# ATTron/astroz

Hardware: AMD Instinct MI355X
Metric: propagations/sec, 13,478 sats x 1,440 times, at 1/2/4/8 MI355X (higher is better)
Workload: dtype f64

## Files before the change

astroz_amd/csrc/astroz_hip.hip:

```cpp
#include "../../include/astroz_hip.h"

#include <hip/hip_runtime.h>
#include <dlfcn.h>
#include <rccl/rccl.h>

#include <algorithm>
#include <atomic>
#include <cmath>
#include <condition_variable>
#include <deque>
#include <map>
#include <cstdio>
#include <cstdlib>
#include <cstring>
#include <mutex>
#include <new>
#include <memory>
#include <string>
#include <thread>
#include <type_traits>
#include <vector>

#include "kernels.h"
#include "passes_kernel.h"
#include "coverage_kernel.h"
#include "sun.h"
#include "eclipse_kernel.h"
#include "los.h"
#include "access_kernel.h"
#include "conjunction.h"
#include "conjunction_kernel.h"
#include "tle_host.h"
#include "host_step.h"

namespace {

thread_local std::string g_last_error;

bool hip_ok(hipError_t e, const char *what)
{
    if (e == hipSuccess) return true;
    g_last_error = std::string(what) + ": " + hipGetErrorString(e);
    (void)hipGetLastError();
    return false;
}
#define HIP_TRY(expr)                                                                                       \
    do {                                                                                                    \
        if (!hip_ok((expr), #expr)) return AZ_ERR_HIP;                                                      \
    } while (0)

AzGrav make_grav(int which)
{
    AzGrav g;
    if (which == AZ_WGS72) {
        g.radius_km = 6378.135;
        g.j2 = 0.001082616;
        g.j4 = -0.00000165597;
        g.xke = 0.0743669161331734132;
        g.j3oj2 = -0.00234506972242078;
    } else {
        g.radius_km = 6378.137;
        g.j2 = 0.00108262998905;
        g.j4 = -0.00000161098761;
        g.xke = 0.07436685316871385;
        g.j3oj2 = -0.00233899967218727;
    }
    g.vkmpersec = g.xke * g.radius_km / 60.0;
    g.half_j2 = 0.5 * g.j2;
    return g;
}

const char *const kFieldNames[] = {
#define X(n) #n,
    AZ_SGP4_FIELDS(X) AZ_DEEP_FIELDS(X)
#undef X
};


template <class T>
struct DevBuf {
    T *p = nullptr;
    size_t cap = 0;
    DevBuf() = default;
    DevBuf(DevBuf &&o) noexcept { swap(o); }
    DevBuf &operator=(DevBuf &&o) noexcept { swap(o); return *this; }
    ~DevBuf() { if (p) (void)hipFree(p); }
    void swap(DevBuf &o) noexcept { std::swap(p, o.p); std::swap(cap, o.cap); }
    int ensure(size_t n)
    {
        if (n <= cap) return AZ_OK;
        if (p) (void)hipFree(p);
        p = nullptr;
        cap = 0;
        size_t want = std::max<size_t>(n, 64);
        if (!hip_ok(hipMalloc((void **)&p, want * sizeof(T)), "hipMalloc")) return AZ_ERR_HIP;
        cap = want;
        return AZ_OK;
    }
};

struct PinnedBuf {
    void *p = nullptr;
    size_t cap = 0;
    PinnedBuf() = default;
    PinnedBuf(PinnedBuf &&o) noexcept { swap(o); }
    PinnedBuf &operator=(PinnedBuf &&o) noexcept { swap(o); return *this; }
    ~PinnedBuf() { if (p) (void)hipHostFree(p); }
    void swap(PinnedBuf &o) noexcept { std::swap(p, o.p); std::swap(cap, o.cap); }
    int32_t ensure(size_t bytes)
    {
        if (bytes <= cap) return AZ_OK;
        size_t want = std::max<size_t>(cap, 65536);
        while (want < bytes) want *= 2;
        if (p) (void)hipHostFree(p);
        p = nullptr;
        cap = 0;
        if (!hip_ok(hipHostMalloc(&p, want, hipHostMallocDefault), "hipHostMalloc")) return AZ_ERR_HIP;
        cap = want;
        return AZ_OK;
    }
};

template <class H, hipError_t (*Create)(H *, unsigned), hipError_t (*Destroy)(H)>
class HipHandle {
  public:
    HipHandle() = default;
    HipHandle(HipHandle &&o) noexcept { swap(o); }
    HipHandle &operator=(HipHandle &&o) noexcept { swap(o); return *this; }
    ~HipHandle() { reset(); }
    void swap(HipHandle &o) noexcept { std::swap(h_, o.h_); std::swap(own_, o.own_); }
    hipError_t create(unsigned flags)
    {
        reset();
        own_ = true;
        return Create(&h_, flags);
    }
    void borrow(H h)
    {
        reset();
        h_ = h;
        own_ = false;
    }
    void reset()
    {
        if (h_ && own_) (void)Destroy(h_);
        h_ = nullptr;
    }
    bool owned() const { return h_ && own_; }
    operator H() const { return h_; }

  private:
    H h_ = nullptr;
    bool own_ = false;
};
using Stream = HipHandle<hipStream_t, hipStreamCreateWithFlags, hipStreamDestroy>;
using Event = HipHandle<hipEvent_t, hipEventCreateWithFlags, hipEventDestroy>;

constexpr int kStageSlots = 3;
constexpr size_t kStageChunk = size_t(16) << 20;
struct HostStager {
    Event ev[kStageSlots];
    PinnedBuf slot[kStageSlots];
    int32_t ensure()
    {
        for (int k = 0; k < kStageSlots; ++k) {
            if (slot[k].ensure(kStageChunk) != AZ_OK) return AZ_ERR_HIP;
            if (!ev[k] && !hip_ok(ev[k].create(hipEventDisableTiming), "hipEventCreate")) return AZ_ERR_HIP;
        }
        return AZ_OK;
    }
};
}

struct azh_constellation {
    int device = 0;
    size_t n = 0, n_pad = 0;
    AzGrav g{};
    Stream s_main, s_deep, s_ecc;
    Event ev_fork, ev_join, ev_fork2, ev_join2, ev_t0, ev_t1;
    Event ev_one;
    Event ev_graph;
    DevBuf<double> d_el;
    DevBuf<unsigned> d_flags;
    std::vector<unsigned> h_flags;
    std::vector<double> h_epoch;
    std::vector<double> h_raw[AZ_NUM_RAW];
    DevBuf<unsigned> d_list;
    std::vector<unsigned> h_list;
    unsigned n_sgp4 = 0, n_sdp4 = 0, n_bad = 0;
    DevBuf<double> d_times, d_offsets, d_sin, d_cos, d_seeds;
    DevBuf<double> d_node_cache;
    struct FastPlan {
        bool valid = false, mixed32 = false;
        unsigned tile_c = 0, tile_e = 0, n_list = 0, n_seg = 0, parity = 0;
        DevBuf<double> win;
        DevBuf<unsigned char> flag;
        DevBuf<unsigned> redo;
    } plan[4];
    int last_plan = -1;
    DevBuf<double> d_inc;
    DevBuf<double> d_fast_rec;
    double uniform_step = 0.0;
    DevBuf<float> d_delta;
    double delta_max = 0.0;
    std::vector<float> h_delta;
    DevBuf<double> d_delta64;
    std::vector<double> h_delta64;
    bool delta_wide = false;
    double grid_t0 = 0.0;
    unsigned last_path = 0;
    DevBuf<double> d_tgt, d_part_d2, d_out_d;
    DevBuf<unsigned> d_part_t, d_out_t;
    DevBuf<double> d_one_t, d_one_o;
    DevBuf<unsigned char> d_one_e;
    DevBuf<unsigned> d_one_items;
    unsigned one_segments = 0;
    PinnedBuf h_stage;
    std::vector<double> h_times, h_offsets;
    std::vector<uint8_t> h_mask;
    double staged_ref_jd = 0.0;
    hipStream_t staged_stream = nullptr;
    bool staged_valid = false;
    PinnedBuf h_small;
    HostStager stager;
    bool seeds_valid = false;
    unsigned seeds_tile = 0;
    bool seeds_rows = false;
    DevBuf<unsigned char> d_mask;
    DevBuf<double> d_host_pos, d_host_vel;
    DevBuf<unsigned char> d_host_err;
    bool have_offsets = false, have_mask = false;
    AzObserver obs{};
    DevBuf<AzObserver> d_obs;
    bool have_observer = false, obs_dirty = false;
    DevBuf<double> d_pass_pos, d_pass_vel;
    DevBuf<unsigned char> d_pass_err;
    DevBuf<azh_pass> d_pass_out;
    DevBuf<uint32_t> d_pass_n;
    std::vector<AzStation> h_stations;
    DevBuf<AzStation> d_stations;
    DevBuf<azh_coverage> d_cov_stats;
    DevBuf<uint32_t> d_cov_counts;
    DevBuf<AzSunPoint> d_sun;
    DevBuf<azh_eclipse> d_ecl_out;
    DevBuf<unsigned char> d_ecl_state;
    DevBuf<double> d_acc_track;
    DevBuf<azh_access> d_acc_out;
    DevBuf<unsigned char> d_acc_state;
    DevBuf<double> d_conj_track;
    std::vector<unsigned> h_conj_slots;
    DevBuf<unsigned> d_conj_slots;
    DevBuf<azh_conjunction> d_conj_out;
    unsigned cached_n_times = 0;
    int cached_mode = 0;
    unsigned off_cat = 0;
    unsigned off_deep_cat = 0;
    unsigned off_rowmap = 0;
    unsigned off_rowmap2 = 0;
    struct LaunchGraph {
        const void *pos, *vel, *err;
        int layout, f32;
        size_t stride, row_lo, row_hi;
        hipStream_t st;
        unsigned sig_before, sig_after;
        unsigned path;
        unsigned seen;
        unsigned fails;
        hipGraph_t graph;
        hipGraphExec_t exec;
        int plan = -1;
    };
    std::vector<LaunchGraph> graphs;
    int graphs_on = 0;
    bool capturing = false;
    int cols_kernel = 0;
    DevBuf<double> d_deep_tmp;
    bool tile_kernel = true;
    unsigned off_circ = 0, n_circ = 0;
    bool timed = false;
    bool timing = true;
    unsigned tile_sgp4 = 0, tile_sdp4 = 0;
    int f32_mode = 0;
    bool fast_path = true;
    std::vector<double> h_el;
    std::vector<std::pair<size_t, std::vector<double>>> h_cols;
    size_t h_cols_next = 0;
    ~azh_constellation();
};

namespace {

constexpr size_t kHostMirrorPad = 64;
constexpr size_t kHostCols = 256;
constexpr size_t kHostColsBeforeTable = 8;
constexpr size_t kHostTableMax = size_t(64) << 20;
std::atomic<size_t> g_host_points{[] {
    const char *e = getenv("ASTROZ_AMD_HOST_POINTS");
    return e ? (size_t)strtoull(e, nullptr, 10) : size_t(128);
}()};
inline size_t host_points() { return azhost::cpu_ok() ? g_host_points.load(std::memory_order_relaxed) : 0; }

constexpr int32_t AZ_RC_EAGER = 0x7a5eca9;
int set_device(const azh_constellation *c) { return hip_ok(hipSetDevice(c->device), "hipSetDevice") ? AZ_OK : AZ_ERR_HIP; }

hipStream_t small_stream(int device)
{
    static std::mutex mu;
    static std::map<int, hipStream_t> streams;
    std::lock_guard<std::mutex> lk(mu);
    auto it = streams.find(device);
    if (it != streams.end()) return it->second;
    hipStream_t s = nullptr;
    if (!hip_ok(hipStreamCreateWithFlags(&s, hipStreamNonBlocking), "hipStreamCreate")) return nullptr;
    streams[device] = s;
    return s;
}

void drop_graphs(azh_constellation *c);

int32_t build(const std::vector<double> (&cols)[AZ_NUM_RAW], size_t n, int grav, int device, azh_constellation **out)
{
    if (!out) return AZ_ERR_NULL_POINTER;
    *out = nullptr;
    if (n == 0) return AZ_ERR_VALUE;
    if (n > 0x7fffffffu) return AZ_ERR_VALUE;
    int ndev = 0;
    HIP_TRY(hipGetDeviceCount(&ndev));
    if (device < 0 || device >= ndev) {
        g_last_error = "no such HIP device";
        return AZ_ERR_HIP;
    }
    std::unique_ptr<azh_constellation> c(new (std::nothrow) azh_constellation());
    if (!c) return AZ_ERR_ALLOC_FAILED;
    c->device = device;
    c->n = n;
    c->n_pad = (n + 63) / 64 * 64;
    c->g = make_grav(grav);
    if (set_device(c.get()) != AZ_OK) return AZ_ERR_HIP;
    if (n > 16) {
        if (!hip_ok(c->s_main.create(hipStreamNonBlocking), "hipStreamCreate") ||
            !hip_ok(c->s_deep.create(hipStreamNonBlocking), "hipStreamCreate") ||
            !hip_ok(c->s_ecc.create(hipStreamNonBlocking), "hipStreamCreate") ||
            !hip_ok(c->ev_graph.create(hipEventDisableTiming | hipEventDisableSystemFence), "hipEventCreate"))
            return AZ_ERR_HIP;
    } else {
        c->s_main.borrow(small_stream(device));
        if (!c->s_main) return AZ_ERR_HIP;
        c->s_deep.borrow(c->s_main);
        c->s_ecc.borrow(c->s_main);
    }
    for (Event *e : {&c->ev_fork2, &c->ev_join2, &c->ev_fork, &c->ev_join, &c->ev_one})
        if (!hip_ok(e->create(hipEventDisableTiming), "hipEventCreate")) return AZ_ERR_HIP;
    if (!hip_ok(c->ev_t0.create(hipEventDefault), "hipEventCreate") || !hip_ok(c->ev_t1.create(hipEventDefault), "hipEventCreate"))
        return AZ_ERR_HIP;
    const size_t np = c->n_pad;
    DevBuf<double> d_raw;
    if (c->d_el.ensure((size_t)AZ_NUM_FIELDS * np) != AZ_OK || c->d_flags.ensure(np) != AZ_OK || d_raw.ensure((size_t)AZ_NUM_RAW * np) != AZ_OK)
        return AZ_ERR_HIP;
    std::vector<double> staging((size_t)AZ_NUM_RAW * np, 0.0);
    for (int k = 0; k < AZ_NUM_RAW; ++k) memcpy(&staging[(size_t)k * np], cols[k].data(), sizeof(double) * n);
    if (!hip_ok(hipMemcpyAsync(d_raw.p, staging.data(), sizeof(double) * staging.size(), hipMemcpyHostToDevice, c->s_main), "H2D raw") ||
        !hip_ok(hipMemsetAsync(c->d_el.p, 0, sizeof(double) * AZ_NUM_FIELDS * np, c->s_main), "memset el") ||
        !hip_ok(hipMemsetAsync(c->d_flags.p, 0, sizeof(unsigned) * np, c->s_main), "memset flags"))
        return AZ_ERR_HIP;
    hipLaunchKernelGGL(k_init, dim3((unsigned)(np / 64)), dim3(64), 0, c->s_main, d_raw.p, n, np, c->g, c->d_el.p, c->d_flags.p);
    if (!hip_ok(hipGetLastError(), "k_init launch")) return AZ_ERR_HIP;
    c->h_flags.resize(n);
    if (np <= kHostMirrorPad) {
        c->h_el.resize((size_t)AZ_NUM_FIELDS * np);
        if (!hip_ok(hipMemcpyAsync(c->h_el.data(), c->d_el.p, sizeof(double) * c->h_el.size(), hipMemcpyDeviceToHost, c->s_main), "D2H el"))
            return AZ_ERR_HIP;
    }
    if (!hip_ok(hipMemcpyAsync(c->h_flags.data(), c->d_flags.p, sizeof(unsigned) * n, hipMemcpyDeviceToHost, c->s_main), "D2H flags") ||
        !hip_ok(hipStreamSynchronize(c->s_main), "sync(init)"))
        return AZ_ERR_HIP;
    c->h_epoch = cols[R_epoch_jd];
    for (int k = 0; k < AZ_NUM_RAW; ++k) c->h_raw[k] = cols[k];
    std::vector<unsigned> list;
    list.reserve(n);
    for (size_t s = 0; s < n; ++s)
        if (AZ_FLAG_ERR(c->h_flags[s]) == 0 && !(c->h_flags[s] & AZ_FLAG_DEEP)) list.push_back((unsigned)s);
    c->n_sgp4 = (unsigned)list.size();
    for (size_t g0 = 0; g0 < list.size(); g0 += AZ_BLOCK) {
        const size_t g1 = std::min(g0 + (size_t)AZ_BLOCK, list.size());
        std::stable_sort(list.begin() + g0, list.begin() + g1, [&](unsigned x, unsigned y) {
            return AZ_FLAG_ECLASS(c->h_flags[x]) < AZ_FLAG_ECLASS(c->h_flags[y]);
        });
    }
    {
        std::vector<unsigned> deep;
        for (size_t s = 0; s < n; ++s)
            if (AZ_FLAG_ERR(c->h_flags[s]) == 0 && (c->h_flags[s] & AZ_FLAG_DEEP)) deep.push_back((unsigned)s);
        const std::vector<double> &incl = cols[R_incl_deg];
        auto key = [&](unsigned s) {
            const unsigned f = c->h_flags[s];
            const unsigned low = incl[s] < 12.5 ? 1u : 0u;
            return (AZ_FLAG_IREZ(f) << 4) | (low << 2) | AZ_FLAG_ECLASS(f);
        };
        std::stable_sort(deep.begin(), deep.end(), [&](unsigned x, unsigned y) { return key(x) < key(y); });
        list.insert(list.end(), deep.begin(), deep.end());
    }
    c->n_sdp4 = (unsigned)list.size() - c->n_sgp4;
    for (size_t s = 0; s < n; ++s)
        if (AZ_FLAG_ERR(c->h_flags[s]) != 0) list.push_back((unsigned)s);
    c->n_bad = (unsigned)list.size() - c->n_sgp4 - c->n_sdp4;
    c->off_circ = (unsigned)list.size();
    for (size_t s = 0; s < n; ++s)
        if (AZ_FLAG_ERR(c->h_flags[s]) == 0 && !(c->h_flags[s] & AZ_FLAG_DEEP) && AZ_FLAG_ECLASS(c->h_flags[s]) == 0)
            list.push_back((unsigned)s);
    c->n_circ = (unsigned)list.size() - c->off_circ;
    for (size_t s = 0; s < n; ++s)
        if (AZ_FLAG_ERR(c->h_flags[s]) == 0 && !(c->h_flags[s] & AZ_FLAG_DEEP) && AZ_FLAG_ECLASS(c->h_flags[s]) != 0)
            list.push_back((unsigned)s);
    c->off_cat = (unsigned)list.size();
    for (size_t s = 0; s < n; ++s)
        if (AZ_FLAG_ERR(c->h_flags[s]) == 0 && !(c->h_flags[s] & AZ_FLAG_DEEP)) list.push_back((unsigned)s);
    c->off_deep_cat = (unsigned)list.size();
    for (size_t s = 0; s < n; ++s)
        if (AZ_FLAG_ERR(c->h_flags[s]) == 0 && (c->h_flags[s] & AZ_FLAG_DEEP)) list.push_back((unsigned)s);
    c->off_rowmap = (unsigned)list.size();
    {
        unsigned near = 0, deepn = 0;
        for (size_t s = 0; s < n; ++s) {
            const unsigned f = c->h_flags[s];
            if (AZ_FLAG_ERR(f) != 0) list.push_back((unsigned)AZ_ROW_ZERO << 30);
            else if (f & AZ_FLAG_DEEP) list.push_back(((unsigned)AZ_ROW_COPY << 30) | deepn++);
            else list.push_back(((unsigned)AZ_ROW_NEAR << 30) | near++);
        }
    }
    c->off_rowmap2 = (unsigned)list.size();
    {
        unsigned circ = 0, eccn = 0, deepn = 0;
        for (size_t s = 0; s < n; ++s) {
            const unsigned f = c->h_flags[s];
            if (AZ_FLAG_ERR(f) != 0) list.push_back((unsigned)AZ_ROW_ZERO << 30);
            else if (f & AZ_FLAG_DEEP) list.push_back(((unsigned)AZ_ROW_COPY << 30) | deepn++);
            else if (AZ_FLAG_ECLASS(f) == 0) list.push_back(((unsigned)AZ_ROW_NEAR << 30) | circ++);
            else list.push_back(((unsigned)AZ_ROW_NEAR << 30) | (c->n_circ + eccn++));
        }
    }
    if (const char *e = getenv("ASTROZ_AMD_COLS")) c->cols_kernel = atoi(e);
    if (const char *e = getenv("ASTROZ_AMD_GRAPHS")) c->graphs_on = atoi(e);
    c->h_list = list;
    if (c->d_list.ensure(list.size()) != AZ_OK ||
        !hip_ok(hipMemcpy(c->d_list.p, list.data(), sizeof(unsigned) * list.size(), hipMemcpyHostToDevice), "H2D list"))
        return AZ_ERR_HIP;
    *out = c.release();
    return AZ_OK;
}

int32_t build_from_records(const std::vector<azh::TleRecord> &recs, int grav, int device, azh_constellation **out)
{
    std::vector<double> cols[AZ_NUM_RAW];
    for (auto &v : cols) v.resize(recs.size());
    azh::parallel_ranges(recs.size(), azh::parse_threads_for(recs.size() * 140), [&](size_t a, size_t b) {
        for (size_t i = a; i < b; ++i) {
            const azh::TleRecord &r = recs[i];
            cols[R_epoch_jd][i] = r.epoch_jd;
            cols[R_mm_revday][i] = r.mm_revday;
            cols[R_ecc][i] = r.ecc;
            cols[R_incl_deg][i] = r.incl_deg;
            cols[R_raan_deg][i] = r.raan_deg;
            cols[R_argp_deg][i] = r.argp_deg;
            cols[R_ma_deg][i] = r.ma_deg;
            cols[R_bstar][i] = r.bstar;
        }
    });
    return build(cols, recs.size(), grav, device, out);
}

unsigned auto_tile(unsigned n_list, unsigned n_times, unsigned forced, unsigned min_tile)
{
    if (forced) return std::min(std::max(forced, 1u), std::max(n_times, 1u));
    const unsigned waves_x = (n_list + 63) / 64;
    unsigned n_tiles = (16384 + waves_x - 1) / std::max(waves_x, 1u);
    n_tiles = std::max(1u, std::min(n_tiles, n_times));
    unsigned tile = (n_times + n_tiles - 1) / n_tiles;
    tile = std::max(tile, std::min(min_tile, n_times));
    return std::max(tile, 1u);
}

inline unsigned pad8(unsigned n) { return (n + 7) / 8 * 8; }
inline unsigned cgrid_y(unsigned n_times, unsigned tile) { return (n_times + tile - 1) / tile; }

template <int V>
using int_c = std::integral_constant<int, V>;
template <class F>
void with_bool(bool b, F &&f)
{
    if (b) f(std::true_type{});
    else f(std::false_type{});
}
template <class F>
void with_vel_frame(bool vel, int mode, F &&f)
{
    const int frame = mode == AZ_OUT_TOPOCENTRIC ? 3 : (mode == AZ_OUT_GEODETIC ? 2 : (mode != AZ_OUT_TEME ? 1 : 0));
    with_bool(vel, [&](auto VEL) {
        if (frame == 3) f(VEL, int_c<3>{});
        else if (frame == 2) f(VEL, int_c<2>{});
        else if (frame == 1) f(VEL, int_c<1>{});
        else f(VEL, int_c<0>{});
    });
}
constexpr int gen_frame(int frame) { return frame == 3 ? 3 : (frame != 0 ? 1 : 0); }
template <class F>
void with_outputs(const PropArgs &a, bool vel, F &&f)
{
    if (a.screen_target) return f(std::false_type{}, int_c<0>{}, int_c<AZ_SINK_SCREEN>{});
    with_vel_frame(vel, a.mode, [&](auto VEL, auto FRAME) {
        if (a.f32) f(VEL, FRAME, int_c<AZ_SINK_F32>{});
        else f(VEL, FRAME, int_c<AZ_SINK_F64>{});
    });
}
template <class F>
void with_delta(int form, F &&f)
{
    if (form == 2) f(int_c<2>{});
    else if (form == 1) f(int_c<1>{});
    else f(int_c<0>{});
}

int32_t stream_after(hipStream_t to, hipStream_t from, hipEvent_t ev)
{
    HIP_TRY(hipEventRecord(ev, from));
    HIP_TRY(hipStreamWaitEvent(to, ev, 0));
    return AZ_OK;
}

unsigned rows_tile(unsigned n_list, unsigned n_times, unsigned forced)
{
    unsigned segs = std::max(1u, std::min((16384u + n_list - 1) / std::max(n_list, 1u), (n_times + 255) / 256));
    if (forced) segs = std::max(1u, (n_times + forced - 1) / forced);
    return ((n_times + segs - 1) / segs + 63) / 64 * 64;
}

bool use_rows(const PropArgs &a, int layout, bool deep)
{
    if (deep && layout == AZ_LAYOUT_TIME_MAJOR && a.n_times >= 32) return true;
    return (layout == AZ_LAYOUT_SAT_MAJOR || a.screen_target) && a.n_times >= 32;
}

unsigned screen_parts(const PropArgs &a, bool deep)
{
    if (use_rows(a, AZ_LAYOUT_SAT_MAJOR, deep)) {
        unsigned tile = rows_tile(a.n_list, a.n_times, a.tile_forced);
        if (deep) tile = std::min(tile, 64u * (unsigned)AZ_DEEP_SEED_MAX);
        return cgrid_y(a.n_times, tile);
    }
    return cgrid_y(a.n_times, a.tile);
}

struct EccSide {
    hipStream_t stream = nullptr;
    hipEvent_t fork = nullptr, join = nullptr;
};

struct FastShape {
    unsigned tile_c = 0, tile_e = 0;
    bool packed32 = false;
    bool mixed32 = false;
    int kind = 0;
};
unsigned fast_window_cap(double step)
{
    const double span = 3000.0 / std::max(std::fabs(step), 1e-9);
    return span >= 4.0e9 ? 0xffffffc0u : std::max(64u, (unsigned)span / 64u * 64u);
}
FastShape fast_shape_rows(const PropArgs &a, unsigned n_sgp4, unsigned n_circ)
{
    FastShape f;
    const unsigned cap = fast_window_cap(a.uniform_step);
    const unsigned n_ecc = n_sgp4 - n_circ;
    f.tile_c = std::min(rows_tile(n_sgp4, a.n_times, a.tile_forced), cap);
    f.tile_e = n_circ >= 4u * n_ecc ? f.tile_c : std::min(rows_tile(std::max(n_ecc, 1u), a.n_times, 256), cap);
    if (a.delta || a.delta64) {
        f.tile_c = std::min(f.tile_c, (unsigned)AZ_DELTA_SEG);
        f.tile_e = std::min(f.tile_e, (unsigned)AZ_DELTA_SEG);
    }
    f.packed32 = a.f32 && a.mode == AZ_OUT_TEME && a.arith32 != 2 && cap >= 128u && !a.delta_wide;
    f.mixed32 = f.packed32 && a.arith32 == 0;
    if (f.packed32) f.tile_c = std::max(128u, f.tile_c / 128u * 128u);
    f.kind = f.packed32 ? 1 : 0;
    return f;
}
FastShape fast_shape_tiles(const PropArgs &a, unsigned n_rows)
{
    FastShape f;
    unsigned tile = std::min(rows_tile(std::max((n_rows + 15u) / 16u, 1u) * 16u, a.n_times, a.tile_forced), fast_window_cap(a.uniform_step));
    if (a.mode != AZ_OUT_TEME) tile = std::min(tile, (unsigned)AZ_TILE_SEG_MAX);
    if (a.delta || a.delta64) tile = std::min(tile, (unsigned)AZ_DELTA_SEG);
    f.tile_c = f.tile_e = tile;
    f.kind = 2;
    return f;
}

template <bool VEL, int FRAME, int SINK, bool ECC>
void launch_rows_fast(const PropArgs &a, unsigned n_slots, hipStream_t st)
{
    with_delta(a.delta_wide ? 2 : (a.delta ? 1 : 0), [&](auto DELTA) {
        hipLaunchKernelGGL((k_rows_fast<VEL, FRAME, SINK, ECC, DELTA>), dim3(pad8(n_slots), cgrid_y(a.n_times, a.tile)), dim3(64), 0, st, a);
    });
}
PropArgs ecc_part(const PropArgs &a, unsigned tile)
{
    PropArgs e = a;
    e.list = a.list + a.n_circ;
    e.n_list = a.n_list - a.n_circ;
    e.tile = tile;
    e.redo_slot0 = a.n_circ;
    return e;
}
template <bool VEL, int FRAME, int SINK>
void launch_redo(const PropArgs &a, dim3 grid, hipStream_t st)
{
    hipLaunchKernelGGL((k_rows<VEL, gen_frame(FRAME), SINK, true>), grid, dim3(64), 0, st, a);
}

int32_t launch_near_fast(const PropArgs &a, bool vel, const FastShape &shape, dim3 rgrid, hipStream_t st, const EccSide &side)
{
    PropArgs e = ecc_part(a, shape.tile_e), c = a;
    c.n_list = a.n_circ;
    c.tile = shape.tile_c;
    unsigned n_e = e.n_list, n_c = c.n_list;
    if (a.row_lo > 0 || a.row_hi < a.n_rows) {
        c.slot_lo = a.win_circ_lo; c.slot_hi = a.win_circ_hi; n_c = c.slot_hi - c.slot_lo;
        e.slot_lo = a.win_ecc_lo; e.slot_hi = a.win_ecc_hi; n_e = e.slot_hi - e.slot_lo;
        if (c.slot_hi == 0) c.n_list = n_c = 0;
        if (e.slot_hi == 0) e.n_list = n_e = 0;
    }
    const bool beside = side.stream != nullptr && n_c;
    const hipStream_t se = beside ? side.stream : st;
    if (beside)
        if (int32_t rc = stream_after(se, st, side.fork); rc != AZ_OK) return rc;
    with_outputs(a, vel, [&](auto VEL, auto FRAME, auto SINK) {
        if (n_e) launch_rows_fast<VEL, FRAME, SINK, true>(e, n_e, se);
        launch_redo<VEL, FRAME, SINK>(a, rgrid, se);
        if (n_c && FRAME == 0 && shape.packed32)
            with_bool(shape.mixed32, [&](auto MIXED) {
                with_bool(a.delta != nullptr, [&](auto DELTA) {
                    hipLaunchKernelGGL((k_rows_fast32<VEL, MIXED, DELTA>), dim3(pad8(n_c), cgrid_y(a.n_times, c.tile)), dim3(64), 0, st, c);
                });
            });
        else if (n_c)
            launch_rows_fast<VEL, FRAME, SINK, false>(c, n_c, st);
    });
    return beside ? stream_after(st, se, side.join) : AZ_OK;
}

void launch_tiles(const PropArgs &a0, bool vel, hipStream_t st, const FastShape &shape)
{
    PropArgs a = a0, r = a0;
    a.tile = r.tile = shape.tile_c;
    r.tm_rows = 1;
    const dim3 grid(pad8((a.n_rows + 15u) / 16u), cgrid_y(a.n_times, a.tile));
    with_vel_frame(vel, a.mode, [&](auto VEL, auto FRAME) {
        with_bool(a.delta64 != nullptr, [&](auto WIDE) {
            hipLaunchKernelGGL((k_tiles_fast<VEL, FRAME, WIDE ? 2 : 0>), grid, dim3(1024), 0, st, a);
        });
        launch_redo<VEL, FRAME, AZ_SINK_F64>(r, dim3(256, 4), st);
    });
}
unsigned cols_tile(unsigned n_rows, unsigned n_times, unsigned forced, double step)
{
    const unsigned cap = fast_window_cap(step);
    if (forced) return std::min(std::max(forced, 1u), std::min(std::max(n_times, 1u), cap));
    const unsigned groups = (n_rows + 63u) / 64u, places = 1024u * (unsigned)AZ_COLS_WAVES;
    const unsigned segs = std::max(1u, places / std::max(groups, 1u));
    unsigned tile = (n_times + segs - 1u) / segs;
    if (tile < 32u) tile = std::min(128u, std::max(n_times, 1u));
    return std::max(1u, std::min(tile, cap));
}
FastShape fast_shape_cols(const PropArgs &a, unsigned n_rows, unsigned n_sgp4, unsigned n_circ)
{
    FastShape f = fast_shape_rows(a, n_sgp4, n_circ);
    f.tile_e = std::min(rows_tile(std::max(n_sgp4 - n_circ, 1u), a.n_times, a.tile_forced ? a.tile_forced : 256u), fast_window_cap(a.uniform_step));
    if (a.delta || a.delta64) f.tile_e = std::min(f.tile_e, (unsigned)AZ_DELTA_SEG);
    f.tile_c = cols_tile(n_rows, a.n_times, a.tile_forced, a.uniform_step);
    f.packed32 = f.mixed32 = false;
    f.kind = 3;
    return f;
}
int32_t launch_cols(const PropArgs &a0, bool vel, hipStream_t st, const FastShape &shape, const EccSide &side, unsigned ecc_row0)
{
    PropArgs a = a0;
    PropArgs e = ecc_part(a, shape.tile_e);
    e.pos = const_cast<double *>(a.tmp_pos);
    e.vel = vel ? const_cast<double *>(a.tmp_vel) : nullptr;
    e.rows_compact = 1;
    e.ecc_row0 = ecc_row0;
    if (e.n_list) {
        const hipStream_t se = side.stream ? side.stream : st;
        if (se != st)
            if (int32_t rc = stream_after(se, st, side.fork); rc != AZ_OK) return rc;
        with_vel_frame(vel, a.mode, [&](auto VEL, auto FRAME) { launch_rows_fast<VEL, FRAME, AZ_SINK_F64, true>(e, e.n_list, se); });
        if (se != st)
            if (int32_t rc = stream_after(st, se, side.join); rc != AZ_OK) return rc;
    }
    a.tile = shape.tile_c;
    a.ecc_row0 = ecc_row0;
    PropArgs r = a;
    r.tm_rows = 1;
    const dim3 grid(pad8((a.n_rows + 63u) / 64u), cgrid_y(a.n_times, a.tile));
    with_vel_frame(vel, a.mode, [&](auto VEL, auto FRAME) {
        with_bool(a.delta64 != nullptr, [&](auto WIDE) {
            hipLaunchKernelGGL((k_cols_fast<VEL, FRAME, WIDE ? 2 : 0>), grid, dim3(64), 0, st, a);
        });
        launch_redo<VEL, FRAME, AZ_SINK_F64>(r, dim3(256, 4), st);
    });
    return AZ_OK;
}

unsigned launch_propagate(const PropArgs &a, int layout, bool vel, bool deep, hipStream_t st)
{
    if (use_rows(a, layout, deep)) {
        PropArgs b = a;
        b.tile = rows_tile(a.n_list, a.n_times, a.tile_forced);
        if (deep) b.tile = std::min(b.tile, 64u * (unsigned)AZ_DEEP_SEED_MAX);
        const unsigned n_slots = a.slot_hi ? a.slot_hi - a.slot_lo : a.n_list;
        const dim3 grid(pad8(n_slots), cgrid_y(a.n_times, b.tile));
        with_outputs(a, vel, [&](auto VEL, auto FRAME, auto SINK) {
            if (deep) hipLaunchKernelGGL((k_rows_deep<VEL, gen_frame(FRAME), SINK>), grid, dim3(64), 0, st, b);
            else hipLaunchKernelGGL((k_rows<VEL, gen_frame(FRAME), SINK>), grid, dim3(64), 0, st, b);
        });
        return deep ? AZH_PATH_DEEP_ROWS : AZH_PATH_ROWS_GENERIC;
    }
    const dim3 grid(pad8((a.n_list + AZ_BLOCK - 1) / AZ_BLOCK), cgrid_y(a.n_times, a.tile));
    with_bool(deep, [&](auto DEEP) {
        if (a.screen_target)
            hipLaunchKernelGGL((k_propagate<0, false, DEEP, 0, true>), grid, dim3(AZ_BLOCK), 0, st, a);
        else
            with_bool(layout == AZ_LAYOUT_TIME_MAJOR, [&](auto TIME_MAJOR) {
                with_vel_frame(vel, a.mode, [&](auto VEL, auto FRAME) {
                    hipLaunchKernelGGL((k_propagate<TIME_MAJOR, VEL, DEEP, gen_frame(FRAME)>), grid, dim3(AZ_BLOCK), 0, st, a);
                });
            });
    });
    return AZH_PATH_LANE_SAT;
}

int32_t stage_inputs(azh_constellation *c, const double *times, size_t n_times, const double *offsets,
                     const uint8_t *mask, int mode, double reference_jd, hipStream_t st)
{
    if (n_times > 0xffffffffu) return AZ_ERR_VALUE;
    {
        const bool same = c->staged_valid && st == c->staged_stream && n_times == c->h_times.size() && mode == c->cached_mode &&
                          (mode == AZ_OUT_TEME || reference_jd == c->staged_ref_jd) &&
                          (offsets != nullptr) == c->have_offsets && (mask != nullptr) == c->have_mask &&
                          (n_times == 0 || memcmp(times, c->h_times.data(), sizeof(double) * n_times) == 0) &&
                          (!offsets || (c->h_offsets.size() == c->n && memcmp(offsets, c->h_offsets.data(), sizeof(double) * c->n) == 0)) &&
                          (!mask || (c->h_mask.size() == c->n && memcmp(mask, c->h_mask.data(), c->n) == 0));
        if (same) return AZ_OK;
        c->staged_valid = false;
    }
    if (c->d_times.ensure(n_times) != AZ_OK) return AZ_ERR_HIP;
    HIP_TRY(hipMemcpyAsync(c->d_times.p, times, sizeof(double) * n_times, hipMemcpyHostToDevice, st));
    c->have_offsets = offsets != nullptr;
    if (offsets) {
        if (c->d_offsets.ensure(c->n) != AZ_OK) return AZ_ERR_HIP;
        HIP_TRY(hipMemcpyAsync(c->d_offsets.p, offsets, sizeof(double) * c->n, hipMemcpyHostToDevice, st));
    }
    c->have_mask = mask != nullptr;
    if (mask) {
        if (c->d_mask.ensure(c->n) != AZ_OK) return AZ_ERR_HIP;
        HIP_TRY(hipMemcpyAsync(c->d_mask.p, mask, c->n, hipMemcpyHostToDevice, st));
    }
    if (mode != AZ_OUT_TEME) {
        if (c->d_sin.ensure(n_times) != AZ_OK || c->d_cos.ensure(n_times) != AZ_OK) return AZ_ERR_HIP;
        hipLaunchKernelGGL(k_gmst, dim3((unsigned)((n_times + 255) / 256)), dim3(256), 0, st, c->d_times.p,
                           (unsigned)n_times, reference_jd, c->d_sin.p, c->d_cos.p);
        HIP_TRY(hipGetLastError());
    }
    c->cached_n_times = (unsigned)n_times;
    c->cached_mode = mode;
    c->seeds_valid = false;
    drop_graphs(c);
    for (auto &pl : c->plan) pl.valid = false;
    c->last_plan = -1;
    c->uniform_step = 0.0;
    c->delta_max = 0.0;
    c->delta_wide = false;
    c->grid_t0 = n_times ? times[0] : 0.0;
    if (n_times >= 2) {
        double t0 = times[0], step = (times[n_times - 1] - t0) / (double)(n_times - 1);
        double tmax = std::max(std::fabs(t0), std::fabs(times[n_times - 1]));
        const double tol = 4.0 * 2.220446049250313e-16 * std::max(tmax, std::fabs(step));
        bool uni = std::isfinite(step) && step != 0.0;
        double dmax = 0.0;
        for (size_t i = 1; uni && i < n_times; ++i) {
            dmax = std::max(dmax, std::fabs(times[i] - std::fma((double)i, step, t0)));
            uni = dmax <= AZ_DELTA_MAX;
        }
        if (uni && dmax > tol) {
            c->h_delta.assign(n_times + AZ_DELTA_SEG, 0.0f);
            for (size_t i = 0; i < n_times; ++i) c->h_delta[i] = (float)(times[i] - std::fma((double)i, step, t0));
            if (c->d_delta.ensure(c->h_delta.size()) != AZ_OK) return AZ_ERR_HIP;
            HIP_TRY(hipMemcpyAsync(c->d_delta.p, c->h_delta.data(), sizeof(float) * c->h_delta.size(), hipMemcpyHostToDevice, st));
            c->h_delta64.assign(n_times + AZ_DELTA_SEG, 0.0);
            for (size_t i = 0; i < n_times; ++i) c->h_delta64[i] = times[i] - std::fma((double)i, step, t0);
            if (c->d_delta64.ensure(c->h_delta64.size()) != AZ_OK) return AZ_ERR_HIP;
            HIP_TRY(hipMemcpyAsync(c->d_delta64.p, c->h_delta64.data(), sizeof(double) * c->h_delta64.size(), hipMemcpyHostToDevice, st));
            c->delta_max = dmax * (1.0 + 1e-6) + 1e-12;
        }
        if (!uni && n_times >= 64) {
            const double nn = (double)n_times, im = 0.5 * (nn - 1.0);
            double tm = 0.0;
            for (size_t i = 0; i < n_times; ++i) tm += times[i];
            tm /= nn;
            double sxy = 0.0, sxx = 0.0;
            for (size_t i = 0; i < n_times; ++i) {
                sxy += ((double)i - im) * (times[i] - tm);
                sxx += ((double)i - im) * ((double)i - im);
            }
            step = sxy / sxx;
            t0 = tm - step * im;
            bool ok = std::isfinite(step) && std::isfinite(t0) && step != 0.0;
            dmax = 0.0;
            for (size_t i = 0; ok && i < n_times; ++i) {
                dmax = std::max(dmax, std::fabs(times[i] - std::fma((double)i, step, t0)));
                ok = dmax <= AZ_DELTA_WIDE_MAX;
            }
            if (ok && dmax <= 0.5 * std::fabs(step)) {
                c->h_delta64.assign(n_times + AZ_DELTA_SEG, 0.0);
                for (size_t i = 0; i < n_times; ++i) c->h_delta64[i] = times[i] - std::fma((double)i, step, t0);
                if (c->d_delta64.ensure(c->h_delta64.size()) != AZ_OK) return AZ_ERR_HIP;
                HIP_TRY(hipMemcpyAsync(c->d_delta64.p, c->h_delta64.data(), sizeof(double) * c->h_delta64.size(), hipMemcpyHostToDevice, st));
                c->delta_max = dmax * (1.0 + 1e-6) + 1e-12;
                c->delta_wide = true;
                c->grid_t0 = t0;
                uni = true;
            }
        }
        if (uni) {
            if (c->d_inc.ensure((size_t)2 * AZ_INC_NUM * c->n_pad) != AZ_OK) return AZ_ERR_HIP;
            hipLaunchKernelGGL(k_prep_inc, dim3((unsigned)((c->n + 255) / 256)), dim3(256), 0, st, c->d_el.p, c->n, c->n_pad,
                               step, c->d_inc.p);
            HIP_TRY(hipGetLastError());
            if (c->d_fast_rec.ensure((size_t)FR_NUM * c->n_pad) != AZ_OK) return AZ_ERR_HIP;
            hipLaunchKernelGGL(k_prep_rec, dim3((unsigned)((c->n + 255) / 256)), dim3(256), 0, st, c->d_el.p, c->d_flags.p, c->n, c->n_pad,
                               c->d_inc.p, c->d_fast_rec.p);
            HIP_TRY(hipGetLastError());
            c->uniform_step = step;
        }
    }
    try {
        c->h_times.assign(times, times + n_times);
        if (offsets) c->h_offsets.assign(offsets, offsets + c->n);
        if (mask) c->h_mask.assign(mask, mask + c->n);
        c->staged_ref_jd = reference_jd;
        c->staged_stream = st;
        c->staged_valid = true;
    } catch (const std::bad_alloc &) {
        c->staged_valid = false;
    }
    return AZ_OK;
}

int32_t prepare_deep(azh_constellation *c, PropArgs &d, hipStream_t st, bool rows, bool beside_bulk = false)
{
    const unsigned n_times = d.n_times;
    d.list = c->d_list.p + (rows ? c->off_deep_cat : c->n_sgp4);
    d.n_list = c->n_sdp4;
    d.tile = auto_tile(c->n_sdp4, n_times, c->tile_sdp4, 8);
    d.tile_forced = c->tile_sdp4 ? c->tile_sdp4 : (rows && beside_bulk && c->n_sgp4 >= 4u * c->n_sdp4 ? rows_tile(c->n_sgp4, n_times, c->tile_sgp4) : 0u);
    const unsigned seed_tile = rows ? 64u : d.tile;
    const unsigned n_tiles = (n_times + seed_tile - 1) / seed_tile;
    if (!c->seeds_valid || c->seeds_tile != seed_tile || c->seeds_rows != rows) {
        if (c->capturing) return AZ_RC_EAGER;
        drop_graphs(c);
        if (c->d_seeds.ensure((size_t)n_tiles * 3 * c->n_sdp4) != AZ_OK) return AZ_ERR_HIP;
        if (c->d_node_cache.p == nullptr) {
            if (c->d_node_cache.ensure(3 * c->n_pad) != AZ_OK) return AZ_ERR_HIP;
            HIP_TRY(hipMemsetAsync(c->d_node_cache.p, 0, sizeof(double) * 3 * c->n_pad, st));
        }
        hipLaunchKernelGGL(k_deep_seed, dim3((c->n_sdp4 + 63) / 64), dim3(64), 0, st, c->d_el.p, c->d_flags.p, c->n_pad,
                           d.list, c->n_sdp4, d.times, n_times, d.offsets, seed_tile, c->d_seeds.p, rows ? 1 : 0, c->d_node_cache.p);
        HIP_TRY(hipGetLastError());
        c->seeds_valid = true;
        c->seeds_tile = seed_tile;
        c->seeds_rows = rows;
    }
    d.seeds = c->d_seeds.p;
    return AZ_OK;
}

int32_t ensure_plan(azh_constellation *c, PropArgs &a, const FastShape &shape, hipStream_t st)
{
    azh_constellation::FastPlan &pl = c->plan[shape.kind];
    const unsigned n_list = a.n_list;
    const unsigned n_seg = (a.n_times + std::min(shape.tile_c, shape.tile_e) - 1) / std::min(shape.tile_c, shape.tile_e);
    if (!pl.valid || pl.tile_c != shape.tile_c || pl.tile_e != shape.tile_e || pl.n_list != n_list || pl.mixed32 != shape.mixed32) {
        if (c->capturing) return AZ_RC_EAGER;
        drop_graphs(c);
        const size_t items = (size_t)n_list * n_seg + ((size_t)a.n_times + 63) / 64 * (c->n_sgp4 - c->n_circ);
        if (pl.redo.cap < 4 + 3 * items || pl.win.cap < (size_t)n_list * n_seg * AZ_PLAN_NUM) HIP_TRY(hipStreamSynchronize(st));
        if (pl.redo.ensure(4 + 3 * items) != AZ_OK || pl.win.ensure((size_t)n_list * n_seg * AZ_PLAN_NUM) != AZ_OK ||
            pl.flag.ensure((size_t)n_list * n_seg) != AZ_OK)
            return AZ_ERR_HIP;
        HIP_TRY(hipMemsetAsync(pl.redo.p, 0, 4 * sizeof(unsigned), st));
        HIP_TRY(hipMemsetAsync(pl.flag.p, 0, (size_t)n_list * n_seg, st));
        PlanArgs q{};
        q.el = a.el; q.flags = a.flags; q.n_pad = a.n_pad; q.list = a.list; q.n_list = n_list; q.n_circ = a.n_circ;
        q.n_times = a.n_times; q.tile_c = shape.tile_c; q.tile_e = shape.tile_e; q.by_flags = shape.kind == 2 ? 1u : 0u;
        q.times = a.times; q.offsets = a.offsets; q.inc = a.inc; q.step = a.uniform_step; q.dt_mult = shape.kind == 1 ? 128.0 : 64.0;
        q.delta_max = (a.delta || a.delta64) ? a.delta_max : 0.0;
        q.grid_t0 = a.grid_t0;
        q.f32_mixed = shape.mixed32 ? 1u : 0u;
        q.win = pl.win.p; q.flag = pl.flag.p;
        q.redo_static = pl.redo.p + 2; q.redo_c0 = pl.redo.p; q.redo_c1 = pl.redo.p + 1; q.redo_items = pl.redo.p + 4;
        q.g = a.g;
        hipLaunchKernelGGL(k_plan_windows, dim3((n_list + 255) / 256, n_seg), dim3(256), 0, st, q);
        hipLaunchKernelGGL(k_plan_arm, dim3(1), dim3(64), 0, st, q.redo_static, q.redo_c0, q.redo_c1);
        HIP_TRY(hipGetLastError());
        pl.valid = true;
        pl.tile_c = shape.tile_c; pl.tile_e = shape.tile_e; pl.n_list = n_list; pl.n_seg = n_seg; pl.parity = 0; pl.mixed32 = shape.mixed32;
    }
    c->last_plan = (int)shape.kind;
    a.plan_win = pl.win.p;
    a.plan_flag = pl.flag.p;
    a.plan_stride = n_list;
    a.redo_static = pl.redo.p + 2;
    a.redo_count = pl.redo.p + pl.parity;
    a.redo_next = pl.redo.p + (pl.parity ^ 1u);
    a.redo_items = pl.redo.p + 4;
    pl.parity ^= 1u;
    return AZ_OK;
}

void drop_graphs(azh_constellation *c)
{
    if (c->graphs.empty()) return;
    if (hipEventSynchronize(c->ev_graph) != hipSuccess) (void)hipGetLastError();
    for (auto &g : c->graphs) {
        if (g.exec) (void)hipGraphExecDestroy(g.exec);
        if (g.graph) (void)hipGraphDestroy(g.graph);
    }
    c->graphs.clear();
}
}

azh_constellation::~azh_constellation()
{
    (void)hipSetDevice(device);
    drop_graphs(this);
}

namespace {
unsigned plan_sig(const azh_constellation *c)
{
    unsigned s = 0;
    for (unsigned k = 0; k < 4; ++k) s |= (c->plan[k].parity & 1u) << k;
    return s;
}

int32_t launch_all(azh_constellation *c, double *d_pos, double *d_vel, int layout, size_t stride, uint8_t *d_err,
                   hipStream_t st, int f32 = 0, size_t row_lo = 0, size_t row_hi = ~(size_t)0)
{
    const unsigned n_times = c->cached_n_times;
    if (n_times == 0) return AZ_OK;
    row_hi = std::min(row_hi, c->n);
    if (row_lo >= row_hi) return AZ_OK;
    if (stride == 0) stride = c->n;
    if (layout == AZ_LAYOUT_TIME_MAJOR && stride < c->n) return AZ_ERR_VALUE;
    c->last_plan = -1;

    PropArgs a{};
    a.el = c->d_el.p;
    a.flags = c->d_flags.p;
    a.n_pad = c->n_pad;
    a.times = c->d_times.p;
    a.n_times = n_times;
    a.offsets = c->have_offsets ? c->d_offsets.p : nullptr;
    a.pos = d_pos;
    a.vel = d_vel;
    a.sin_g = c->d_sin.p;
    a.cos_g = c->d_cos.p;
    a.mask = c->have_mask ? c->d_mask.p : nullptr;
    a.err = d_err;
    a.stride_sats = stride;
    a.mode = c->cached_mode;
    if (a.mode == AZ_OUT_TOPOCENTRIC) {
        if (c->obs_dirty) {
            if (c->capturing) return AZ_RC_EAGER;
            if (c->d_obs.ensure(1) != AZ_OK) return AZ_ERR_HIP;
            HIP_TRY(hipMemcpyAsync(c->d_obs.p, &c->obs, sizeof(AzObserver), hipMemcpyHostToDevice, st));
            c->obs_dirty = false;
        }
        a.obs = c->d_obs.p;
    }
    a.f32 = f32;
    a.arith32 = f32 ? c->f32_mode : 2;
    a.g = c->g;
    a.uniform_step = c->fast_path ? c->uniform_step : 0.0;
    a.inc = (a.uniform_step != 0.0) ? c->d_inc.p : nullptr;
    a.fast_rec = (a.uniform_step != 0.0) ? c->d_fast_rec.p : nullptr;
    a.delta = (a.uniform_step != 0.0 && c->delta_max > 0.0 && !c->delta_wide) ? c->d_delta.p : nullptr;
    a.delta64 = (a.uniform_step != 0.0 && c->delta_max > 0.0) ? c->d_delta64.p : nullptr;
    a.delta_wide = c->delta_wide ? 1 : 0;
    a.grid_t0 = c->grid_t0;
    a.delta_max = c->delta_max;
    a.grid_exact_uniform = (c->uniform_step != 0.0 && c->delta_max == 0.0) ? 1 : 0;
    a.row_lo = (unsigned)row_lo;
    a.row_hi = (unsigned)row_hi;
    const bool windowed = row_lo > 0 || row_hi < c->n;
    auto slots_of = [&](unsigned off, unsigned cnt, unsigned &lo, unsigned &hi) {
        const unsigned *b = c->h_list.data() + off, *e = b + cnt;
        lo = (unsigned)(std::lower_bound(b, e, (unsigned)row_lo) - b);
        hi = (unsigned)(std::lower_bound(b, e, (unsigned)row_hi) - b);
    };
    unsigned deep_lo = 0, deep_hi = 0;
    if (windowed) {
        slots_of(c->off_circ, c->n_circ, a.win_circ_lo, a.win_circ_hi);
        slots_of(c->off_circ + c->n_circ, c->n_sgp4 - c->n_circ, a.win_ecc_lo, a.win_ecc_hi);
        slots_of(c->off_deep_cat, c->n_sdp4, deep_lo, deep_hi);
    }

    unsigned path = 0;
    if (c->timing) HIP_TRY(hipEventRecord(c->ev_t0, st));
    if (d_err) HIP_TRY(hipMemsetAsync(d_err + row_lo * (size_t)n_times, 0, (row_hi - row_lo) * (size_t)n_times, st));
    const bool tiles = c->n_sgp4 > 0 && c->tile_kernel && a.inc != nullptr && layout == AZ_LAYOUT_TIME_MAJOR && !f32 &&
                       n_times >= 64 &&
                       (size_t)stride * 64 * 24 < 0xf0000000ull;
    const bool cols = tiles && c->cols_kernel != 0 && a.mask == nullptr;
    const unsigned n_ecc = c->n_sgp4 - c->n_circ;
    const size_t scratch_rows = (size_t)c->n_sdp4 + (cols ? n_ecc : 0u);
    const size_t scratch_per = scratch_rows * n_times * 3, scratch_words = f32 ? (scratch_per + 1) / 2 : scratch_per;
    auto ensure_scratch = [&](hipStream_t user) -> int32_t {
        if (c->capturing && c->d_deep_tmp.cap < scratch_words * (d_vel ? 2 : 1)) return AZ_RC_EAGER;
        if (c->d_deep_tmp.cap < scratch_words * (d_vel ? 2 : 1)) {
            drop_graphs(c);
            HIP_TRY(hipStreamSynchronize(user));
        }
        if (c->d_deep_tmp.ensure(scratch_words * (d_vel ? 2 : 1)) != AZ_OK) return AZ_ERR_HIP;
        a.tmp_pos = c->d_deep_tmp.p;
        a.tmp_vel = d_vel ? c->d_deep_tmp.p + scratch_words : nullptr;
        return AZ_OK;
    };
    const bool fork = c->n_sdp4 > 0;
    if (cols && !fork && n_ecc)
        if (int32_t rc = ensure_scratch(st); rc != AZ_OK) return rc;
    if (fork) {
        if (int32_t rc = stream_after(c->s_deep, st, c->ev_fork); rc != AZ_OK) return rc;
        PropArgs d = a;
        const bool deep_rows = use_rows(d, layout, true);
        const bool deep_skip = windowed && deep_rows && deep_hi == deep_lo;
        if (windowed && deep_rows) { d.slot_lo = deep_lo; d.slot_hi = deep_hi; }
        if (int32_t rc = prepare_deep(c, d, c->s_deep, deep_rows, !tiles && a.inc != nullptr); rc != AZ_OK) return rc;
        if (deep_rows && layout == AZ_LAYOUT_TIME_MAJOR) {
            if (int32_t rc = ensure_scratch(c->s_deep); rc != AZ_OK) return rc;
            PropArgs t = d;
            t.pos = const_cast<double *>(a.tmp_pos);
            t.vel = const_cast<double *>(a.tmp_vel);
            t.rows_compact = 1;
            if (!deep_skip) path |= launch_propagate(t, AZ_LAYOUT_SAT_MAJOR, d_vel != nullptr, true, c->s_deep);
            HIP_TRY(hipGetLastError());
            dim3 tg((c->n_sdp4 + AZ_TR_ROWS - 1) / AZ_TR_ROWS, (n_times + 63) / 64);
            if (tiles || deep_skip) {  }
            else if (f32)
                hipLaunchKernelGGL((k_deep_transpose<float>), tg, dim3(192), 0, c->s_deep, reinterpret_cast<const float *>(t.pos),
                                   reinterpret_cast<const float *>(t.vel), reinterpret_cast<float *>(d_pos), reinterpret_cast<float *>(d_vel),
                                   d.list, c->n_sdp4, n_times, stride, d.mask, d.row_lo, d.row_hi);
            else
                hipLaunchKernelGGL((k_deep_transpose<double>), tg, dim3(192), 0, c->s_deep, t.pos, t.vel, d_pos, d_vel, d.list, c->n_sdp4,
                                   n_times, stride, d.mask, d.row_lo, d.row_hi);
        } else if (!deep_skip) {
            path |= launch_propagate(d, layout, d_vel != nullptr, true, c->s_deep);
        }
        HIP_TRY(hipGetLastError());
        HIP_TRY(hipEventRecord(c->ev_join, c->s_deep));
    }
    if (c->n_sgp4 > 0) {
        a.list = c->d_list.p;
        a.n_list = c->n_sgp4;
        a.tile = auto_tile(c->n_sgp4, n_times, c->tile_sgp4, 8);
        a.tile_forced = c->tile_sgp4;
        if (tiles && fork) HIP_TRY(hipStreamWaitEvent(st, c->ev_join, 0));
        if (tiles && !cols) a.list = c->d_list.p + c->off_cat;
        FastShape shape;
        const bool fast = a.inc != nullptr && (tiles || use_rows(a, layout, false));
        if (fast) {
            if (!tiles || cols) a.list = c->d_list.p + c->off_circ;
            a.n_list = c->n_sgp4;
            a.n_circ = c->n_circ;
            a.rowmap = c->d_list.p + (cols ? c->off_rowmap2 : c->off_rowmap);
            a.n_rows = (unsigned)c->n;
            shape = cols ? fast_shape_cols(a, (unsigned)c->n, c->n_sgp4, c->n_circ)
                         : (tiles ? fast_shape_tiles(a, (unsigned)c->n) : fast_shape_rows(a, c->n_sgp4, c->n_circ));
            if (int32_t rc = ensure_plan(c, a, shape, st); rc != AZ_OK) return rc;
        }
        const EccSide side{c->s_ecc, c->ev_fork2, c->ev_join2};
        if (a.n_list > 0 && cols) {
            if (int32_t rc = launch_cols(a, d_vel != nullptr, st, shape, side, c->n_sdp4); rc != AZ_OK) return rc;
            path |= AZH_PATH_COLS_FAST;
        } else if (a.n_list > 0 && tiles) {
            launch_tiles(a, d_vel != nullptr, st, shape);
            path |= AZH_PATH_TILES_FAST;
        } else if (a.n_list > 0 && fast) {
            const dim3 rgrid(std::min(8192u, std::max(256u, (a.n_list * cgrid_y(a.n_times, shape.tile_c) + 63u) / 64u)), 4);
            if (int32_t rc = launch_near_fast(a, d_vel != nullptr, shape, rgrid, st, side); rc != AZ_OK) return rc;
            path |= AZH_PATH_ROWS_FAST;
        } else if (a.n_list > 0) {
            path |= launch_propagate(a, layout, d_vel != nullptr, false, st);
        }
        if ((a.delta || a.delta64) && (path & (AZH_PATH_TILES_FAST | AZH_PATH_ROWS_FAST | AZH_PATH_COLS_FAST))) path |= AZH_PATH_QUASI_UNIFORM;
        HIP_TRY(hipGetLastError());
    }
    if (c->n_bad > 0) {
        hipLaunchKernelGGL(k_fill_bad, dim3((n_times + 255) / 256, c->n_bad), dim3(256), 0, st,
                           c->d_list.p + c->n_sgp4 + c->n_sdp4, c->n_bad, c->d_flags.p, n_times, d_pos, d_vel, d_err,
                           c->have_mask ? c->d_mask.p : nullptr, layout, stride, f32, a.row_lo, a.row_hi);
        HIP_TRY(hipGetLastError());
    }
    if (fork && !tiles) HIP_TRY(hipStreamWaitEvent(st, c->ev_join, 0));
    c->last_path = path;
    if (c->timing) {
        HIP_TRY(hipEventRecord(c->ev_t1, st));
        c->timed = true;
    }
    return AZ_OK;
}

int32_t launch_cached(azh_constellation *c, double *d_pos, double *d_vel, int layout, size_t stride, uint8_t *d_err, hipStream_t st,
                      int f32 = 0, size_t row_lo = 0, size_t row_hi = ~(size_t)0)
{
    if (!c->graphs_on || c->timing || c->cached_n_times == 0 || !c->s_main.owned()) return launch_all(c, d_pos, d_vel, layout, stride, d_err, st, f32, row_lo, row_hi);
    const unsigned sig = plan_sig(c);
    azh_constellation::LaunchGraph *hit = nullptr, *pending = nullptr;
    for (auto &g : c->graphs)
        if (g.pos == d_pos && g.vel == d_vel && g.err == d_err && g.layout == layout && g.f32 == f32 && g.stride == stride &&
            g.row_lo == row_lo && g.row_hi == row_hi && g.st == st) {
            if (g.fails >= 2) return launch_all(c, d_pos, d_vel, layout, stride, d_err, st, f32, row_lo, row_hi);
            if (g.exec && g.sig_before == sig) { hit = &g; break; }
            if (!g.exec && g.sig_before == sig) pending = &g;
        }
    if (hit) {
        HIP_TRY(hipGraphLaunch(hit->exec, st));
        for (unsigned k = 0; k < 4; ++k) c->plan[k].parity = (hit->sig_after >> k) & 1u;
        c->last_path = hit->path;
        c->last_plan = hit->plan;
        HIP_TRY(hipEventRecord(c->ev_graph, st));
        return AZ_OK;
    }
    if (!pending) {
        if (c->graphs.size() >= 24) drop_graphs(c);
        const int32_t rc = launch_all(c, d_pos, d_vel, layout, stride, d_err, st, f32, row_lo, row_hi);
        if (rc == AZ_OK) {
            try {
                c->graphs.push_back({d_pos, d_vel, d_err, layout, f32, stride, row_lo, row_hi, st, sig, plan_sig(c), c->last_path, 1u, 0u, nullptr, nullptr});
            } catch (const std::bad_alloc &) {
            }
        }
        return rc;
    }
    if (hipStreamBeginCapture(st, hipStreamCaptureModeThreadLocal) != hipSuccess) {
        (void)hipGetLastError();
        return launch_all(c, d_pos, d_vel, layout, stride, d_err, st, f32, row_lo, row_hi);
    }
    unsigned parity0[4];
    for (unsigned k = 0; k < 4; ++k) parity0[k] = c->plan[k].parity;
    c->capturing = true;
    const int32_t rc = launch_all(c, d_pos, d_vel, layout, stride, d_err, st, f32, row_lo, row_hi);
    c->capturing = false;
    hipGraph_t graph = nullptr;
    const hipError_t e_end = hipStreamEndCapture(st, &graph);
    hipGraphExec_t exec = nullptr;
    if (rc != AZ_OK || e_end != hipSuccess || !graph || hipGraphInstantiate(&exec, graph, nullptr, nullptr, 0) != hipSuccess) {
        (void)hipGetLastError();
        if (graph) (void)hipGraphDestroy(graph);
        for (unsigned k = 0; k < 4; ++k) c->plan[k].parity = parity0[k];
        pending->fails += 1;
        if (rc != AZ_OK && rc != AZ_RC_EAGER) return rc;
        return launch_all(c, d_pos, d_vel, layout, stride, d_err, st, f32, row_lo, row_hi);
    }
    pending->graph = graph;
    pending->exec = exec;
    pending->sig_after = plan_sig(c);
    pending->path = c->last_path;
    pending->plan = c->last_plan;
    HIP_TRY(hipGraphLaunch(exec, st));
    HIP_TRY(hipEventRecord(c->ev_graph, st));
    return AZ_OK;
}

class HostPool {
  public:
    int32_t alloc(size_t bytes, void **out)
    {
        if (!out) return AZ_ERR_NULL_POINTER;
        *out = nullptr;
        const size_t need = std::max<size_t>((bytes + kGrain - 1) / kGrain * kGrain, kGrain);
        {
            std::lock_guard<std::mutex> lock(mu_);
            auto it = free_.lower_bound(need);
            if (it != free_.end() && it->first <= need + need / 4 + kGrain) {
                void *q = it->second;
                free_bytes_ -= it->first;
                live_[static_cast<char *>(q)] = it->first;
                free_.erase(it);
                *out = q;
                return AZ_OK;
            }
        }
        void *q = nullptr;
        if (hipHostMalloc(&q, need, hipHostMallocPortable) != hipSuccess || !q) {
            (void)hipGetLastError();
            trim(0);
            if (!hip_ok(hipHostMalloc(&q, need, hipHostMallocPortable), "hipHostMalloc(result)")) return AZ_ERR_ALLOC_FAILED;
        }
        std::lock_guard<std::mutex> lock(mu_);
        live_[static_cast<char *>(q)] = need;
        *out = q;
        return AZ_OK;
    }
    void release(void *q)
    {
        if (!q) return;
        {
            std::lock_guard<std::mutex> lock(mu_);
            auto it = live_.find(static_cast<char *>(q));
            if (it == live_.end()) return;
            free_.emplace(it->second, q);
            free_bytes_ += it->second;
            live_.erase(it);
        }
        trim(cap());
    }
    bool owns(const void *q, size_t len)
    {
        if (!q) return false;
        std::lock_guard<std::mutex> lock(mu_);
        auto it = live_.upper_bound(const_cast<char *>(static_cast<const char *>(q)));
        if (it == live_.begin()) return false;
        --it;
        return static_cast<const char *>(q) + len <= it->first + it->second;
    }
    void stats(size_t *live_bytes, size_t *free_bytes)
    {
        std::lock_guard<std::mutex> lock(mu_);
        size_t l = 0;
        for (auto &kv : live_) l += kv.second;
        if (live_bytes) *live_bytes = l;
        if (free_bytes) *free_bytes = free_bytes_;
    }
    void trim(size_t keep)
    {
        std::vector<void *> drop;
        {
            std::lock_guard<std::mutex> lock(mu_);
            while (free_bytes_ > keep && !free_.empty()) {
                auto it = std::prev(free_.end());
                drop.push_back(it->second);
                free_bytes_ -= it->first;
                free_.erase(it);
            }
        }
        for (void *q : drop) (void)hipHostFree(q);
    }

  private:
    static constexpr size_t kGrain = size_t(2) << 20;
    static size_t cap()
    {
        static const size_t c = [] {
            const char *e = getenv("ASTROZ_AMD_HOST_POOL_MB");
            return (size_t)(e ? std::max(0L, atol(e)) : 4096L) << 20;
        }();
        return c;
    }
    std::mutex mu_;
    std::map<char *, size_t> live_;
    std::multimap<size_t, void *> free_;
    size_t free_bytes_ = 0;
};
HostPool &host_pool()
{
    static HostPool *p = new HostPool();
    return *p;
}

class CopyPool {
  public:
    explicit CopyPool(unsigned k)
    {
        for (unsigned i = 0; i < k; ++i) {
            try {
                th_.emplace_back([this, i] { work(i); });
            } catch (const std::system_error &) {
                break;
            }
        }
    }
    unsigned size() const { return (unsigned)th_.size(); }
    size_t submit(char *dst, const char *src, size_t len)
    {
        std::lock_guard<std::mutex> lock(mu_);
        jobs_.push_back({dst, src, len, (unsigned)th_.size()});
        cv_.notify_all();
        return jobs_.size() - 1;
    }
    void wait(size_t ticket)
    {
        std::unique_lock<std::mutex> lock(mu_);
        done_cv_.wait(lock, [&] { return jobs_[ticket].left == 0; });
    }
    ~CopyPool()
    {
        {
            std::lock_guard<std::mutex> lock(mu_);
            stop_ = true;
            cv_.notify_all();
        }
        for (auto &t : th_) t.join();
    }

  private:
    struct Job {
        char *dst;
        const char *src;
        size_t len;
        unsigned left;
    };
    void work(unsigned me)
    {
        size_t next = 0;
        for (;;) {
            Job j;
            {
                std::unique_lock<std::mutex> lock(mu_);
                cv_.wait(lock, [&] { return stop_ || next < jobs_.size(); });
                if (next >= jobs_.size()) return;
                j = jobs_[next];
            }
            const size_t k = th_.size(), piece = ((j.len + k - 1) / k + 63) & ~size_t(63);
            const size_t lo = std::min(j.len, piece * me), hi = std::min(j.len, piece * (me + 1));
            if (hi > lo) memcpy(j.dst + lo, j.src + lo, hi - lo);
            {
                std::lock_guard<std::mutex> lock(mu_);
                if (--jobs_[next].left == 0) done_cv_.notify_all();
            }
            ++next;
        }
    }
    std::mutex mu_;
    std::condition_variable cv_, done_cv_;
    std::deque<Job> jobs_;
    std::vector<std::thread> th_;
    bool stop_ = false;
};
std::atomic<int> g_host_copy_threads{-1};

int32_t copy_back_staged(HostStager &hs, void *const *dst, const void *const *src, const size_t *bytes, int n_arrays, hipStream_t st,
                         unsigned threads)
{
    if (int32_t rc = hs.ensure(); rc != AZ_OK) return rc;
    struct Chunk {
        char *dst;
        const char *src;
        size_t len;
    };
    std::vector<Chunk> chunks;
    for (int k = 0; k < n_arrays; ++k)
        for (size_t o = 0; o < bytes[k]; o += kStageChunk)
            chunks.push_back({static_cast<char *>(dst[k]) + o, static_cast<const char *>(src[k]) + o, std::min(kStageChunk, bytes[k] - o)});
    CopyPool pool(threads);
    const bool pooled = pool.size() > 0;
    std::vector<size_t> ticket(chunks.size(), 0);
    auto land = [&](size_t i) -> int32_t {
        HIP_TRY(hipEventSynchronize(hs.ev[i % kStageSlots]));
        if (pooled) ticket[i] = pool.submit(chunks[i].dst, static_cast<const char *>(hs.slot[i % kStageSlots].p), chunks[i].len);
        else memcpy(chunks[i].dst, hs.slot[i % kStageSlots].p, chunks[i].len);
        return AZ_OK;
    };
    for (size_t i = 0; i < chunks.size(); ++i) {
        if (pooled && i >= (size_t)kStageSlots) pool.wait(ticket[i - kStageSlots]);
        HIP_TRY(hipMemcpyAsync(hs.slot[i % kStageSlots].p, chunks[i].src, chunks[i].len, hipMemcpyDeviceToHost, st));
        HIP_TRY(hipEventRecord(hs.ev[i % kStageSlots], st));
        if (i >= 1)
            if (int32_t rc = land(i - 1); rc != AZ_OK) return rc;
    }
    if (!chunks.empty())
        if (int32_t rc = land(chunks.size() - 1); rc != AZ_OK) return rc;
    if (pooled)
        for (size_t i = chunks.size() > (size_t)kStageSlots ? chunks.size() - kStageSlots : 0; i < chunks.size(); ++i) pool.wait(ticket[i]);
    return AZ_OK;
}

unsigned host_copy_threads()
{
    const int want = g_host_copy_threads.load(std::memory_order_relaxed);
    if (want >= 0) return (unsigned)want;
    return std::min(6u, std::max(1u, std::thread::hardware_concurrency() / 2));
}

#ifndef AZ_ONE_FAST
#define AZ_ONE_FAST 1
#endif
constexpr size_t kOneFastMin = size_t(1) << 20;
int32_t launch_one(azh_constellation *c, size_t sat, const double *d_t, size_t n, double *d_p, double *d_v, unsigned char *d_e,
                   int interleaved, hipStream_t st)
{
    const unsigned f = sat < c->h_flags.size() ? c->h_flags[sat] : ~0u;
    const bool fast = AZ_ONE_FAST && !interleaved && n >= kOneFastMin && f != ~0u && AZ_FLAG_ERR(f) == 0 && !(f & AZ_FLAG_DEEP);
    c->one_segments = 0;
    if (fast) {
        const unsigned n_seg = (unsigned)((n + AZ_ONE_SEG - 1) / AZ_ONE_SEG);
        const unsigned cap = (n_seg + AZ_ONE_LISTS - 1) / AZ_ONE_LISTS;
        if (c->d_one_items.ensure((size_t)AZ_ONE_HEAD + (size_t)cap * AZ_ONE_LISTS) != AZ_OK) return AZ_ERR_HIP;
        c->one_segments = n_seg;
        HIP_TRY(hipMemsetAsync(c->d_one_items.p, 0, sizeof(unsigned) * AZ_ONE_HEAD, st));
        if (d_v)
            hipLaunchKernelGGL((k_one_fast<true>), dim3(n_seg), dim3(64), 0, st, c->d_el.p, c->d_flags.p, c->n_pad, (unsigned)sat, d_t,
                               (unsigned)n, d_p, d_v, d_e, c->g, (const double *)nullptr, c->d_one_items.p, cap);
        else
            hipLaunchKernelGGL((k_one_fast<false>), dim3(n_seg), dim3(64), 0, st, c->d_el.p, c->d_flags.p, c->n_pad, (unsigned)sat, d_t,
                               (unsigned)n, d_p, d_v, d_e, c->g, (const double *)nullptr, c->d_one_items.p, cap);
        HIP_TRY(hipGetLastError());
        hipLaunchKernelGGL((k_one_satellite<true>), dim3(4096), dim3(64), 0, st, c->d_el.p, c->d_flags.p, c->n_pad, (unsigned)sat, d_t,
                           (unsigned)n, d_p, d_v, d_e, 0, c->g, (const double *)nullptr, 0, (const unsigned *)c->d_one_items.p, cap);
        HIP_TRY(hipEventRecord(c->ev_one, st));
    } else {
        hipLaunchKernelGGL((k_one_satellite<false>), dim3((unsigned)((n + 63) / 64)), dim3(64), 0, st, c->d_el.p, c->d_flags.p, c->n_pad,
                           (unsigned)sat, d_t, (unsigned)n, d_p, d_v, d_e, interleaved, c->g, (const double *)nullptr, 0,
                           (const unsigned *)nullptr);
    }
    HIP_TRY(hipGetLastError());
    return AZ_OK;
}

#ifndef AZ_ONE_ZERO_COPY
#define AZ_ONE_ZERO_COPY 1
#endif
#ifndef AZ_ONE_ZERO_COPY_MAX
#define AZ_ONE_ZERO_COPY_MAX 16384
#endif
constexpr size_t kOneStage = 16384;
constexpr size_t kOnePointBytes = 7 * sizeof(double) + 8;
constexpr size_t kSmallOut = size_t(512) << 10;
constexpr size_t kOneZeroCopy = AZ_ONE_ZERO_COPY_MAX;

const double *host_column(azh_constellation *c, size_t sat, size_t &n_pad, size_t &col)
{
    if (!c->h_el.empty()) {
        n_pad = c->n_pad;
        col = sat;
        return c->h_el.data();
    }
    for (auto &e : c->h_cols)
        if (e.first == sat) {
            n_pad = 1;
            col = 0;
            return e.second.data();
        }
    if (set_device(c) != AZ_OK) return nullptr;
    if (c->h_cols.size() >= kHostColsBeforeTable && (size_t)AZ_NUM_FIELDS * c->n_pad * sizeof(double) <= kHostTableMax) {
        try {
            c->h_el.resize((size_t)AZ_NUM_FIELDS * c->n_pad);
        } catch (const std::bad_alloc &) {
            c->h_el.clear();
        }
        if (!c->h_el.empty()) {
            if (hip_ok(hipMemcpy(c->h_el.data(), c->d_el.p, sizeof(double) * c->h_el.size(), hipMemcpyDeviceToHost), "D2H table")) {
                c->h_cols.clear();
                n_pad = c->n_pad;
                col = sat;
                return c->h_el.data();
            }
            c->h_el.clear();
        }
    }
    n_pad = 1;
    col = 0;
    std::vector<double> f(AZ_NUM_FIELDS);
// ... 2372 lines not shown
```

astroz_amd/csrc/fast_step.h:

```cpp
#pragma once
#include <type_traits>

#include "propagate_device.h"

#define AZ_FASTK_COLD(X)                                                                                     \
    X(cc1) X(d2) X(d3) X(d4) X(nl2) X(nl3) X(nl4) X(nl5) X(eta) X(omgcof) X(xmcof) X(xd) X(bc4) X(bc5) X(ecb) X(sab)
#define AZ_FASTK_HOT(X)                                                                                      \
    X(aycof) X(xlcof) X(xnodcf) X(sinio) X(cosio) X(k_mrt) X(k_c2u) X(k_su) X(k_node) X(k_inc) X(x1mth2) X(k_rv) \
    X(sdA) X(cdA) X(sdW) X(cdW) X(tc) X(sdU) X(cdU) X(tmid) X(nodedot) X(sOc) X(cOc)
enum FastCold {
#define X(n) FC_##n,
    AZ_FASTK_COLD(X)
#undef X
    FC_NUM
};
#define AZ_FASTK_DELTA(X) X(mdot) X(argpdot) X(udot)
enum FastColdX {
    FCX_first_ = FC_NUM - 1,
#define X(n) FCX_##n,
    AZ_FASTK_DELTA(X)
#undef X
    FCX_NUM
};
#define AZ_DELTA_MAX 4.0e-6
#define AZ_DELTA_WIDE_MAX 0.5
#define AZ_DELTA_SEG 768
struct FastK {
    static constexpr bool SCALAR = false;
#define X(n) double n##_;
    AZ_FASTK_COLD(X) AZ_FASTK_HOT(X) AZ_FASTK_DELTA(X)
#undef X
#define X(n) AZ_MEMBER double n() const { return n##_; }
    AZ_FASTK_COLD(X) AZ_FASTK_HOT(X) AZ_FASTK_DELTA(X)
#undef X
};
struct FastKBcast {
    static constexpr bool SCALAR = true;
    const double *cold;
#define X(n) double n##_;
    AZ_FASTK_HOT(X)
#undef X
#define X(n) AZ_MEMBER double n() const { return n##_; }
    AZ_FASTK_HOT(X)
#undef X
#define X(n) AZ_MEMBER double n() const { return cold[FC_##n]; }
    AZ_FASTK_COLD(X)
#undef X
#define X(n) AZ_MEMBER double n() const { return cold[FCX_##n]; }
    AZ_FASTK_DELTA(X)
#undef X
};

struct FastKCol {
    static constexpr bool SCALAR = false;
    const double *cold;
#define X(n) double n##_;
    AZ_FASTK_HOT(X)
#undef X
#define X(n) AZ_MEMBER double n() const { return n##_; }
    AZ_FASTK_HOT(X)
#undef X
#define X(n) AZ_MEMBER double n() const { return cold[FC_##n * AZ_COLD_STRIDE]; }
    AZ_FASTK_COLD(X)
#undef X
#define X(n) AZ_MEMBER double n() const { return 0.0; }
    AZ_FASTK_DELTA(X)
#undef X
};

struct FastCarry {
    double sA, cA, sW, cW, sU, cU;
};

enum { AZ_INC_sdA, AZ_INC_cdA, AZ_INC_sdW, AZ_INC_cdW, AZ_INC_NUM };

AZ_DEVICE void az_load_fast_with(const double *__restrict__ el, size_t n_pad, size_t i, unsigned flags, double sdA, double cdA,
                                 double sdW, double cdW, FastK &k)
{
#define L(f) el[(size_t)F_##f * n_pad + i]
    const bool ho = !(flags & AZ_FLAG_ISIMP);
    const double no = L(no_unkozai);
    k.cc1_ = L(cc1); k.d2_ = L(d2); k.d3_ = L(d3); k.d4_ = L(d4);
    k.nl2_ = no * L(t2cof); k.nl3_ = no * L(t3cof); k.nl4_ = no * L(t4cof); k.nl5_ = no * L(t5cof);
    k.eta_ = L(eta);
    k.omgcof_ = ho ? L(omgcof) : 0.0;
    k.xmcof_ = ho ? L(xmcof) : 0.0;
    k.xd_ = k.xmcof_ * L(delmo);
    k.bc4_ = L(bc4);
    k.bc5_ = ho ? L(bc5) : 0.0;
    k.ecb_ = fma(k.bc5_, L(sinmao), L(ecco));
    k.sab_ = L(sqrt_a_base);
    k.aycof_ = L(aycof); k.xlcof_ = L(xlcof); k.xnodcf_ = L(xnodcf);
    k.sinio_ = L(sinio); k.cosio_ = L(cosio);
    az_j2_factors(L(con41), L(x1mth2), L(x7thm1), k.sinio_, k.cosio_, k.k_mrt_, k.k_c2u_, k.k_su_, k.k_node_,
                  k.k_inc_, k.k_rv_);
    k.x1mth2_ = L(x1mth2);
    k.sdA_ = sdA; k.cdA_ = cdA;
    k.sdW_ = sdW; k.cdW_ = cdW;
    k.nodedot_ = L(nodedot);
    k.mdot_ = L(mdot); k.argpdot_ = L(argpdot);
    k.udot_ = k.mdot_ + k.argpdot_;
#undef L
}
AZ_DEVICE void az_load_fast(const double *__restrict__ el, size_t n_pad, size_t i, unsigned flags,
                            const double *__restrict__ inc, int which, FastK &k)
{
    const double *q = inc + (size_t)(AZ_INC_NUM * which) * n_pad + i;
    az_load_fast_with(el, n_pad, i, flags, q[(size_t)AZ_INC_sdA * n_pad], q[(size_t)AZ_INC_cdA * n_pad], q[(size_t)AZ_INC_sdW * n_pad],
                      q[(size_t)AZ_INC_cdW * n_pad], k);
}
AZ_DEVICE void az_fast_udot(FastK &k) { k.udot_ = fma(2.0 * k.nl2_, k.tc_, k.mdot_ + k.argpdot_); }

template <class K>
AZ_DEVICE void az_fast_window(const double *__restrict__ el, size_t n_pad, size_t i, double t_a, double t_b, double dt, K &k)
{
#define L(f) el[(size_t)F_##f * n_pad + i]
    const double kappa = L(no_unkozai) * L(t2cof);
    const double tmax = fmax(fabs(t_a), fabs(t_b));
    k.tmid_ = 0.5 * (t_a + t_b);
    az_sincos(fma(k.nodedot_, k.tmid_, L(nodeo)), k.sOc_, k.cOc_);
    if (!az_any(fabs(kappa) * tmax * tmax > 0.05)) {
        k.tc_ = 0.0;
        k.sdU_ = fma(k.sdA_, k.cdW_, k.cdA_ * k.sdW_);
        k.cdU_ = fma(k.cdA_, k.cdW_, -(k.sdA_ * k.sdW_));
    } else {
        k.tc_ = 0.5 * (t_a + t_b);
        az_sincos((L(mdot) + L(argpdot) + 2.0 * kappa * k.tc_) * dt, k.sdU_, k.cdU_);
    }
    if constexpr (std::is_same<K, FastK>::value) az_fast_udot(k);
#undef L
}

#define AZ_FASTK_HOT_REC(X)                                                                                  \
    X(aycof) X(xlcof) X(xnodcf) X(sinio) X(cosio) X(k_mrt) X(k_c2u) X(k_su) X(k_node) X(k_inc) X(x1mth2) X(k_rv) \
    X(sdA) X(cdA) X(sdW) X(cdW) X(nodedot)
enum FastRec {
    FR_COLD0 = 0,
    FR_HOT0 = FCX_NUM,
#define X(n) FR_##n,
    FR_first_hot_ = FR_HOT0 - 1,
    AZ_FASTK_HOT_REC(X)
#undef X
    FR_mo, FR_mdot, FR_argpo, FR_argpdot,
    FR_USED,
    FR_NUM = (FR_USED + 7) & ~7
};
AZ_DEVICE void az_fast_rec_store(const double *__restrict__ el, size_t n_pad, size_t i, const FastK &k, double *__restrict__ rec)
{
#define X(n) rec[FC_##n] = k.n##_;
    AZ_FASTK_COLD(X)
#undef X
    rec[FCX_mdot] = k.mdot_; rec[FCX_argpdot] = k.argpdot_; rec[FCX_udot] = k.mdot_ + k.argpdot_;
#define X(n) rec[FR_##n] = k.n##_;
    AZ_FASTK_HOT_REC(X)
#undef X
#define L(f) el[(size_t)F_##f * n_pad + i]
    rec[FR_mo] = L(mo); rec[FR_mdot] = L(mdot); rec[FR_argpo] = L(argpo); rec[FR_argpdot] = L(argpdot);
#undef L
    for (int j = FR_USED; j < FR_NUM; ++j) rec[j] = 0.0;
}
template <class K, class P = const double *__restrict__>
AZ_DEVICE void az_fast_rec_hot(P rec, K &k)
{
#define X(n) k.n##_ = rec[FR_##n];
    AZ_FASTK_HOT_REC(X)
#undef X
}
template <class M>
AZ_DEVICE void az_seed_fast_rec(const double *__restrict__ rec, double kappa, double t, double tc, FastCarry &st, const M &m)
{
    az_sincos_m(fma(rec[FR_mdot], t, rec[FR_mo]), st.sA, st.cA, m);
    az_sincos_m(fma(rec[FR_argpdot], t, rec[FR_argpo]), st.sW, st.cW, m);
    if (!az_any(tc != 0.0)) {
        st.sU = fma(st.sA, st.cW, st.cA * st.sW);
        st.cU = fma(st.cA, st.cW, -(st.sA * st.sW));
    } else {
        az_sincos_m(fma(rec[FR_mdot] + rec[FR_argpdot] + 2.0 * kappa * tc, t, rec[FR_mo] + rec[FR_argpo] - kappa * tc * tc), st.sU, st.cU, m);
    }
}

AZ_DEVICE void az_seed_fast(const double *__restrict__ el, size_t n_pad, size_t i, double t, double tc, FastCarry &st)
{
#define L(f) el[(size_t)F_##f * n_pad + i]
    az_sincos(fma(L(mdot), t, L(mo)), st.sA, st.cA);
    az_sincos(fma(L(argpdot), t, L(argpo)), st.sW, st.cW);
    if (!az_any(tc != 0.0)) {
        st.sU = fma(st.sA, st.cW, st.cA * st.sW);
        st.cU = fma(st.cA, st.cW, -(st.sA * st.sW));
    } else {
        const double kappa = L(no_unkozai) * L(t2cof);
        az_sincos(fma(L(mdot) + L(argpdot) + 2.0 * kappa * tc, t, L(mo) + L(argpo) - kappa * tc * tc), st.sU, st.cU);
    }
#undef L
}

AZ_DEVICE void az_rot_apply2(double &s, double &c, double p, double q)
{
    const double ns = fma(c, p, fma(s, q, s));
    c = fma(-s, p, fma(c, q, c));
    s = ns;
}
enum RotCoef { RC_n6, RC_p24, RC_p120, RC_n720, RC_n5040, RC_p40320, RC_p362880, RC_n3628800, RC_p8,
               RC_n11f, RC_p12f, RC_p13f, RC_n14f, RC_n15f, RC_p16f, RC_NUM };
#define AZ_RC_VALUES                                                                                                      \
    {-1.0 / 6.0, 1.0 / 24.0, 1.0 / 120.0, -1.0 / 720.0, -1.0 / 5040.0, 1.0 / 40320.0, 1.0 / 362880.0, -1.0 / 3628800.0, 0.125,     \
     -1.0 / 39916800.0, 1.0 / 479001600.0, 1.0 / 6227020800.0, -1.0 / 87178291200.0, -1.0 / 1307674368000.0,                   \
     1.0 / 20922789888000.0}
struct RotCoefLit {
    AZ_MEMBER double operator()(int k) const
    {
        constexpr double v[RC_NUM] = AZ_RC_VALUES;
        return v[k];
    }
};
struct RotCoefLds {
    const double *p;
    AZ_MEMBER double operator()(int k) const { return p[k]; }
};
template <class W>
AZ_DEVICE void az_rotcoef_store(W write)
{
    const RotCoefLit lit;
#pragma unroll
    for (int k = 0; k < RC_NUM; ++k) write(k, lit(k));
}

template <class RC>
AZ_DEVICE void az_rotate_tiny2(double &s, double &c, double d, const RC &k)
{
    const double d2 = d * d;
    const double q = -0.5 * d2;
    const double p = fma(d2 * k(RC_n6), d, d);
    az_rot_apply2(s, c, p, q);
}
template <class RC>
AZ_DEVICE void az_fpq_small(double d, const RC &k, double &p, double &q)
{
    const double d2 = d * d;
    q = d2 * fma(d2, fma(d2, k(RC_n720), k(RC_p24)), -0.5);
    p = d * fma(d2, fma(d2, k(RC_p120), k(RC_n6)), 1.0);
}

#define AZ_ROT_16TH 0.0625
template <class RC>
AZ_DEVICE void az_pq_16th(double d, const RC &k, double &p, double &q)
{
    const double d2 = d * d;
    q = d2 * fma(d2, fma(d2, fma(d2, k(RC_p40320), k(RC_n720)), k(RC_p24)), -0.5);
    p = d * fma(d2, fma(d2, fma(d2, k(RC_n5040), k(RC_p120)), k(RC_n6)), 1.0);
}

template <class RC>
AZ_DEVICE void az_pq_large(double d, const RC &k, double &p, double &q)
{
    const double d2 = d * d;
    q = fma(d2, k(RC_p16f), k(RC_n14f));
    q = fma(d2, q, k(RC_p12f));
    q = fma(d2, q, k(RC_n3628800));
    q = fma(d2, q, k(RC_p40320));
    q = fma(d2, q, k(RC_n720));
    q = fma(d2, q, k(RC_p24));
    q = d2 * fma(d2, q, -0.5);
    p = fma(d2, k(RC_n15f), k(RC_p13f));
    p = fma(d2, p, k(RC_n11f));
    p = fma(d2, p, k(RC_p362880));
    p = fma(d2, p, k(RC_n5040));
    p = fma(d2, p, k(RC_p120));
    p = fma(d2, p, k(RC_n6));
    p = d * fma(d2, p, 1.0);
}

template <class RC>
AZ_DEVICE void az_pq_med(double d, const RC &k, double &p, double &q)
{
    const double d2 = d * d;
    q = fma(d2, k(RC_n3628800), k(RC_p40320));
    q = fma(d2, q, k(RC_n720));
    q = fma(d2, q, k(RC_p24));
    q = d2 * fma(d2, q, -0.5);
    p = fma(d2, k(RC_p362880), k(RC_n5040));
    p = fma(d2, p, k(RC_p120));
    p = fma(d2, p, k(RC_n6));
    p = d * fma(d2, p, 1.0);
}


template <bool SCALAR>
AZ_DEVICE void az_pair_advance(double &s, double &c, double sd, double cd)
{
#ifndef AZ_HOST_EMUL
    if (SCALAR) {
        double m, m2;
        asm("v_mul_f64 %2, %1, %4\n\t"
            "v_mul_f64 %3, %0, %4\n\t"
            "v_fma_f64 %0, %0, %5, %2\n\t"
            "v_fma_f64 %1, %1, %5, -%3"
            : "+v"(s), "+v"(c), "=&v"(m), "=&v"(m2)
            : "s"(sd), "s"(cd));
        return;
    }
#endif
    const double ns = fma(s, cd, c * sd);
    c = fma(c, cd, -(s * sd));
    s = ns;
}

template <class RC>
AZ_DEVICE void az_pq_ecc_scaled(double d, const RC &k, double &p, double &q)
{
    const double d2 = d * d;
    q = d2 * fma(d2, k(RC_p24), -0.5);
    p = d * fma(d2, fma(d2, k(RC_p120), k(RC_n6)), 1.0);
}
template <class RC>
AZ_DEVICE void az_fpq_milli(double d, const RC &k, double &p, double &q)
{
    const double d2 = d * d;
    q = d2 * fma(d2, k(RC_p24), -0.5);
    p = fma(d2 * k(RC_n6), d, d);
}

#define AZ_FAST_EL2 1.6e-5
#define AZ_FAST_TEMP2 6.0e-4

enum { AZ_TIER_GENERAL = 0, AZ_TIER_EPS = 1, AZ_TIER_NUM = 2 };
#define AZ_TIER_EPS_MAX 0.0009765625
#define AZ_FAST_EM_MIN 1.0e-6

enum { AZ_ETIER_E1 = 1, AZ_ETIER_E2 = 2, AZ_ETIER_NUM = 3 };
#define AZ_ETIER_E1_MAX 0.01
#define AZ_ETIER_E2_MAX 0.1

template <bool ECC>
AZ_DEVICE int az_fast_window_tier(const FastK &k, const AzGrav &g, double t_a, double t_b, double dmax = 0.0)
{
    const double T = fmax(fabs(t_a), fabs(t_b)) + dmax;
    const double ae = fabs(k.eta_);
    const double th = fma(fabs(k.xmcof_), ae * fma(2.0 * ae, ae, 6.0), fabs(k.omgcof_) * T);
    const double da = T * fma(T, fma(T, fma(T, fabs(k.d4_), fabs(k.d3_)), fabs(k.d2_)), fabs(k.cc1_));
    const double dem = fma(fabs(k.bc4_), T, fabs(k.bc5_));
    const double em = fabs(k.ecb_) + dem;
    bool ok = (th <= AZ_ROT_16TH) & (da <= 0.25) & (em <= 0.9);
    ok &= k.ecb_ - dem >= AZ_FAST_EM_MIN;
    const double sam = k.sab_ * (1.0 - da);
    const double inv_am = 1.0 / (sam * sam);
    const double temp = inv_am / fma(-em, em, 1.0);
    const double el = fma(temp, fabs(k.aycof_), em);
    const double el2 = el * el;
    if (!ECC) ok &= el2 <= AZ_FAST_EL2;
    ok &= el2 <= 0.81;
    const double dc = fmax(fabs(t_a - k.tc_), fabs(t_b - k.tc_)) + dmax;
    const double eps = fma(temp * fabs(k.xlcof_), em, fma(fabs(k.nl2_) * dc, dc, T * T * T * fma(T, fma(T, fabs(k.nl5_), fabs(k.nl4_)), fabs(k.nl3_)))) +
                       fabs(k.udot_) * dmax;
    ok &= eps <= AZ_ROT_MED;
    const double inv_pl = inv_am / (1.0 - el2);
    const double temp2 = g.half_j2 * inv_pl * inv_pl;
    ok &= temp2 <= AZ_FAST_TEMP2;
    const double a_nd = fma(fabs(k.k_node_), temp2, fma(fabs(k.nodedot_), 0.5 * fabs(t_b - t_a) + dmax, fabs(k.xnodcf_) * T * T));
    ok &= a_nd <= AZ_ROT_MED;
    if (!ok) return -1;
    if (ECC) return el <= AZ_ETIER_E1_MAX ? (int)AZ_ETIER_E1 : (el <= AZ_ETIER_E2_MAX ? (int)AZ_ETIER_E2 : (int)AZ_TIER_GENERAL);
    return eps <= AZ_TIER_EPS_MAX ? AZ_TIER_EPS : AZ_TIER_GENERAL;
}
template <bool ECC>
AZ_DEVICE bool az_fast_window_ok(const FastK &k, const AzGrav &g, double t_a, double t_b, double dmax = 0.0)
{
    return az_fast_window_tier<ECC>(k, g, t_a, t_b, dmax) >= 0;
}

#ifndef AZ_FAST_PROBE
#define AZ_FAST_PROBE(name, value)
#endif
#ifndef AZ_FAST_PROBE_KEPLER
#define AZ_FAST_PROBE_KEPLER(name, value)
#endif

template <bool VEL, bool ECC = false, int DELTA = 0, int TIER = AZ_TIER_GENERAL, class K = FastK, class RC = RotCoefLit>
AZ_DEVICE bool az_sgp4_fast_step(const K &k, const AzGrav &g, const RC &rk, double t, FastCarry &st, double r[3],
                                  double v[3], double dl = 0.0)
{
    az_pair_advance<K::SCALAR>(st.sA, st.cA, k.sdA(), k.cdA());
    az_pair_advance<K::SCALAR>(st.sW, st.cW, k.sdW(), k.cdW());
    az_pair_advance<K::SCALAR>(st.sU, st.cU, k.sdU(), k.cdU());
    double sA = st.sA, cA = st.cA, sW = st.sW, cW = st.cW;
    if constexpr ((DELTA == 1 && ECC) || DELTA == 2) {
        const double a = k.mdot() * dl, b = k.argpdot() * dl;
        if constexpr (DELTA == 2 && ECC) {
            double pa, qa;
            az_pq_16th(a, rk, pa, qa);
            az_rot_apply2(sA, cA, pa, qa);
        } else if constexpr (DELTA == 2) {
            az_rotate_tiny2(sA, cA, a, rk);
        } else {
            sA = fma(st.cA, a, st.sA); cA = fma(-st.sA, a, st.cA);
        }
        if constexpr (DELTA == 2 && ECC) az_rotate_tiny2(sW, cW, b, rk);
        else { sW = fma(st.cW, b, st.sW); cW = fma(-st.sW, b, st.cW); }
    }
    const double t2 = t * t;
    constexpr bool E1 = ECC && TIER == AZ_ETIER_E1, E2 = ECC && TIER == AZ_ETIER_E2;

    const double dm = fma(k.eta(), cA, 1.0);
    const double th = fma(k.xmcof(), dm * dm * dm, fma(k.omgcof(), t, -k.xd()));
    const double tempa = fma(-t, fma(t, fma(t, fma(t, k.d4(), k.d3()), k.d2()), k.cc1()), 1.0);
    const double dtc = t - k.tc();
    double nl = fma(k.nl2() * dtc, dtc, t2 * (t * fma(t, fma(t, k.nl5(), k.nl4()), k.nl3())));
    if constexpr (DELTA != 0) nl = fma(k.udot(), dl, nl);
    bool bad = false;
    double p, q;
    if (E1) az_fpq_small(th, rk, p, q);
    else if (ECC) az_pq_16th(th, rk, p, q);
    else az_pq_ecc_scaled(th, rk, p, q);
    const double smm = fma(cA, p, fma(sA, q, sA));
    const double sw = fma(-cW, p, fma(sW, q, sW));
    const double cw = fma(sW, p, fma(cW, q, cW));
    const double em = fma(-k.bc5(), smm, fma(-k.bc4(), t, k.ecb()));
    AZ_FAST_PROBE(th, th)
    AZ_FAST_PROBE(em, em)

    const double sqrt_am = k.sab() * fabs(tempa);
    const double am = sqrt_am * sqrt_am;
    const double omem2 = fma(-em, em, 1.0);
    const double R = az_rcp(sqrt_am * omem2);
    const double ra = R * omem2;
    const double temp = ra * R;

    const double axnl = em * cw;
    const double aynl = fma(em, sw, temp * k.aycof());
    double s = st.sU, c = st.cU;
    {
        const double eps = fma(temp * k.xlcof(), axnl, nl);
        AZ_FAST_PROBE(eps, eps)
        if constexpr (!ECC && TIER >= AZ_TIER_EPS) az_rotate_tiny2(s, c, eps, rk);
        else {
            az_pq_16th(eps, rk, p, q);
            az_rot_apply2(s, c, p, q);
        }
    }

    const double el2 = fma(axnl, axnl, aynl * aynl);
    double ecose, esine, ome, inv_ome, betal, inv_omel2, inv_1pb;
    AZ_FAST_PROBE_KEPLER(el2, el2)
    if (!ECC || E1) {
        const double rden = az_rcp1(fma(-s, aynl, fma(-c, axnl, 1.0)));
        const double d0 = fma(axnl, s, -(aynl * c)) * rden;
        AZ_FAST_PROBE_KEPLER(d0, d0)
        if (E1) az_pq_ecc_scaled(d0, rk, p, q);
        else az_fpq_milli(d0, rk, p, q);
        az_rot_apply2(s, c, p, q);
        const double d1 = fma(axnl, s, fma(-aynl, c, -d0)) * rden;
        AZ_FAST_PROBE_KEPLER(d1, d1)
        {
            const double s1 = fma(c, d1, s);
            c = fma(-s, d1, c);
            s = s1;
        }
        if (E1) {
            const double d2 = fma(axnl, s, fma(-aynl, c, -(d0 + d1))) * rden;
            AZ_FAST_PROBE_KEPLER(d2, d2)
            const double s1 = fma(c, d2, s);
            c = fma(-s, d2, c);
            s = s1;
        }
        ecose = fma(axnl, c, aynl * s);
        esine = fma(axnl, s, -(aynl * c));
        ome = 1.0 - ecose;
        const double x = fma(-ome, rden, 1.0);
        inv_ome = fma(rden, E1 ? fma(x, fma(x, x, x), x) : fma(x, x, x), rden);
        betal = fma(el2, fma(el2, -0.125, -0.5), 1.0);
        inv_omel2 = el2 + 1.0;
        if (E1) inv_omel2 = fma(el2, inv_omel2, 1.0);
        inv_1pb = fma(el2, rk(RC_p8), 0.5);
    } else if (E2) {
        double rden = az_rcp1(fma(-s, aynl, fma(-c, axnl, 1.0)));
        const double d0 = fma(axnl, s, -(aynl * c)) * rden;
        AZ_FAST_PROBE_KEPLER(d0, d0)
        az_pq_med(d0, rk, p, q);
        az_rot_apply2(s, c, p, q);
        rden = az_rcp1(fma(-s, aynl, fma(-c, axnl, 1.0)));
        const double d1 = fma(axnl, s, fma(-aynl, c, -d0)) * rden;
        AZ_FAST_PROBE_KEPLER(d1, d1)
        az_fpq_milli(d1, rk, p, q);
        az_rot_apply2(s, c, p, q);
        rden = az_rcp1(fma(-s, aynl, fma(-c, axnl, 1.0)));
        const double d2 = fma(axnl, s, fma(-aynl, c, -(d0 + d1))) * rden;
        AZ_FAST_PROBE_KEPLER(d2, d2)
        {
            const double s1 = fma(c, d2, s);
            c = fma(-s, d2, c);
            s = s1;
        }
        ecose = fma(axnl, c, aynl * s);
        esine = fma(axnl, s, -(aynl * c));
        ome = 1.0 - ecose;
        inv_ome = fma(rden, fma(-ome, rden, 1.0), rden);
        const double omel2 = 1.0 - el2;
        const double rb = az_rsqrt(omel2);
        betal = omel2 * rb;
        inv_omel2 = rb * rb;
        inv_1pb = az_rcp(1.0 + betal);
    } else {
        double eps = 0.0, rden = 1.0, d = 0.0;
#pragma unroll
        for (int it = 0; it < 5; ++it) {
            rden = az_rcp1(fma(-s, aynl, fma(-c, axnl, 1.0)));
            d = fma(axnl, s, fma(-aynl, c, -eps)) * rden;
            eps += d;
            if (it == 0) {
                bad |= !(fabs(d) <= 0.5);
                az_pq_large(d, rk, p, q);
                az_rot_apply2(s, c, p, q);
            } else if (it == 1) {
                bad |= !(fabs(d) <= AZ_ROT_MED);
                az_pq_med(d, rk, p, q);
                az_rot_apply2(s, c, p, q);
            } else {
                bad |= !(fabs(d) <= AZ_ROT_SMALL);
                az_fpq_small(d, rk, p, q);
                az_rot_apply2(s, c, p, q);
            }
        }
        const double d2 = d * d;
        bad |= !(el2 * d2 * d2 < 4.0e-26);
        ecose = fma(axnl, c, aynl * s);
        esine = fma(axnl, s, -(aynl * c));
        ome = 1.0 - ecose;
        inv_ome = fma(rden, fma(-ome, rden, 1.0), rden);
        const double omel2 = 1.0 - el2;
        const double rb = az_rsqrt(omel2);
        betal = omel2 * rb;
        inv_omel2 = rb * rb;
        inv_1pb = az_rcp(1.0 + betal);
    }

    const double est = esine * inv_1pb;
    const double sinu = inv_ome * (s - fma(axnl, est, aynl));
    const double cosu = inv_ome * (c + fma(aynl, est, -axnl));
    const double sin2u = (sinu + sinu) * cosu;
    const double cos2u = fma(-2.0 * sinu, sinu, 1.0);

    const double inv_am = ra * ra;
    const double rl = am * ome;
    const double inv_pl = inv_am * inv_omel2;
    const double temp1 = g.half_j2 * inv_pl;
    const double temp2 = temp1 * inv_pl;

    const double mrt = fma(rl, fma(k.k_mrt() * temp2, betal, 1.0), k.k_c2u() * temp1 * cos2u);
    const double t2s = temp2 * sin2u;
    const double a_nd = fma(k.k_node(), t2s, fma(k.nodedot(), t - k.tmid(), k.xnodcf() * t2));
    AZ_FAST_PROBE(a_nd, a_nd)
    double ssu = sinu, csu = cosu, sn = k.sOc(), cn = k.cOc(), si = k.sinio(), ci = k.cosio();
    az_rotate_tiny2(ssu, csu, k.k_su() * t2s, rk);
    az_pq_16th(a_nd, rk, p, q);
    az_rot_apply2(sn, cn, p, q);
    az_rotate_tiny2(si, ci, k.k_inc() * temp2 * cos2u, rk);

    const double xmx = -sn * ci, xmy = cn * ci;
    const double rs = mrt * g.radius_km;
    const double ra_s = rs * ssu, ra_c = rs * csu;
    r[0] = fma(xmx, ra_s, cn * ra_c);
    r[1] = fma(xmy, ra_s, sn * ra_c);
    r[2] = si * ra_s;
    if (VEL) {
        const double rv = ra * g.vkmpersec;
        const double vk = rv * inv_ome;
        const double nxt = rv * inv_am * temp1;
        const double mvt = fma(-nxt * k.x1mth2(), sin2u, vk * esine);
        const double rvdot = fma(nxt, fma(k.x1mth2(), cos2u, k.k_rv()), vk * betal);
        const double va_s = fma(mvt, ssu, rvdot * csu), va_c = fma(mvt, csu, -(rvdot * ssu));
        v[0] = fma(xmx, va_s, cn * va_c);
        v[1] = fma(xmy, va_s, sn * va_c);
        v[2] = si * va_s;
    }
    return bad;
}
```

astroz_amd/csrc/kernels.h:

```cpp
#pragma once
#include <hip/hip_runtime.h>

#include <type_traits>

#include "init_device.h"
#include "propagate_device.h"
#include "fast_step.h"
#include "fast_step_f32.h"

#ifndef AZ_BLOCK
#define AZ_BLOCK 256
#endif
#ifndef AZ_PROP_FAST
#define AZ_PROP_FAST 1
#endif
#ifndef AZ_MIN_WAVES
#define AZ_MIN_WAVES 1
#endif
#ifndef AZ_ROWS_WAVES
#define AZ_ROWS_WAVES 3
#endif
#ifndef AZ_DEEP_WAVES
#define AZ_DEEP_WAVES 2
#endif
#define AZ_RESEED 256
#ifndef AZ_SM_CHUNK
#define AZ_SM_CHUNK 4
#endif

struct PropArgs {
    const double *el;
    const unsigned *flags;
    size_t n_pad;
    const unsigned *list;
    unsigned n_list;
    const double *times;
    unsigned n_times;
    const double *offsets;
    double *pos, *vel;
    const double *sin_g, *cos_g;
    const unsigned char *mask;
    unsigned char *err;
    size_t stride_sats;
    unsigned tile;
    unsigned tile_e, screen_nseg;
    unsigned tile_forced;
    const double *seeds;
    int mode;
    int f32;
    int tm_rows;
    int rows_compact;
    unsigned ecc_row0;
    const double *screen_target;
    union {
        double *part_d2;
        const AzObserver *obs;
    };
    unsigned *part_t;
    double uniform_step;
    int grid_exact_uniform;
    const float *delta;
    double delta_max;
    const double *delta64;
    int delta_wide;
    double grid_t0;
    const double *inc;
    const double *fast_rec;
    unsigned row_lo, row_hi;
    unsigned slot_lo, slot_hi;
    unsigned win_circ_lo, win_circ_hi, win_ecc_lo, win_ecc_hi;
    int arith32;
    unsigned n_circ;
    unsigned redo_slot0;
    unsigned *redo_count;
    unsigned *redo_next;
    unsigned *redo_items;
    const unsigned *rowmap;
    const double *tmp_pos, *tmp_vel;
    unsigned n_rows;
    const double *plan_win;
    const unsigned char *plan_flag;
    unsigned plan_stride;
    const unsigned *redo_static;
    AzGrav g;
};
enum { AZ_ROW_NEAR = 0, AZ_ROW_COPY = 1, AZ_ROW_ZERO = 2 };
enum { AZ_PLAN_sOc, AZ_PLAN_cOc, AZ_PLAN_sdU, AZ_PLAN_cdU, AZ_PLAN_s1U, AZ_PLAN_c1U, AZ_PLAN_NUM };
#define AZ_PLAN_OK 1u
#define AZ_PLAN_TC 2u
#define AZ_PLAN_TIER_SHIFT 2
#define AZ_PLAN_TIER_MASK 1u
#define AZ_PLAN_ETIER_MASK 3u
#ifndef AZ_ROWS_ETIERS
#define AZ_ROWS_ETIERS 1
#endif
#define AZ_PLAN_ECC 16u
#define AZ_PLAN_SET 32u

template <class T>
__device__ __forceinline__ void az_put3(T *o, const double r[3])
{
    o[0] = (T)r[0];
    o[1] = (T)r[1];
    o[2] = (T)r[2];
}
typedef double az_d2s __attribute__((ext_vector_type(2), aligned(8)));
typedef float az_f3s __attribute__((ext_vector_type(3), aligned(4)));
#ifndef AZ_ROWS_NT
#define AZ_ROWS_NT 1
#endif
__device__ __forceinline__ void az_put3_stream(double *o, const double r[3])
{
#if AZ_ROWS_NT
    const az_d2s a = {r[0], r[1]};
    __builtin_nontemporal_store(a, reinterpret_cast<az_d2s *>(o));
    __builtin_nontemporal_store(r[2], o + 2);
#else
    az_put3(o, r);
#endif
}
__device__ __forceinline__ void az_put3_stream(float *o, const double r[3])
{
#if AZ_ROWS_NT
    const az_f3s a = {(float)r[0], (float)r[1], (float)r[2]};
    __builtin_nontemporal_store(a, reinterpret_cast<az_f3s *>(o));
#else
    az_put3(o, r);
#endif
}

__device__ __forceinline__ void az_epilogue(double r[3], double v[3], int mode, bool vel, const double *sin_g,
                                            const double *cos_g, unsigned i)
{
    if (mode != 0) {
        const double sg = sin_g[i], cg = cos_g[i];
        az_to_ecef(r, sg, cg);
        if (vel) az_to_ecef(v, sg, cg);
        if (mode == 2) az_ecef_to_geodetic(r);
    }
}
template <bool VEL>
__device__ __forceinline__ void az_epilogue_topo(double r[3], double v[3], const PropArgs &p, unsigned i)
{
    const double sg = p.sin_g[i], cg = p.cos_g[i];
    az_to_ecef(r, sg, cg);
    if (VEL) az_to_ecef(v, sg, cg);
    az_topocentric<VEL>(r, v, *p.obs);
}

#define AZ_TM_ROW 256
#define AZ_SM_ROW (AZ_SM_CHUNK * 3 + 1)

typedef double az_d2 __attribute__((ext_vector_type(2)));

#if defined(AZ_STORE_POLICY) && AZ_STORE_POLICY == 1
#define AZ_ST1(ptr, val) __builtin_nontemporal_store((val), (ptr))
#define AZ_ST2(ptr, val) __builtin_nontemporal_store((val), (ptr))
#else
#define AZ_ST1(ptr, val) (*(ptr) = (val))
#define AZ_ST2(ptr, val) (*(ptr) = (val))
#endif

__device__ __forceinline__ double az_readlane_f64(double x, unsigned lane_uniform)
{
    const int lo = __builtin_amdgcn_readlane(__double2loint(x), (int)lane_uniform);
    const int hi = __builtin_amdgcn_readlane(__double2hiint(x), (int)lane_uniform);
    return __hiloint2double(hi, lo);
}

__device__ __forceinline__ void az_wave_lds_fence()
{
    __builtin_amdgcn_fence(__ATOMIC_RELEASE, "wavefront");
    __builtin_amdgcn_wave_barrier();
    __builtin_amdgcn_fence(__ATOMIC_ACQUIRE, "wavefront");
}

__device__ __forceinline__ void az_tm_flush(const double *L, double *row, size_t pitch, unsigned lane, unsigned par, bool last)
{
    const az_d2 *lp = reinterpret_cast<const az_d2 *>(L);
    az_d2 *g = reinterpret_cast<az_d2 *>(row);
    if (par == 0u) {
        AZ_ST2(g + lane, lp[32u + lane]);
        if (last && lane < 32u) AZ_ST2(g + 64u + lane, lp[96u + lane]);
    } else {
        az_d2 *gprev = reinterpret_cast<az_d2 *>(row - pitch);
        AZ_ST2(lane < 32u ? gprev + (64u + lane) : g + (lane - 32u), lp[lane < 32u ? 96u + lane : lane - 32u]);
        AZ_ST2(g + (32u + lane), lp[32u + lane]);
    }
}

template <int LAYOUT, bool VEL, bool DEEP, int FRAME, bool SCREEN = false>
__global__ void __launch_bounds__(AZ_BLOCK, (AZ_MIN_WAVES > 1 ? AZ_MIN_WAVES : (FRAME ? 1 : (DEEP ? (LAYOUT == 1 ? 1 : AZ_DEEP_WAVES) : 3)))) k_propagate(PropArgs p)
{
    constexpr int WAVES = AZ_BLOCK / 64;
    constexpr int SLICE = (LAYOUT == 1) ? (DEEP ? 0 : AZ_TM_ROW) : (AZ_SM_CHUNK > 0 ? 64 * AZ_SM_ROW : 0);
    constexpr int COLD = (DEEP ? (int)D_NUM : (int)C_NUM) * 64;
    __shared__ __attribute__((aligned(16))) double lds[WAVES * ((VEL ? 2 : 1) * SLICE + COLD)];

    const unsigned lane = threadIdx.x & 63u;
    const unsigned wave = threadIdx.x >> 6;
    double *lds_w = lds + wave * ((VEL ? 2 : 1) * SLICE + COLD);
    double *lds_p = lds_w;
    double *lds_v = lds_w + SLICE;
    double *cold = lds_w + (VEL ? 2 : 1) * SLICE + lane;
    ColdLds cold4{cold};

    const unsigned li0 = blockIdx.x * AZ_BLOCK + wave * 64;
    if (li0 >= p.n_list) return;
    const unsigned li = li0 + lane;
    const bool in_range = li < p.n_list;
    const unsigned s = p.list[in_range ? li : p.n_list - 1];
    const unsigned fl = p.flags[s];
    const bool wr = in_range && (p.mask == nullptr || p.mask[s] != 0) && s >= p.row_lo && s < p.row_hi;
    if (!SCREEN && !az_any(wr)) return;
    const double off = p.offsets ? p.offsets[s] : 0.0;
    const unsigned t0 = blockIdx.y * p.tile;
    const unsigned t1 = min(t0 + p.tile, p.n_times);

    const unsigned s_first = p.list[li0];
    const bool dense = (LAYOUT == 1) && !DEEP && (p.mask == nullptr) && !p.f32 && !az_any(!(wr && s == s_first + lane));

    double tcache = 0.0;
    const RotK rk = az_rotk();
    double best_d2 = __builtin_inf();
    unsigned best_t = 0xffffffffu;

    auto emit = [&](unsigned i, double (&r)[3], double (&v)[3], int rc) {
        if (FRAME == 3) az_epilogue_topo<VEL>(r, v, p, i);
        else if (FRAME) az_epilogue(r, v, p.mode, VEL, p.sin_g, p.cos_g, i);
        if (SCREEN) {
            const double *q = p.screen_target + (size_t)i * 3;
            const double dx = q[0] - r[0], dy = q[1] - r[1], dz = q[2] - r[2];
            const double d2 = dx * dx + dy * dy + dz * dz;
            if (rc == 0 && d2 < best_d2) {
                best_d2 = d2;
                best_t = i;
            }
            return;
        }
        if (DEEP) {
            if (rc != 0) {
                r[0] = r[1] = r[2] = 0.0;
                v[0] = v[1] = v[2] = 0.0;
                if (p.err && wr) p.err[(size_t)s * p.n_times + i] = (unsigned char)rc;
            }
        }
#if defined(AZ_ABLATE) && AZ_ABLATE == 1
        if (r[0] != 1.2345e300) return;
#endif
        if (LAYOUT == 1) {
            if (dense) {
                const unsigned par = (i - t0) & 1u;
                double *sp = lds_p + (par ? 0 : 64);
                sp[lane * 3 + 0] = r[0];
                sp[lane * 3 + 1] = r[1];
                sp[lane * 3 + 2] = r[2];
                if (VEL) {
                    double *sv = lds_v + (par ? 0 : 64);
                    sv[lane * 3 + 0] = v[0];
                    sv[lane * 3 + 1] = v[1];
                    sv[lane * 3 + 2] = v[2];
                }
                az_wave_lds_fence();
                const size_t ob = ((size_t)i * p.stride_sats + s_first) * 3;
                az_tm_flush(lds_p, p.pos + ob, (size_t)p.stride_sats * 3, lane, par, i + 1 == t1);
                if (VEL) az_tm_flush(lds_v, p.vel + ob, (size_t)p.stride_sats * 3, lane, par, i + 1 == t1);
                az_wave_lds_fence();
            } else if (wr) {
#if defined(AZ_ABLATE) && AZ_ABLATE == 3
                const size_t ob = (((size_t)i * p.stride_sats + s) * 3) & 0x1ffffu;
#else
                const size_t ob = ((size_t)i * p.stride_sats + s) * 3;
#endif
                if (p.f32) {
                    az_put3(reinterpret_cast<float *>(p.pos) + ob, r);
                    if (VEL) az_put3(reinterpret_cast<float *>(p.vel) + ob, v);
                    return;
                }
                AZ_ST1(p.pos + ob, r[0]);
                AZ_ST1(p.pos + ob + 1, r[1]);
                AZ_ST1(p.pos + ob + 2, r[2]);
                if (VEL) {
                    AZ_ST1(p.vel + ob, v[0]);
                    AZ_ST1(p.vel + ob + 1, v[1]);
                    AZ_ST1(p.vel + ob + 2, v[2]);
                }
            }
        } else if (AZ_SM_CHUNK == 0) {
            if (wr) {
                const size_t ob = ((size_t)s * p.n_times + i) * 3;
                if (p.f32) {
                    az_put3(reinterpret_cast<float *>(p.pos) + ob, r);
                    if (VEL) az_put3(reinterpret_cast<float *>(p.vel) + ob, v);
                    return;
                }
                AZ_ST1(p.pos + ob, r[0]);
                AZ_ST1(p.pos + ob + 1, r[1]);
                AZ_ST1(p.pos + ob + 2, r[2]);
                if (VEL) {
                    AZ_ST1(p.vel + ob, v[0]);
                    AZ_ST1(p.vel + ob + 1, v[1]);
                    AZ_ST1(p.vel + ob + 2, v[2]);
                }
            }
        } else {
            const unsigned k = (i - t0) % (AZ_SM_CHUNK > 0 ? AZ_SM_CHUNK : 1);
            double *row = lds_p + lane * AZ_SM_ROW + k * 3;
            row[0] = r[0];
            row[1] = r[1];
            row[2] = r[2];
            if (VEL) {
                double *vrow = lds_v + lane * AZ_SM_ROW + k * 3;
                vrow[0] = v[0];
                vrow[1] = v[1];
                vrow[2] = v[2];
            }
            const bool flush = (k == AZ_SM_CHUNK - 1) || (i + 1 == t1);
            if (flush) {
                az_wave_lds_fence();
                const unsigned nsteps = k + 1;
                const unsigned tb = i - k;
                const unsigned words = nsteps * 3;
                const unsigned total = 64 * words;
                for (unsigned w = lane; w < total; w += 64) {
                    const unsigned rl = w / words, cw = w - rl * words;
                    const unsigned lj = li0 + rl;
                    if (lj < p.n_list) {
                        const unsigned sj = p.list[lj];
                        if (p.mask == nullptr || p.mask[sj] != 0) {
                            const size_t ob = ((size_t)sj * p.n_times + tb) * 3 + cw;
                            if (p.f32) {
                                reinterpret_cast<float *>(p.pos)[ob] = (float)lds_p[rl * AZ_SM_ROW + cw];
                                if (VEL) reinterpret_cast<float *>(p.vel)[ob] = (float)lds_v[rl * AZ_SM_ROW + cw];
                            } else {
                                p.pos[ob] = lds_p[rl * AZ_SM_ROW + cw];
                                if (VEL) p.vel[ob] = lds_v[rl * AZ_SM_ROW + cw];
                            }
                        }
                    }
                }
                az_wave_lds_fence();
            }
        }
    };
    auto time_at = [&](unsigned i) {
        const unsigned k64 = __builtin_amdgcn_readfirstlane((i - t0) & 63u);
        if (k64 == 0) tcache = p.times[min(i + lane, p.n_times - 1)];
        return az_readlane_f64(tcache, k64) + off;
    };

    unsigned i = t0;
#if AZ_PROP_FAST
    if (!DEEP && p.inc != nullptr && p.uniform_step != 0.0 && p.delta == nullptr && p.delta64 == nullptr && !az_any(AZ_FLAG_ECLASS(fl) != 0)) {
        FastKCol k;
        bool window_ok;
        {
            FastK k0;
            az_load_fast(p.el, p.n_pad, s, fl, p.inc, 1, k0);
            az_fast_window(p.el, p.n_pad, s, p.times[t0] + off, p.times[t1 - 1] + off, p.uniform_step, k0);
            window_ok = !az_any(in_range && !az_fast_window_ok<false>(k0, p.g, p.times[t0] + off, p.times[t1 - 1] + off));
            static_assert((int)FC_NUM <= (int)C_NUM, "the fast step's cold constants share the generic step's LDS columns");
#define X(n) cold[FC_##n * AZ_COLD_STRIDE] = k0.n##_;
            AZ_FASTK_COLD(X)
#undef X
#define X(n) k.n##_ = k0.n##_;
            AZ_FASTK_HOT(X)
#undef X
            k.cold = cold;
            az_wave_lds_fence();
        }
        FastCarry fc;
        az_seed_fast(p.el, p.n_pad, s, p.times[t0] + off - p.uniform_step, k.tc_, fc);
#pragma unroll 1
        for (; window_ok && i < t1; ++i) {
            const double t = time_at(i);
            double r[3], v[3];
#if defined(AZ_ABLATE) && AZ_ABLATE == 2
            r[0] = t; r[1] = t + 1.0; r[2] = t + 2.0; v[0] = t + 3.0; v[1] = t + 4.0; v[2] = t + 5.0;
#else
            az_sgp4_fast_step<VEL, false>(k, p.g, RotCoefLit(), t, fc, r, v);
#endif
            emit(i, r, v, 0);
        }
    }
#endif
    if (i < t1) {
        const unsigned g0 = i;
        if ((g0 - t0) & 63u) tcache = p.times[min(g0 - ((g0 - t0) & 63u) + lane, p.n_times - 1)];
        Sgp4Lane e4;
        Sgp4Carry c4;
        Sdp4Lane e8;
        Sdp4Carry c8;
        if (DEEP) {
            az_load_sdp4(p.el, p.n_pad, s, fl, e8, ColdLds{cold});
            if (p.seeds) {
                const double *sd = p.seeds + (size_t)blockIdx.y * 3 * p.n_list + (in_range ? li : p.n_list - 1);
                c8.atime = sd[0];
                c8.xli = sd[p.n_list];
                c8.xni = sd[2 * (size_t)p.n_list];
            } else {
                c8.atime = 0.0;
                c8.xli = e8(H_xlamo);
                c8.xni = e8(H_no_unkozai);
            }
        } else {
            az_load_sgp4(p.el, p.n_pad, s, fl, e4, cold4);
            c4.t_prev = 0.0;
            c4.sW = c4.sO = c4.sA = 0.0;
            c4.cW = c4.cO = c4.cA = 1.0;
        }
#pragma unroll 1
        for (; i < t1; ++i) {
            const double t = time_at(i);
            double r[3], v[3];
            int rc = 0;
#if defined(AZ_ABLATE) && AZ_ABLATE == 2
            r[0] = t; r[1] = t + 1.0; r[2] = t + 2.0; v[0] = t + 3.0; v[1] = t + 4.0; v[2] = t + 5.0;
#else
            if (DEEP) {
                rc = az_sdp4_step<VEL>(e8, ColdLds{cold}, p.g, rk, t, c8, r, v);
            } else {
                const bool first = ((i - g0) % AZ_RESEED) == 0;
                az_sgp4_step<VEL>(e4, cold4, p.el, p.n_pad, s, p.g, rk, t, first, c4, r, v);
            }
#endif
            emit(i, r, v, rc);
        }
    }
    if (SCREEN && in_range) {
        p.part_d2[(size_t)blockIdx.y * p.n_list + li] = best_d2;
        p.part_t[(size_t)blockIdx.y * p.n_list + li] = best_t;
    }
}

__global__ void __launch_bounds__(64) k_deep_seed(const double *el, const unsigned *flags, size_t n_pad,
                                                  const unsigned *list, unsigned n_list, const double *times,
                                                  unsigned n_times, const double *offsets, unsigned tile,
                                                  double *seeds, int nearest, double *node_cache)
{
    __shared__ double cold_lds[D_NUM * 64];
    const unsigned li = blockIdx.x * 64 + threadIdx.x;
    const bool in_range = li < n_list;
    const unsigned s = list[in_range ? li : n_list - 1];
    const unsigned fl = flags[s];
    Sdp4Lane e;
    double *cold = cold_lds + threadIdx.x;
    az_load_sdp4(el, n_pad, s, fl, e, ColdLds{cold});
    Sdp4Carry cy;
    cy.atime = 0.0;
    cy.xli = e(H_xlamo);
    cy.xni = e(H_no_unkozai);
    if (node_cache && node_cache[s] != 0.0) {
        cy.atime = node_cache[s];
        cy.xli = node_cache[n_pad + s];
        cy.xni = node_cache[2 * n_pad + s];
    }
    Sdp4Carry near = cy;
    bool have_near = false;
    const double off = offsets ? offsets[s] : 0.0;
    const unsigned n_tiles = (n_times + tile - 1) / tile;
    for (unsigned k = 0; k < n_tiles; ++k) {
        double t = times[k * tile] + off;
        if (nearest) {
            const double t_end = times[min((k + 1) * tile, n_times) - 1] + off;
            if (t * t_end <= 0.0) t = 0.0;
            else if (fabs(t_end) < fabs(t)) t = t_end;
        }
        if (az_any(e.irez != 0)) az_resonance_advance(e, ColdLds{cold}, t, cy);
        if (!have_near || fabs(cy.atime) < fabs(near.atime)) {
            near = cy;
            have_near = true;
        }
        if (in_range) {
            double *sd = seeds + (size_t)k * 3 * n_list + li;
            sd[0] = cy.atime;
            sd[n_list] = cy.xli;
            sd[2 * (size_t)n_list] = cy.xni;
        }
    }
    if (node_cache && in_range && e.irez != 0 && have_near) {
        node_cache[s] = near.atime;
        node_cache[n_pad + s] = near.xli;
        node_cache[2 * n_pad + s] = near.xni;
    }
}

#ifndef AZ_ONE_SEG
#define AZ_ONE_SEG 1024
#endif
#define AZ_ONE_LISTS 64u
#define AZ_ONE_HEAD (32u * AZ_ONE_LISTS)
template <bool ITEMS = false>
__global__ void __launch_bounds__(64) k_one_satellite(const double *__restrict__ el, const unsigned *__restrict__ flags,
                                                            size_t n_pad, unsigned sat, const double *__restrict__ tsince,
                                                            unsigned n, double *pos, double *vel,
                                                            unsigned char *err, int interleaved, AzGrav g,
                                                            const double *__restrict__ offsets, int nan_on_error,
                                                            const unsigned *__restrict__ items = nullptr, unsigned list_cap = 0)
{
    const unsigned sub = ITEMS ? (blockIdx.x % AZ_ONE_LISTS) : 0u;
    const unsigned n_work = ITEMS ? items[32u * sub] * (AZ_ONE_SEG / 64u) : 1u;
#pragma unroll 1
    for (unsigned w = ITEMS ? blockIdx.x / AZ_ONE_LISTS : 0u; w < n_work; w += ITEMS ? gridDim.x / AZ_ONE_LISTS : 1u) {
    const unsigned i = ITEMS ? items[AZ_ONE_HEAD + sub * list_cap + w / (AZ_ONE_SEG / 64u)] * AZ_ONE_SEG + (w % (AZ_ONE_SEG / 64u)) * 64u + threadIdx.x
                             : blockIdx.x * 64 + threadIdx.x;
    if (ITEMS && i - threadIdx.x >= n) continue;
    const double t = tsince[i < n ? i : n - 1] + (offsets ? offsets[sat] : 0.0);
    const unsigned fl = flags[sat];
    double r[3], v[3];
    int rc = AZ_FLAG_ERR(fl);
    if (rc == 0) {
        if (fl & AZ_FLAG_DEEP) {
            Sdp4Lane e;
            Sdp4Carry c;
            __shared__ double cold_deep[D_NUM * 64];
            double *cold = cold_deep + threadIdx.x;
            az_load_sdp4(el, n_pad, sat, fl, e, ColdLds{cold});
            c.atime = 0.0;
            c.xli = e(H_xlamo);
            c.xni = e(H_no_unkozai);
            rc = az_sdp4_step<true>(e, ColdLds{cold}, g, az_rotk(), t, c, r, v);
        } else {
            Sgp4Lane e;
            Sgp4Carry c;
            ColdRegs cold;
            az_load_sgp4(el, n_pad, sat, fl, e, cold);
            c.t_prev = 0.0;
            az_sgp4_step<true>(e, cold, el, n_pad, sat, g, az_rotk(), t, true, c, r, v);
        }
    }
    if (rc != 0) {
        r[0] = r[1] = r[2] = nan_on_error ? __builtin_nan("") : 0.0;
        v[0] = v[1] = v[2] = 0.0;
    }
    if (i < n) {
        if (interleaved) {
            double *o = pos + (size_t)i * 6;
            o[0] = r[0]; o[1] = r[1]; o[2] = r[2]; o[3] = v[0]; o[4] = v[1]; o[5] = v[2];
        } else {
            pos[(size_t)i * 3] = r[0]; pos[(size_t)i * 3 + 1] = r[1]; pos[(size_t)i * 3 + 2] = r[2];
            if (vel) { vel[(size_t)i * 3] = v[0]; vel[(size_t)i * 3 + 1] = v[1]; vel[(size_t)i * 3 + 2] = v[2]; }
        }
        if (err) err[i] = (unsigned char)rc;
    }
    }
}

struct PlanArgs {
    const double *el;
    const unsigned *flags;
    size_t n_pad;
    const unsigned *list;
    unsigned n_list, n_circ, n_times, tile_c, tile_e, by_flags;
    unsigned f32_mixed;
    const double *times, *offsets, *inc;
    double step, dt_mult, delta_max, grid_t0;
    double *win;
    unsigned char *flag;
    unsigned *redo_static, *redo_c0, *redo_c1, *redo_items;
    AzGrav g;
};
__global__ void __launch_bounds__(256) k_plan_windows(PlanArgs a)
{
    const unsigned slot = blockIdx.x * 256 + threadIdx.x;
    const unsigned seg = blockIdx.y;
    if (slot >= a.n_list) return;
    const unsigned s = a.list[slot];
    const unsigned fl = a.flags[s];
    const bool ecc = a.by_flags ? AZ_FLAG_ECLASS(fl) != 0 : slot >= a.n_circ;
    const unsigned tile = ecc ? a.tile_e : a.tile_c;
    const unsigned t_lo = seg * tile;
    if (t_lo >= a.n_times) return;
    const unsigned t_hi = min(t_lo + tile, a.n_times);
    const double t_first = a.grid_t0 + (a.offsets ? a.offsets[s] : 0.0);
    const double w_a = fma((double)t_lo, a.step, t_first), w_b = fma((double)(t_hi - 1), a.step, t_first);
    FastK k0, k1;
    az_load_fast(a.el, a.n_pad, s, fl, a.inc, 0, k0);
    const double dt_mult = ecc ? 64.0 : a.dt_mult;
    if (dt_mult == 128.0) az_double_increments(k0);
    az_fast_window(a.el, a.n_pad, s, w_a, w_b, dt_mult * a.step, k0);
    az_load_fast(a.el, a.n_pad, s, fl, a.inc, 1, k1);
    az_fast_window(a.el, a.n_pad, s, w_a, w_b, a.step, k1);
    int tier = ecc ? az_fast_window_tier<true>(k0, a.g, w_a, w_b, a.delta_max) : az_fast_window_tier<false>(k0, a.g, w_a, w_b, a.delta_max);
    if (ecc && (AZ_ROWS_ETIERS == 0 || (AZ_ROWS_ETIERS == 2 && tier == AZ_ETIER_E2))) tier = min(tier, (int)AZ_TIER_GENERAL);
    bool ok = tier >= 0;
    if (!ecc && AZ_FLAG_ECLASS(fl) != 0) ok = false;
    if (!ecc && a.f32_mixed && !az_fast32p_window_ok(k0, w_a, w_b)) ok = false;
    const size_t at = (size_t)seg * a.n_list + slot;
    double *w = a.win + at * AZ_PLAN_NUM;
    w[AZ_PLAN_sOc] = k0.sOc_; w[AZ_PLAN_cOc] = k0.cOc_; w[AZ_PLAN_sdU] = k0.sdU_; w[AZ_PLAN_cdU] = k0.cdU_;
    w[AZ_PLAN_s1U] = k1.sdU_; w[AZ_PLAN_c1U] = k1.cdU_;
    a.flag[at] = (unsigned char)((ok ? AZ_PLAN_OK | ((unsigned)tier << AZ_PLAN_TIER_SHIFT) : 0u) | (k0.tc_ != 0.0 ? AZ_PLAN_TC : 0u) |
                                 (ecc ? AZ_PLAN_ECC : 0u) | AZ_PLAN_SET);
    if (!ok) {
        const unsigned k = atomicAdd(a.redo_static, 1u);
        a.redo_items[3 * (size_t)k + 0] = slot;
        a.redo_items[3 * (size_t)k + 1] = t_lo;
        a.redo_items[3 * (size_t)k + 2] = t_hi;
    }
}
__global__ void k_plan_arm(unsigned *redo_static, unsigned *c0, unsigned *c1)
{
    if (threadIdx.x == 0 && blockIdx.x == 0) *c0 = *c1 = *redo_static;
}
template <class K>
__device__ __forceinline__ bool az_plan_window(const PropArgs &p, unsigned seg, unsigned slot, double w_a, double w_b, K &k0, unsigned *tier = nullptr)
{
    const size_t at = (size_t)seg * p.plan_stride + slot;
    const double *w = p.plan_win + at * AZ_PLAN_NUM;
    const unsigned f = p.plan_flag[at];
    k0.tmid_ = 0.5 * (w_a + w_b);
    k0.tc_ = (f & AZ_PLAN_TC) ? k0.tmid_ : 0.0;
    k0.sOc_ = w[AZ_PLAN_sOc]; k0.cOc_ = w[AZ_PLAN_cOc]; k0.sdU_ = w[AZ_PLAN_sdU]; k0.cdU_ = w[AZ_PLAN_cdU];
    if (tier) *tier = (f >> AZ_PLAN_TIER_SHIFT) & ((f & AZ_PLAN_ECC) ? AZ_PLAN_ETIER_MASK : AZ_PLAN_TIER_MASK);
    return (f & AZ_PLAN_OK) != 0;
}

AZ_DEVICE double az_uniform(double x)
{
#ifdef AZ_HOST_EMUL
    return x;
#else
    return __hiloint2double(__builtin_amdgcn_readfirstlane(__double2hiint(x)),
                            __builtin_amdgcn_readfirstlane(__double2loint(x)));
#endif
}
AZ_DEVICE float az_uniform32(float x)
{
#ifdef AZ_HOST_EMUL
    return x;
#else
    return __int_as_float(__builtin_amdgcn_readfirstlane(__float_as_int(x)));
#endif
}
__device__ __forceinline__ const double *az_opaque_lds(const double *p)
{
    typedef __attribute__((address_space(3))) const double lds_cdouble;
    lds_cdouble *q = (lds_cdouble *)p;
    asm volatile("" : "+v"(q));
    return (const double *)q;
}
struct ColdBroadcast;
struct ColdBroadcast {
    double *p;
    const double *m = nullptr;
    __device__ __forceinline__ double operator()(int k) const { return p[k]; }
    __device__ __forceinline__ void set(int k, double v) const { p[k] = v; }
    __device__ __forceinline__ double mc(int k) const { return m[k]; }
    __device__ __forceinline__ ColdBroadcast fresh() const;
};
struct ColdBroadcastLit {
    double *p;
    __device__ __forceinline__ double operator()(int k) const { return p[k]; }
    __device__ __forceinline__ void set(int k, double v) const { p[k] = v; }
    __device__ __forceinline__ double mc(int k) const { return az_mc_literal(k); }
    __device__ __forceinline__ const ColdBroadcastLit &fresh() const { return *this; }
};
__device__ const double az_mc_table[MC_NUM] = AZ_MC_VALUES;
__device__ const double az_rc_table[RC_NUM] = AZ_RC_VALUES;
#define AZ_SC_NUM (MC_C5 + 1)
#define AZ_FAST_TABLE ((FCX_NUM + RC_NUM + AZ_SC_NUM + 1) & ~1)
struct McLds {
    const double *p;
    __device__ __forceinline__ double mc(int k) const { return p[k]; }
};
__device__ __forceinline__ void az_fill_fast_table(double *table, const double *__restrict__ rec, unsigned lane)
{
    static_assert(FCX_NUM + RC_NUM + AZ_SC_NUM <= 64, "one lane per table entry");
    const double *src = lane < FCX_NUM ? rec + lane
                        : lane < FCX_NUM + RC_NUM ? az_rc_table + (lane - FCX_NUM) : az_mc_table + (lane - (FCX_NUM + RC_NUM));
    if (lane < FCX_NUM + RC_NUM + AZ_SC_NUM) table[lane] = *src;
}
__device__ __forceinline__ ColdBroadcast ColdBroadcast::fresh() const { return ColdBroadcast{p, az_opaque_lds(m)}; }
#ifndef AZ_ROWSF_WAVES
#define AZ_ROWSF_WAVES 6
#endif
#ifndef AZ_ROWS_TIERS
#define AZ_ROWS_TIERS 1
#endif
#ifndef AZ_ROWSF32_WAVES
#define AZ_ROWSF32_WAVES 4
#endif
#ifndef AZ_ROWSF32P_WAVES
#define AZ_ROWSF32P_WAVES 3
#endif
#ifndef AZ_ROWSF_ECC_WAVES
#define AZ_ROWSF_ECC_WAVES 4
#endif
#ifndef AZ_ROWS_TLDS
#define AZ_ROWS_TLDS 1024
#endif

enum { AZ_SINK_F64 = 0, AZ_SINK_F32 = 1, AZ_SINK_SCREEN = 2 };

__device__ __forceinline__ void az_wave_argmin(double &d2, unsigned &t)
{
#pragma unroll
    for (int off = 32; off > 0; off >>= 1) {
        const double od = __shfl_xor(d2, off, 64);
        const unsigned ot = __shfl_xor(t, off, 64);
        if (od < d2 || (od == d2 && ot < t)) {
            d2 = od;
            t = ot;
        }
    }
}


#ifndef AZ_ROWS_LDS_STORE
#define AZ_ROWS_LDS_STORE 1
#endif
typedef float az_f4 __attribute__((ext_vector_type(4)));
template <class T>
__device__ __forceinline__ void az_stage3(T *stage, unsigned lane, const double r[3])
{
    stage[lane * 3 + 0] = (T)r[0];
    stage[lane * 3 + 1] = (T)r[1];
    stage[lane * 3 + 2] = (T)r[2];
}
typedef unsigned az_u4 __attribute__((ext_vector_type(4)));
struct AzRowSink {
    __amdgpu_buffer_rsrc_t pos, vel;
};
template <class T>
__device__ __forceinline__ AzRowSink az_row_sink(T *prow, T *vrow, unsigned n_times)
{
    const unsigned row_bytes = n_times * 3u * (unsigned)sizeof(T);
    return AzRowSink{__builtin_amdgcn_make_buffer_rsrc(prow, 0, row_bytes, 0x00020000),
                     __builtin_amdgcn_make_buffer_rsrc(vrow ? vrow : prow, 0, row_bytes, 0x00020000)};
}
#ifndef AZ_AUX_NT
#define AZ_AUX_NT 2
#endif
template <bool VEL, class T>
__device__ __forceinline__ void az_flush_stage(const T *stage, const AzRowSink &sink, unsigned base, unsigned lane)
{
    constexpr unsigned PIECES = 64 * 3 * sizeof(T) / 16;
    constexpr int aux = AZ_ROWS_NT ? AZ_AUX_NT : 0;
    const az_u4 *src = reinterpret_cast<const az_u4 *>(stage) + lane;
    const unsigned voff = lane * 16u, soff = base * 3u * (unsigned)sizeof(T);
    if constexpr (PIECES >= 64) {
        const az_u4 a = src[0];
        __builtin_amdgcn_raw_buffer_store_b128(a, sink.pos, voff, soff, aux);
        if (VEL) {
            const az_u4 c = src[PIECES];
            __builtin_amdgcn_raw_buffer_store_b128(c, sink.vel, voff, soff, aux);
        }
        if (lane < PIECES - 64) {
            const az_u4 b = src[64];
            __builtin_amdgcn_raw_buffer_store_b128(b, sink.pos, voff + 1024u, soff, aux);
            if (VEL) {
                const az_u4 d = src[PIECES + 64];
                __builtin_amdgcn_raw_buffer_store_b128(d, sink.vel, voff + 1024u, soff, aux);
            }
        }
    } else if (lane < PIECES) {
        const az_u4 a = src[0];
        __builtin_amdgcn_raw_buffer_store_b128(a, sink.pos, voff, soff, aux);
        if (VEL) {
            const az_u4 c = src[PIECES];
            __builtin_amdgcn_raw_buffer_store_b128(c, sink.vel, voff, soff, aux);
        }
    }
}
__device__ __forceinline__ unsigned az_xcd_row()
{
    const unsigned per_xcd = gridDim.x >> 3;
    const unsigned range = per_xcd <= 8u ? ((blockIdx.x + blockIdx.y) & 7u) : (blockIdx.x & 7u);
    return range * per_xcd + (blockIdx.x >> 3);
}
__device__ __forceinline__ unsigned az_list_slot(const PropArgs &p) { return p.slot_lo + az_xcd_row(); }
__device__ __forceinline__ unsigned az_list_end(const PropArgs &p) { return p.slot_hi ? p.slot_hi : p.n_list; }
template <bool VEL, class out_t>
__device__ __forceinline__ void az_rows_store(bool staged, bool full, bool live, unsigned lane, out_t *stage, out_t *prow,
                                              out_t *vrow, unsigned base, const double r[3], const double v[3], const AzRowSink &sink)
{
    if (staged && full) {
        az_stage3(stage, lane, r);
        if (VEL) az_stage3(stage + 192, lane, v);
        az_wave_lds_fence();
        az_flush_stage<VEL>(stage, sink, base, lane);
        az_wave_lds_fence();
    } else if (live) {
        az_put3_stream(prow + (size_t)(base + lane) * 3, r);
        if (VEL) az_put3_stream(vrow + (size_t)(base + lane) * 3, v);
    }
}

template <bool VEL>
__global__ void __launch_bounds__(64, 3) k_one_fast(const double *el, const unsigned *flags, size_t n_pad, unsigned sat,
                                                    const double *tsince, unsigned n, double *pos, double *vel, unsigned char *err,
                                                    AzGrav g, const double *offsets, unsigned *items, unsigned list_cap)
{
    const unsigned lane = threadIdx.x, seg = blockIdx.x, lo = seg * AZ_ONE_SEG;
    const unsigned cnt = min((unsigned)AZ_ONE_SEG, n - lo);
    const unsigned fl = flags[sat];
    __shared__ float dl_lds[AZ_ONE_SEG];
    __shared__ __attribute__((aligned(16))) double rows_stage[2 * 64 * 3];
    const double off = az_uniform(offsets ? offsets[sat] : 0.0);
    const bool ecc = AZ_FLAG_ECLASS(fl) != 0;
    bool ok = AZ_FLAG_ERR(fl) == 0 && !(fl & AZ_FLAG_DEEP) && cnt >= 128u;
    double t0 = 0.0, step = 0.0;
    FastK k;
    if (ok) {
        t0 = az_uniform(tsince[lo]) + off;
        step = ((az_uniform(tsince[lo + cnt - 1]) + off) - t0) / (double)(cnt - 1u);
        bool far = false;
#pragma unroll 4
        for (unsigned j = lane; j < (unsigned)AZ_ONE_SEG; j += 64u) {
            const unsigned jj = min(j, cnt - 1u);
            const double d = (tsince[lo + jj] + off) - fma((double)jj, step, t0);
            dl_lds[j] = (float)d;
            far |= !(fabs(d) <= AZ_DELTA_MAX);
        }
        ok = !az_any(far) && step != 0.0 && fabs(step) * (double)cnt <= 3000.0;
    }
    if (ok) {
#define L(f) el[(size_t)F_##f * n_pad + sat]
        double sdA, cdA, sdW, cdW;
        az_sincos(L(mdot) * (64.0 * step), sdA, cdA);
        az_sincos(L(argpdot) * (64.0 * step), sdW, cdW);
#undef L
        az_load_fast_with(el, n_pad, sat, fl, sdA, cdA, sdW, cdW, k);
        const double w_a = t0, w_b = fma((double)(cnt - 1u), step, t0);
        az_fast_window(el, n_pad, sat, w_a, w_b, 64.0 * step, k);
        ok = ecc ? az_fast_window_ok<true>(k, g, w_a, w_b, AZ_DELTA_MAX) : az_fast_window_ok<false>(k, g, w_a, w_b, AZ_DELTA_MAX);
    }
    if (ok) {
        FastCarry fc;
        az_seed_fast(el, n_pad, sat, fma((double)lane - 64.0, step, t0), k.tc_, fc);
        double *prow = pos + (size_t)lo * 3, *vrow = VEL ? vel + (size_t)lo * 3 : nullptr;
        const bool staged = ((reinterpret_cast<size_t>(prow) | (VEL ? reinterpret_cast<size_t>(vrow) : 0)) & 15u) == 0;
        const AzRowSink sink = az_row_sink(prow, vrow, cnt);
        az_wave_lds_fence();
#pragma unroll 1
        for (unsigned base = 0; base < cnt; base += 64u) {
            const unsigned i = base + lane;
            const bool live = i < cnt;
            const double dl = (double)dl_lds[i];
            const double t = fma((double)i, step, t0) + dl;
            double r[3], v[3];
            const bool bad = ecc ? az_sgp4_fast_step<VEL, true, 1>(k, g, RotCoefLit(), t, fc, r, v, dl)
                                 : az_sgp4_fast_step<VEL, false, 1>(k, g, RotCoefLit(), t, fc, r, v, dl);
            if (az_any(bad && live)) {
                ok = false;
                break;
            }
            az_rows_store<VEL>(staged, base + 64u <= cnt, live, lane, rows_stage, prow, vrow, base, r, v, sink);
            if (err && live) err[lo + i] = 0;
        }
    }
    if (!ok && lane == 0) {
        const unsigned sub = seg % AZ_ONE_LISTS;
        items[AZ_ONE_HEAD + sub * list_cap + atomicAdd(items + 32u * sub, 1u)] = seg;
    }
}

#define AZ_FRAME_SEG 256
template <bool VEL, int FRAME, int SINK, bool ECC, int DELTA = 0>
__global__ void __launch_bounds__(64, FRAME >= 2 ? 4 : (ECC ? AZ_ROWSF_ECC_WAVES : (FRAME == 1 || DELTA == 2 ? 5 : AZ_ROWSF_WAVES))) k_rows_fast(PropArgs p)
{
    typedef typename std::conditional<SINK == AZ_SINK_F32, float, double>::type out_t;
    const unsigned lane = threadIdx.x;
    const unsigned row = az_list_slot(p);
    [[maybe_unused]] const AzObserver obs = FRAME == 3 ? *p.obs : AzObserver{};
    if (row >= az_list_end(p)) return;
    const unsigned s = p.list[row];
    if (SINK != AZ_SINK_SCREEN && ((p.mask != nullptr && p.mask[s] == 0) || s < p.row_lo || s >= p.row_hi)) return;
    const unsigned t_lo = blockIdx.y * p.tile;
    if (t_lo >= p.n_times) return;
    const unsigned t_hi = min(t_lo + p.tile, p.n_times);
    unsigned base = t_lo;
    bool window_ok;
    unsigned tier = AZ_TIER_GENERAL;
    double best_d2 = __builtin_inf();
    unsigned best_t = 0xffffffffu;
    {
        __shared__ __attribute__((aligned(16))) double cold_lds[AZ_FAST_TABLE];
        __shared__ __attribute__((aligned(16))) out_t rows_stage[AZ_ROWS_LDS_STORE ? 2 * 64 * 3 : 4];
        const double off = az_uniform(p.offsets ? p.offsets[s] : 0.0);
        const double *__restrict__ rec = p.fast_rec + (size_t)s * FR_NUM;
        az_fill_fast_table(cold_lds, rec, lane);
        const size_t out_row = p.rows_compact ? (size_t)p.ecc_row0 + row : (size_t)s;
        out_t *prow = SINK == AZ_SINK_SCREEN ? nullptr : reinterpret_cast<out_t *>(p.pos) + out_row * p.n_times * 3;
        out_t *vrow = VEL ? reinterpret_cast<out_t *>(p.vel) + out_row * p.n_times * 3 : nullptr;
        const bool staged = AZ_ROWS_LDS_STORE && SINK != AZ_SINK_SCREEN &&
                            (((reinterpret_cast<size_t>(prow) | (VEL ? reinterpret_cast<size_t>(vrow) : 0)) & 15u) == 0);
        FastKBcast k;
        {
            const double w_a = fma((double)t_lo, p.uniform_step, p.grid_t0 + off), w_b = fma((double)(t_hi - 1), p.uniform_step, p.grid_t0 + off);
            window_ok = az_plan_window(p, blockIdx.y, row + p.redo_slot0, w_a, w_b, k, &tier);
            if (!window_ok) return;
            az_fast_rec_hot(rec, k);
            az_wave_lds_fence();
            if (DELTA && k.tc_ != 0.0 && lane == 0) cold_lds[FCX_udot] = fma(2.0 * rec[FC_nl2], k.tc_, rec[FCX_udot]);
        }
        typedef typename std::conditional<DELTA == 2, double, float>::type dl_t;
        __shared__ dl_t dl_lds[DELTA ? AZ_DELTA_SEG : 1];
        if (DELTA) {
            const dl_t *src = DELTA == 2 ? reinterpret_cast<const dl_t *>(p.delta64) : reinterpret_cast<const dl_t *>(p.delta);
#pragma unroll
            for (unsigned j = lane; j < AZ_DELTA_SEG; j += 64) dl_lds[j] = src[t_lo + j];
        }
        az_wave_lds_fence();
        const double step = p.uniform_step;
        const double t_first = p.grid_t0 + off;
        FastCarry fc;
        az_seed_fast_rec(rec, rec[FC_nl2], fma((double)(t_lo + lane) - 64.0, step, t_first), k.tc_, fc,
                         McLds{cold_lds + FCX_NUM + RC_NUM});
        __shared__ double gst_lds[FRAME ? 2 * AZ_FRAME_SEG : 2];
        if (FRAME) {
#pragma unroll
            for (unsigned j = lane; j < AZ_FRAME_SEG; j += 64) {
                const unsigned jj = min(t_lo + j, p.n_times - 1);
                gst_lds[2 * j] = p.sin_g[jj];
                gst_lds[2 * j + 1] = p.cos_g[jj];
            }
            az_wave_lds_fence();
        }
        AzRowSink sink{};
        if constexpr (SINK != AZ_SINK_SCREEN) sink = az_row_sink(prow, vrow, p.n_times);
        auto run = [&](auto tier_c, const unsigned t_end) __attribute__((always_inline)) {
        constexpr int TIER = decltype(tier_c)::value;
#pragma unroll 1
        for (; window_ok && base < t_end; base += 64) {
            const unsigned i = base + lane;
            const bool live = i < t_hi;
            double t = fma((double)i, step, t_first), dl = 0.0;
            if (DELTA) {
                dl = (double)dl_lds[i - t_lo];
                t += dl;
            }
            const double *cold_now = az_opaque_lds(cold_lds);
            k.cold = cold_now;
            const RotCoefLds rk{cold_now + FCX_NUM};
            double r[3], v[3];
#if defined(AZ_ABLATE) && AZ_ABLATE == 2
            r[0] = t; r[1] = t + 1.0; r[2] = t + 2.0; v[0] = t + 3.0; v[1] = t + 4.0; v[2] = t + 5.0;
#else
            const bool bad = az_sgp4_fast_step<VEL, ECC, DELTA, TIER>(k, p.g, rk, t, fc, r, v, dl);
            if (az_any(bad && live)) break;
#endif
            if (SINK == AZ_SINK_SCREEN) {
                const double *q = p.screen_target + (size_t)(live ? i : t_hi - 1) * 3;
                const double dx = q[0] - r[0], dy = q[1] - r[1], dz = q[2] - r[2];
                const double d2 = fma(dx, dx, fma(dy, dy, dz * dz));
                if (live && d2 < best_d2) {
                    best_d2 = d2;
                    best_t = i;
                }
                continue;
            }
            if (FRAME) {
                if (((base - t_lo) & (AZ_FRAME_SEG - 1u)) == 0u && base != t_lo) {
                    az_wave_lds_fence();
#pragma unroll
                    for (unsigned j = lane; j < AZ_FRAME_SEG; j += 64) {
                        const unsigned jn = min(base + j, p.n_times - 1);
                        gst_lds[2 * j] = p.sin_g[jn];
                        gst_lds[2 * j + 1] = p.cos_g[jn];
                    }
                    az_wave_lds_fence();
                }
                const unsigned jj = (i - t_lo) & (AZ_FRAME_SEG - 1u);
                const double sg = gst_lds[2 * jj], cg = gst_lds[2 * jj + 1];
                az_to_ecef(r, sg, cg);
                if (VEL) az_to_ecef(v, sg, cg);
                if (FRAME == 2) az_ecef_to_geodetic(r);
                if (FRAME == 3) az_topocentric<VEL>(r, v, obs);
            }
#if defined(AZ_ABLATE) && AZ_ABLATE == 1
            if (!(live && (r[0] + r[1] + r[2] + (VEL ? v[0] + v[1] + v[2] : 0.0)) == 1.2345e300)) continue;
#endif
            az_rows_store<VEL>(staged, base + 64 <= t_hi, live, lane, rows_stage, prow, vrow, base, r, v, sink);
        }
        };
        if constexpr (AZ_ROWS_TIERS && !ECC && FRAME == 0) run(std::integral_constant<int, AZ_TIER_EPS>(), tier == AZ_TIER_EPS ? t_hi : t_lo);
        if constexpr (AZ_ROWS_ETIERS && ECC && FRAME == 0 && DELTA != 2) {
            run(std::integral_constant<int, AZ_ETIER_E1>(), tier == AZ_ETIER_E1 ? t_hi : t_lo);
            if constexpr (AZ_ROWS_ETIERS == 1) run(std::integral_constant<int, AZ_ETIER_E2>(), tier == AZ_ETIER_E2 ? t_hi : t_lo);
        }
        run(std::integral_constant<int, AZ_TIER_GENERAL>(), t_hi);
    }
    if (SINK == AZ_SINK_SCREEN) {
        az_wave_argmin(best_d2, best_t);
        if (lane == 0) {
            p.part_d2[(size_t)blockIdx.y * p.plan_stride + row + p.redo_slot0] = best_d2;
            p.part_t[(size_t)blockIdx.y * p.plan_stride + row + p.redo_slot0] = best_t;
        }
    }
    if (ECC && base < t_hi && lane == 0) {
        const unsigned k = atomicAdd(p.redo_count, 1u);
        p.redo_items[3 * (size_t)k + 0] = row + p.redo_slot0;
        p.redo_items[3 * (size_t)k + 1] = base;
        p.redo_items[3 * (size_t)k + 2] = t_hi;
    }
}

#define AZ_TILE_SATS 16
#define AZ_TILE_SEG_MAX 1024
#define AZ_TILE_PITCH 49
template <bool VEL, int FRAME = 0, int DELTA = 0>
__global__ void __launch_bounds__(1024, 1) k_tiles_fast(PropArgs p)
{
    constexpr unsigned NA = VEL ? 2u : 1u;
    constexpr bool ECEF = FRAME != 0;
    [[maybe_unused]] const AzObserver obs = FRAME == 3 ? *p.obs : AzObserver{};
    __shared__ __attribute__((aligned(16))) double cold_all[AZ_TILE_SATS * AZ_FAST_TABLE];
    __shared__ __attribute__((aligned(16))) double tile[2 * NA * 64 * AZ_TILE_PITCH];
    __shared__ double gst[ECEF ? 2 * AZ_TILE_SEG_MAX : 2];
    const unsigned lane = threadIdx.x & 63u, w = __builtin_amdgcn_readfirstlane(threadIdx.x >> 6);
    double *cold_lds = cold_all + w * AZ_FAST_TABLE;
    const unsigned tile_id = az_xcd_row();
    const unsigned s_first = tile_id * AZ_TILE_SATS;
    if (s_first >= p.n_rows) return;
    const unsigned n_valid = min((unsigned)AZ_TILE_SATS, p.n_rows - s_first);
    const bool have = w < n_valid;
    const unsigned s = s_first + (have ? w : 0u);
    const unsigned fl = p.flags[s];
    const unsigned rm = p.rowmap[s], kind = rm >> 30, slot = rm & 0x3fffffffu;
    const unsigned t_lo = blockIdx.y * p.tile, t_hi = min(t_lo + p.tile, p.n_times);
    const bool in_window = have && s >= p.row_lo && s < p.row_hi && (p.mask == nullptr || p.mask[s] != 0);
    __shared__ unsigned writable_lds;
    if (threadIdx.x == 0) writable_lds = 0u;
    __syncthreads();
    if (lane == 0 && in_window) atomicOr(&writable_lds, 1u << w);
    __syncthreads();
    const unsigned writable = writable_lds;
    if (writable == 0u) return;
    const bool contig = writable == 0xffffu;
    bool dead = !(in_window && kind == AZ_ROW_NEAR);
    const bool copy = in_window && kind == AZ_ROW_COPY, zero = in_window && kind == AZ_ROW_ZERO;
    if (ECEF) {
        for (unsigned j = threadIdx.x; j < t_hi - t_lo; j += 1024u) {
            gst[2 * j] = p.sin_g[t_lo + j];
            gst[2 * j + 1] = p.cos_g[t_lo + j];
        }
    }
    const bool ecc = AZ_FLAG_ECLASS(fl) != 0;
    const double off = az_uniform(p.offsets ? p.offsets[s] : 0.0);
    const double step = p.uniform_step, t_first = p.grid_t0 + off;
    typedef double dl_t;
    __shared__ dl_t dl_lds[DELTA ? AZ_DELTA_SEG : 1];
    if (DELTA) {
        const dl_t *src = p.delta64;
        if (threadIdx.x < AZ_DELTA_SEG) dl_lds[threadIdx.x] = src[t_lo + threadIdx.x];
        if (!ECEF) __syncthreads();
    }
    if (ECEF) __syncthreads();
    FastKBcast k;
    FastCarry fc;
    if (!dead) {
        const double *__restrict__ rec = p.fast_rec + (size_t)s * FR_NUM;
        az_fill_fast_table(cold_lds, rec, lane);
        const double w_a = fma((double)t_lo, step, t_first), w_b = fma((double)(t_hi - 1), step, t_first);
        if (!az_plan_window(p, blockIdx.y, slot, w_a, w_b, k)) dead = true;
        az_fast_rec_hot(rec, k);
        az_wave_lds_fence();
        if (DELTA && k.tc_ != 0.0 && lane == 0) cold_lds[FCX_udot] = fma(2.0 * rec[FC_nl2], k.tc_, rec[FCX_udot]);
        az_wave_lds_fence();
        az_seed_fast_rec(rec, rec[FC_nl2], fma((double)(t_lo + lane) - 64.0, step, t_first), k.tc_, fc, McLds{cold_lds + FCX_NUM + RC_NUM});
    }
    unsigned f_lds[3], f_out[3], f_row = 0;
#pragma unroll
    for (unsigned m = 0; m < 3; ++m) {
        const unsigned q = 1024u * m + threadIdx.x, arr = q / 1536u, pq = q - arr * 1536u, row = pq / 24u, col = pq - row * 24u;
        f_lds[m] = arr < NA ? (arr * (64u * AZ_TILE_PITCH) + row * AZ_TILE_PITCH + col * 2u) * 8u : 0xffffffffu;
#if defined(AZ_TILE_ABLATE) && AZ_TILE_ABLATE == 5
        f_out[m] = (unsigned)(((size_t)row * p.stride_sats + (s_first & 511u)) * 24u + col * 16u);
#else
        f_out[m] = (unsigned)(((size_t)row * p.stride_sats + s_first) * 24u + col * 16u);
#endif
        f_row |= (row | (arr << 7)) << (8u * m);
        f_row |= (((writable >> ((col * 2u) / 3u)) & 1u) | (((writable >> ((col * 2u + 1u) / 3u)) & 1u) << 1)) << (24u + 2u * m);
    }
    const bool stream_out = ((p.stride_sats * 24u) & 127u) == 0 && ((reinterpret_cast<size_t>(p.pos) | (VEL ? reinterpret_cast<size_t>(p.vel) : 0)) & 127u) == 0;
    unsigned kiter = 0;
#pragma unroll 1
    for (unsigned base = t_lo; base < t_hi; base += 64, ++kiter) {
        const unsigned i = base + lane;
        const bool live = i < t_hi;
        double r[3], v[3];
        if (!dead) {
            double t = fma((double)i, step, t_first), dl = 0.0;
            if (DELTA) {
                dl = (double)dl_lds[i - t_lo];
                t += dl;
            }
            const double *cold_now = az_opaque_lds(cold_lds);
            k.cold = cold_now;
            const RotCoefLds rk{cold_now + FCX_NUM};
            const bool bad = ecc ? az_sgp4_fast_step<VEL, true, DELTA>(k, p.g, rk, t, fc, r, v, dl) : az_sgp4_fast_step<VEL, false, DELTA>(k, p.g, rk, t, fc, r, v, dl);
            if (ECEF) {
                const unsigned jj = min(i, t_hi - 1) - t_lo;
                const double sg = gst[2 * jj], cg = gst[2 * jj + 1];
                az_to_ecef(r, sg, cg);
                if (VEL) az_to_ecef(v, sg, cg);
                if (FRAME == 2) az_ecef_to_geodetic(r);
                if (FRAME == 3) az_topocentric<VEL>(r, v, obs);
            }
            if (az_any(bad && live)) {
                dead = true;
                if (lane == 0) {
                    const unsigned it = atomicAdd(p.redo_count, 1u);
                    p.redo_items[3 * (size_t)it + 0] = slot;
                    p.redo_items[3 * (size_t)it + 1] = base;
                    p.redo_items[3 * (size_t)it + 2] = t_hi;
                }
            }
        }
        if (copy) {
            const size_t at = ((size_t)slot * p.n_times + min(i, t_hi - 1)) * 3;
            r[0] = p.tmp_pos[at]; r[1] = p.tmp_pos[at + 1]; r[2] = p.tmp_pos[at + 2];
            if (VEL) { v[0] = p.tmp_vel[at]; v[1] = p.tmp_vel[at + 1]; v[2] = p.tmp_vel[at + 2]; }
        } else if (zero) {
            r[0] = r[1] = r[2] = 0.0;
            v[0] = v[1] = v[2] = 0.0;
        }
        double *buf = tile + (kiter & 1u) * (NA * 64 * AZ_TILE_PITCH);
        if (!dead || copy || zero) {
            double *q = buf + lane * AZ_TILE_PITCH + w * 3;
            q[0] = r[0]; q[1] = r[1]; q[2] = r[2];
            if (VEL) {
                q += 64 * AZ_TILE_PITCH;
                q[0] = v[0]; q[1] = v[1]; q[2] = v[2];
            }
        }
        __syncthreads();
#if defined(AZ_TILE_ABLATE) && AZ_TILE_ABLATE == 5
        const size_t gbase = 0;
#else
        const size_t gbase = (size_t)base * p.stride_sats * 3;
#endif
        const bool full = base + 64 <= t_hi;
        if (contig) {
            const char *bufc = reinterpret_cast<const char *>(buf);
            char *pos_b = reinterpret_cast<char *>(p.pos + gbase), *vel_b = VEL ? reinterpret_cast<char *>(p.vel + gbase) : nullptr;
#pragma unroll
            for (unsigned m = 0; m < 3; ++m) {
                if (f_lds[m] == 0xffffffffu || (!full && base + ((f_row >> (8u * m)) & 63u) >= t_hi)) continue;
                const az_d2s val = *reinterpret_cast<const az_d2s *>(bufc + f_lds[m]);
                az_d2s *g = reinterpret_cast<az_d2s *>((((f_row >> (8u * m)) & 128u) ? vel_b : pos_b) + f_out[m]);
                if (stream_out) __builtin_nontemporal_store(val, g);
                else *g = val;
            }
        } else {
            const char *bufc = reinterpret_cast<const char *>(buf);
            char *pos_b = reinterpret_cast<char *>(p.pos + gbase), *vel_b = VEL ? reinterpret_cast<char *>(p.vel + gbase) : nullptr;
#pragma unroll
            for (unsigned m = 0; m < 3; ++m) {
                const unsigned en = (f_row >> (24u + 2u * m)) & 3u;
                if (f_lds[m] == 0xffffffffu || en == 0u || (!full && base + ((f_row >> (8u * m)) & 63u) >= t_hi)) continue;
                const az_d2s val = *reinterpret_cast<const az_d2s *>(bufc + f_lds[m]);
                double *g = reinterpret_cast<double *>((((f_row >> (8u * m)) & 128u) ? vel_b : pos_b) + f_out[m]);
                if (en == 3u) *reinterpret_cast<az_d2s *>(g) = val;
                else if (en == 1u) g[0] = val.x;
                else g[1] = val.y;
            }
        }
    }
}

#include "cols_kernel.h"

__device__ __forceinline__ unsigned az_lds_address(const void *p)
{
    return (unsigned)(size_t)(__attribute__((address_space(3))) const void *)p;
}
__device__ __forceinline__ void az_stage_pair3(unsigned a, const az_f2 q[3])
{
    asm volatile("ds_write2_b32 %0, %1, %2 offset1:3\n\t"
                 "ds_write2_b32 %0, %3, %4 offset0:1 offset1:4\n\t"
                 "ds_write2_b32 %0, %5, %6 offset0:2 offset1:5"
                 :
                 : "v"(a), "v"(q[0].x), "v"(q[0].y), "v"(q[1].x), "v"(q[1].y), "v"(q[2].x), "v"(q[2].y));
}
__device__ __forceinline__ void az_flush_pair3(unsigned a, float *out, unsigned lane)
{
    az_f4 lo, hi;
    asm volatile("ds_read_b128 %0, %2\n\t"
                 "ds_read_b128 %1, %2 offset:1024\n\t"
                 "s_waitcnt lgkmcnt(0)"
                 : "=&v"(lo), "=&v"(hi)
                 : "v"(a));
    az_f4 *dst = reinterpret_cast<az_f4 *>(out);
    __builtin_nontemporal_store(lo, dst + lane);
    if (lane < 32) __builtin_nontemporal_store(hi, dst + lane + 64);
}

template <bool VEL, bool MIXED = false, bool DELTA = false>
__global__ void __launch_bounds__(64, MIXED ? AZ_ROWSF32P_WAVES : AZ_ROWSF32_WAVES) k_rows_fast32(PropArgs p)
{
    const unsigned lane = threadIdx.x;
    const unsigned row = az_list_slot(p);
    if (row >= az_list_end(p)) return;
    const unsigned s = p.list[row];
    const unsigned fl = p.flags[s];
    if ((p.mask != nullptr && p.mask[s] == 0) || s < p.row_lo || s >= p.row_hi) return;
    const unsigned t_lo = blockIdx.y * p.tile;
    const unsigned t_hi = min(t_lo + p.tile, p.n_times);
    unsigned base = t_lo;
    if (AZ_FLAG_ECLASS(fl) == 0) {
        __shared__ __attribute__((aligned(16))) float rows_stage[2 * 128 * 3];
        const double off = az_uniform(p.offsets ? p.offsets[s] : 0.0);
        float *prow = reinterpret_cast<float *>(p.pos) + (size_t)s * p.n_times * 3;
        float *vrow = VEL ? reinterpret_cast<float *>(p.vel) + (size_t)s * p.n_times * 3 : nullptr;
        const bool staged = AZ_ROWS_LDS_STORE &&
                            (((reinterpret_cast<size_t>(prow) | (VEL ? reinterpret_cast<size_t>(vrow) : 0)) & 15u) == 0);
        const double step = p.uniform_step;
        const double t_first = p.grid_t0 + off;
        __shared__ float once_lds[F32_NUM];
        FastK32Bcast k;
        FastCarry32 fc;
        bool window_ok;
        const unsigned stage_w = az_lds_address(rows_stage) + lane * 24, stage_r = az_lds_address(rows_stage) + lane * 16;
        {
            const double w_a = fma((double)t_lo, step, t_first), w_b = fma((double)(t_hi - 1), step, t_first);
            FastK k0, k1;
            az_load_fast(p.el, p.n_pad, s, fl, p.inc, 0, k0);
            az_double_increments(k0);
            window_ok = az_plan_window(p, blockIdx.y, row + p.redo_slot0, w_a, w_b, k0);
            if (!window_ok) return;
            az_fast_udot(k0);
            az_load_fast(p.el, p.n_pad, s, fl, p.inc, 1, k1);
            {
                const double *w = p.plan_win + ((size_t)blockIdx.y * p.plan_stride + row + p.redo_slot0) * AZ_PLAN_NUM;
                k1.sdU_ = w[AZ_PLAN_s1U]; k1.cdU_ = w[AZ_PLAN_c1U];
                k1.tc_ = k0.tc_; k1.tmid_ = k0.tmid_; k1.sOc_ = k0.sOc_; k1.cOc_ = k0.cOc_;
            }
            FastK32 kk;
            az_load_fast32(k0, k1, step, p.g, kk);
#define X(n) if (lane == 0) once_lds[F32_##n] = kk.n##_;
            AZ_F32_ONCE(X)
#undef X
#define X(n) k.n##_ = az_uniform32(kk.n##_);
            AZ_F32_MANY(X)
#undef X
#define U(n) k.n = az_uniform(kk.n);
            U(sab64) U(sdU) U(cdU) U(tc) U(tmid) U(s1U) U(c1U)
            if (MIXED) { U(abase_km64) U(rv0_64) U(sOc64) U(cOc64) U(sinio64) U(cosio64) }
#undef U
            az_wave_lds_fence();
            FastCarry f0;
            az_seed_fast(p.el, p.n_pad, s, fma((double)(t_lo + 2 * lane) - 128.0, step, t_first), k.tc, f0);
            az_seed_fast32(f0, k1, fc);
        }
        __shared__ __attribute__((aligned(8))) float dl_lds[DELTA ? AZ_DELTA_SEG : 2];
        if (DELTA) {
#pragma unroll
            for (unsigned j = lane; j < AZ_DELTA_SEG; j += 64) dl_lds[j] = p.delta[t_lo + j];
            az_wave_lds_fence();
        }
#pragma unroll 1
        for (; window_ok && base < t_hi; base += 128) {
            const unsigned i = base + 2 * lane;
            const bool live_a = i < t_hi, live_b = i + 1 < t_hi;
            const double t = fma((double)i, step, t_first);
            unsigned zero = 0;
            asm volatile("" : "+v"(zero));
            k.once = once_lds + zero;
            az_f2 r[3], v[3];
#if defined(AZ_ABLATE) && AZ_ABLATE == 2
            r[0] = az_splat2((float)t); r[1] = r[0] + 1.0f; r[2] = r[0] + 2.0f; v[0] = r[0] + 3.0f; v[1] = r[0] + 4.0f; v[2] = r[0] + 5.0f;
#else
            az_f2 dl = az_splat2(0.0f);
            if (DELTA) dl = *reinterpret_cast<const az_f2 *>(dl_lds + (i - t_lo));
            if (MIXED) az_sgp4_fast_step_f32p<VEL, DELTA>(k, p.g, t, fc, r, v, dl);
            else az_sgp4_fast_step_f32<VEL, DELTA>(k, p.g, t, fc, r, v, dl);
#endif
#if defined(AZ_ABLATE) && AZ_ABLATE == 1
            if (!(live_a && (r[0].x + r[1].x + r[2].x + r[0].y + r[1].y + r[2].y +
                             (VEL ? v[0].x + v[1].x + v[2].x + v[0].y + v[1].y + v[2].y : 0.0f)) == 1.2345e30f)) continue;
#endif
            if (staged && base + 128 <= t_hi) {
                az_stage_pair3(stage_w, r);
                az_flush_pair3(stage_r, prow + (size_t)base * 3, lane);
                if (VEL) {
                    az_stage_pair3(stage_w + 1536, v);
                    az_flush_pair3(stage_r + 1536, vrow + (size_t)base * 3, lane);
                }
            } else {
                if (live_a) {
                    const az_f3s a = {r[0].x, r[1].x, r[2].x};
                    __builtin_nontemporal_store(a, reinterpret_cast<az_f3s *>(prow + (size_t)i * 3));
                    if (VEL) {
// ... 622 lines not shown
```

Measured before the change: 98.34 billion.

## Precompute per-64-step Taylor blocks for secular polynomials in rows fast path

Adds a precomputed per-satellite, per-64-timestep table of re-centred polynomial coefficients (drag tempa, mean-motion nl, linear theta/em terms, node sin/cos and derivative). The planner fills the table when an error bound holds, and k_rows_fast stages blocks into LDS and evaluates lower-degree polynomials in a local offset. This replaces high-degree polynomial evaluation and node rotation per step. The cost is extra global memory for the table, extra planning work and LDS, a new plan slot, and a fallback path for windows that fail the bound.

Result: slower. 97.08 billion (-1.3%).

```diff
diff --git a/astroz_amd/csrc/astroz_hip.hip b/astroz_amd/csrc/astroz_hip.hip
--- a/astroz_amd/csrc/astroz_hip.hip
+++ b/astroz_amd/csrc/astroz_hip.hip
@@ -196,7 +196,8 @@
         DevBuf<double> win;
         DevBuf<unsigned char> flag;
         DevBuf<unsigned> redo;
-    } plan[4];
+        DevBuf<double> iter;
+    } plan[5];
     int last_plan = -1;
     DevBuf<double> d_inc;
     DevBuf<double> d_fast_rec;
@@ -559,8 +560,10 @@
     unsigned tile_c = 0, tile_e = 0;
     bool packed32 = false;
     bool mixed32 = false;
+    bool iter = false;
     int kind = 0;
 };
+constexpr size_t AZ_ITER_TABLE_MAX = (size_t)64 << 20;
 unsigned fast_window_cap(double step)
 {
     const double span = 3000.0 / std::max(std::fabs(step), 1e-9);
@@ -581,6 +584,10 @@
     f.mixed32 = f.packed32 && a.arith32 == 0;
     if (f.packed32) f.tile_c = std::max(128u, f.tile_c / 128u * 128u);
     f.kind = f.packed32 ? 1 : 0;
+    f.iter = AZ_ROWS_ITER && !a.delta && !a.delta64 && a.mode == AZ_OUT_TEME && !a.screen_target && !f.packed32 &&
+             std::max(f.tile_c, f.tile_e) <= 64u * (unsigned)AZ_ITER_STAGE &&
+             (size_t)n_sgp4 * ((a.n_times + 63u) / 64u) * FI_NUM * sizeof(double) <= AZ_ITER_TABLE_MAX;
+    if (f.iter) f.kind = 4;
     return f;
 }
 FastShape fast_shape_tiles(const PropArgs &a, unsigned n_rows)
@@ -595,8 +602,14 @@
 }
 
 template <bool VEL, int FRAME, int SINK, bool ECC>
-void launch_rows_fast(const PropArgs &a, unsigned n_slots, hipStream_t st)
-{
+void launch_rows_fast(const PropArgs &a, unsigned n_slots, hipStream_t st, bool iter = false)
+{
+    if constexpr (AZ_ROWS_ITER && FRAME == 0 && SINK != AZ_SINK_SCREEN) {
+        if (iter) {
+            hipLaunchKernelGGL((k_rows_fast<VEL, FRAME, SINK, ECC, 0, true>), dim3(pad8(n_slots), cgrid_y(a.n_times, a.tile)), dim3(64), 0, st, a);
+            return;
+        }
+    }
     with_delta(a.delta_wide ? 2 : (a.delta ? 1 : 0), [&](auto DELTA) {
         hipLaunchKernelGGL((k_rows_fast<VEL, FRAME, SINK, ECC, DELTA>), dim3(pad8(n_slots), cgrid_y(a.n_times, a.tile)), dim3(64), 0, st, a);
     });
@@ -618,7 +631,8 @@
 
 int32_t launch_near_fast(const PropArgs &a, bool vel, const FastShape &shape, dim3 rgrid, hipStream_t st, const EccSide &side)
 {
-    PropArgs e = ecc_part(a, shape.tile_e), c = a;
+    PropArgs e = ecc_part(a, shape.tile_e), c = a, r = a;
+    r.iter_tab = nullptr;
     c.n_list = a.n_circ;
     c.tile = shape.tile_c;
     unsigned n_e = e.n_list, n_c = c.n_list;
@@ -633,8 +647,8 @@
     if (beside)
         if (int32_t rc = stream_after(se, st, side.fork); rc != AZ_OK) return rc;
     with_outputs(a, vel, [&](auto VEL, auto FRAME, auto SINK) {
-        if (n_e) launch_rows_fast<VEL, FRAME, SINK, true>(e, n_e, se);
-        launch_redo<VEL, FRAME, SINK>(a, rgrid, se);
+        if (n_e) launch_rows_fast<VEL, FRAME, SINK, true>(e, n_e, se, shape.iter);
+        launch_redo<VEL, FRAME, SINK>(r, rgrid, se);
         if (n_c && FRAME == 0 && shape.packed32)
             with_bool(shape.mixed32, [&](auto MIXED) {
                 with_bool(a.delta != nullptr, [&](auto DELTA) {
@@ -642,7 +656,7 @@
                 });
             });
         else if (n_c)
-            launch_rows_fast<VEL, FRAME, SINK, false>(c, n_c, st);
+            launch_rows_fast<VEL, FRAME, SINK, false>(c, n_c, st, shape.iter);
     });
     return beside ? stream_after(st, se, side.join) : AZ_OK;
 }
@@ -676,7 +690,7 @@
     f.tile_e = std::min(rows_tile(std::max(n_sgp4 - n_circ, 1u), a.n_times, a.tile_forced ? a.tile_forced : 256u), fast_window_cap(a.uniform_step));
     if (a.delta || a.delta64) f.tile_e = std::min(f.tile_e, (unsigned)AZ_DELTA_SEG);
     f.tile_c = cols_tile(n_rows, a.n_times, a.tile_forced, a.uniform_step);
-    f.packed32 = f.mixed32 = false;
+    f.packed32 = f.mixed32 = f.iter = false;
     f.kind = 3;
     return f;
 }
@@ -892,9 +906,11 @@
         if (c->capturing) return AZ_RC_EAGER;
         drop_graphs(c);
         const size_t items = (size_t)n_list * n_seg + ((size_t)a.n_times + 63) / 64 * (c->n_sgp4 - c->n_circ);
-        if (pl.redo.cap < 4 + 3 * items || pl.win.cap < (size_t)n_list * n_seg * AZ_PLAN_NUM) HIP_TRY(hipStreamSynchronize(st));
+        const size_t iter_len = shape.iter ? (size_t)n_list * ((a.n_times + 63u) / 64u) * FI_NUM : 0;
+        if (pl.redo.cap < 4 + 3 * items || pl.win.cap < (size_t)n_list * n_seg * AZ_PLAN_NUM || pl.iter.cap < iter_len)
+            HIP_TRY(hipStreamSynchronize(st));
         if (pl.redo.ensure(4 + 3 * items) != AZ_OK || pl.win.ensure((size_t)n_list * n_seg * AZ_PLAN_NUM) != AZ_OK ||
-            pl.flag.ensure((size_t)n_list * n_seg) != AZ_OK)
+            pl.flag.ensure((size_t)n_list * n_seg) != AZ_OK || (iter_len && pl.iter.ensure(iter_len) != AZ_OK))
             return AZ_ERR_HIP;
         HIP_TRY(hipMemsetAsync(pl.redo.p, 0, 4 * sizeof(unsigned), st));
         HIP_TRY(hipMemsetAsync(pl.flag.p, 0, (size_t)n_list * n_seg, st));
@@ -906,6 +922,7 @@
         q.grid_t0 = a.grid_t0;
         q.f32_mixed = shape.mixed32 ? 1u : 0u;
         q.win = pl.win.p; q.flag = pl.flag.p;
+        q.iter = shape.iter ? pl.iter.p : nullptr;
         q.redo_static = pl.redo.p + 2; q.redo_c0 = pl.redo.p; q.redo_c1 = pl.redo.p + 1; q.redo_items = pl.redo.p + 4;
         q.g = a.g;
         hipLaunchKernelGGL(k_plan_windows, dim3((n_list + 255) / 256, n_seg), dim3(256), 0, st, q);
@@ -918,6 +935,7 @@
     a.plan_win = pl.win.p;
     a.plan_flag = pl.flag.p;
     a.plan_stride = n_list;
+    if (shape.iter) a.iter_tab = pl.iter.p;
     a.redo_static = pl.redo.p + 2;
     a.redo_count = pl.redo.p + pl.parity;
     a.redo_next = pl.redo.p + (pl.parity ^ 1u);
@@ -948,7 +966,7 @@
 unsigned plan_sig(const azh_constellation *c)
 {
     unsigned s = 0;
-    for (unsigned k = 0; k < 4; ++k) s |= (c->plan[k].parity & 1u) << k;
+    for (unsigned k = 0; k < 5; ++k) s |= (c->plan[k].parity & 1u) << k;
     return s;
 }
 
@@ -1134,7 +1152,7 @@
         }
     if (hit) {
         HIP_TRY(hipGraphLaunch(hit->exec, st));
-        for (unsigned k = 0; k < 4; ++k) c->plan[k].parity = (hit->sig_after >> k) & 1u;
+        for (unsigned k = 0; k < 5; ++k) c->plan[k].parity = (hit->sig_after >> k) & 1u;
         c->last_path = hit->path;
         c->last_plan = hit->plan;
         HIP_TRY(hipEventRecord(c->ev_graph, st));
@@ -1155,8 +1173,8 @@
         (void)hipGetLastError();
         return launch_all(c, d_pos, d_vel, layout, stride, d_err, st, f32, row_lo, row_hi);
     }
-    unsigned parity0[4];
-    for (unsigned k = 0; k < 4; ++k) parity0[k] = c->plan[k].parity;
+    unsigned parity0[5];
+    for (unsigned k = 0; k < 5; ++k) parity0[k] = c->plan[k].parity;
     c->capturing = true;
     const int32_t rc = launch_all(c, d_pos, d_vel, layout, stride, d_err, st, f32, row_lo, row_hi);
     c->capturing = false;
@@ -1166,7 +1184,7 @@
     if (rc != AZ_OK || e_end != hipSuccess || !graph || hipGraphInstantiate(&exec, graph, nullptr, nullptr, 0) != hipSuccess) {
         (void)hipGetLastError();
         if (graph) (void)hipGraphDestroy(graph);
-        for (unsigned k = 0; k < 4; ++k) c->plan[k].parity = parity0[k];
+        for (unsigned k = 0; k < 5; ++k) c->plan[k].parity = parity0[k];
         pending->fails += 1;
         if (rc != AZ_OK && rc != AZ_RC_EAGER) return rc;
         return launch_all(c, d_pos, d_vel, layout, stride, d_err, st, f32, row_lo, row_hi);
diff --git a/astroz_amd/csrc/fast_step.h b/astroz_amd/csrc/fast_step.h
--- a/astroz_amd/csrc/fast_step.h
+++ b/astroz_amd/csrc/fast_step.h
@@ -66,6 +66,67 @@
 #define X(n) AZ_MEMBER double n() const { return 0.0; }
     AZ_FASTK_DELTA(X)
 #undef X
+};
+
+enum FastIter { FI_T0, FI_T1, FI_T2, FI_N0, FI_N1, FI_N2, FI_N3, FI_TH0, FI_EM0, FI_sn, FI_cn, FI_ND1, FI_NUM };
+#define AZ_ITER_HALF 32.5
+#define AZ_ITER_RULE 1.0e-13
+#define AZ_ITER_ROT 0.0078125
+#ifndef AZ_ROWS_ITER
+#define AZ_ROWS_ITER 1
+#endif
+template <class K>
+AZ_DEVICE void az_fast_iter_block(const K &k, double nodeo, double t, double *__restrict__ b)
+{
+    const double d2 = k.d2(), d3 = k.d3(), d4 = k.d4();
+    b[FI_T0] = fma(-t, fma(t, fma(t, fma(t, d4, d3), d2), k.cc1()), 1.0);
+    b[FI_T1] = -fma(t, fma(t, fma(4.0 * t, d4, 3.0 * d3), 2.0 * d2), k.cc1());
+    b[FI_T2] = -fma(t, fma(6.0 * t, d4, 3.0 * d3), d2);
+    const double n2 = k.nl2(), n3 = k.nl3(), n4 = k.nl4(), n5 = k.nl5();
+    const double dtc = t - k.tc(), t2 = t * t;
+    b[FI_N0] = fma(n2 * dtc, dtc, t2 * (t * fma(t, fma(t, n5, n4), n3)));
+    b[FI_N1] = fma(2.0 * n2, dtc, t2 * fma(t, fma(5.0 * t, n5, 4.0 * n4), 3.0 * n3));
+    b[FI_N2] = fma(t, fma(t, fma(10.0 * t, n5, 6.0 * n4), 3.0 * n3), n2);
+    b[FI_N3] = fma(t, fma(10.0 * t, n5, 4.0 * n4), n3);
+    b[FI_TH0] = fma(k.omgcof(), t, -k.xd());
+    b[FI_EM0] = fma(-k.bc4(), t, k.ecb());
+    az_sincos(fma(k.xnodcf(), t2, fma(k.nodedot(), t, nodeo)), b[FI_sn], b[FI_cn]);
+    b[FI_ND1] = fma(2.0 * k.xnodcf(), t, k.nodedot());
+}
+template <class K, class = void>
+struct az_k_iter : std::false_type {};
+template <class K>
+struct az_k_iter<K, std::void_t<decltype(K::ITER)>> : std::integral_constant<bool, K::ITER> {};
+#define AZ_FASTK_ITER(X) X(T0) X(T1) X(T2) X(N0) X(N1) X(N2) X(N3) X(TH0) X(EM0) X(sn) X(cn) X(ND1)
+struct FastKIt : FastK {
+    static constexpr bool ITER = true;
+    double blk[FI_NUM];
+#define X(n) AZ_MEMBER double n() const { return blk[FI_##n]; }
+    AZ_FASTK_ITER(X)
+#undef X
+};
+struct FastKBcastItT {
+    static constexpr bool SCALAR = true;
+    static constexpr bool ITER = false;
+    const double *cold, *blk;
+#define X(n) double n##_;
+    AZ_FASTK_HOT(X)
+#undef X
+#define X(n) AZ_MEMBER double n() const { return n##_; }
+    AZ_FASTK_HOT(X)
+#undef X
+#define X(n) AZ_MEMBER double n() const { return blk[FI_##n]; }
+    AZ_FASTK_ITER(X)
+#undef X
+#define X(n) AZ_MEMBER double n() const { return cold[FC_##n]; }
+    AZ_FASTK_COLD(X)
+#undef X
+#define X(n) AZ_MEMBER double n() const { return cold[FCX_##n]; }
+    AZ_FASTK_DELTA(X)
+#undef X
+};
+struct FastKBcastIt : FastKBcastItT {
+    static constexpr bool ITER = true;
 };
 
 struct FastCarry {
@@ -362,6 +423,14 @@
     if (ECC) return el <= AZ_ETIER_E1_MAX ? (int)AZ_ETIER_E1 : (el <= AZ_ETIER_E2_MAX ? (int)AZ_ETIER_E2 : (int)AZ_TIER_GENERAL);
     return eps <= AZ_TIER_EPS_MAX ? AZ_TIER_EPS : AZ_TIER_GENERAL;
 }
+AZ_DEVICE bool az_fast_iter_ok(const FastK &k, double t_a, double t_b, double D)
+{
+    const double D3 = D * D * D, Tj = fmax(fabs(t_a), fabs(t_b)) + D;
+    bool ok = fma(D3, fma(4.0 * fabs(k.d4_), Tj, fabs(k.d3_)), D3 * D * fabs(k.d4_)) <= AZ_ITER_RULE * 0.75;
+    ok &= D3 * D * fma(D, fabs(k.nl5_), fma(5.0 * fabs(k.nl5_), Tj, fabs(k.nl4_))) <= AZ_ITER_RULE;
+    ok &= fma(fabs(k.k_node_), AZ_FAST_TEMP2, D * fma(fabs(k.xnodcf_), fma(2.0, Tj, D), fabs(k.nodedot_))) <= AZ_ITER_ROT;
+    return ok;
+}
 template <bool ECC>
 AZ_DEVICE bool az_fast_window_ok(const FastK &k, const AzGrav &g, double t_a, double t_b, double dmax = 0.0)
 {
@@ -397,14 +466,25 @@
         if constexpr (DELTA == 2 && ECC) az_rotate_tiny2(sW, cW, b, rk);
         else { sW = fma(st.cW, b, st.sW); cW = fma(-st.sW, b, st.cW); }
     }
-    const double t2 = t * t;
     constexpr bool E1 = ECC && TIER == AZ_ETIER_E1, E2 = ECC && TIER == AZ_ETIER_E2;
 
     const double dm = fma(k.eta(), cA, 1.0);
-    const double th = fma(k.xmcof(), dm * dm * dm, fma(k.omgcof(), t, -k.xd()));
-    const double tempa = fma(-t, fma(t, fma(t, fma(t, k.d4(), k.d3()), k.d2()), k.cc1()), 1.0);
-    const double dtc = t - k.tc();
-    double nl = fma(k.nl2() * dtc, dtc, t2 * (t * fma(t, fma(t, k.nl5(), k.nl4()), k.nl3())));
+    double th_lin, em_lin, tempa, nl, t2 = 0.0;
+    if constexpr (az_k_iter<K>::value) {
+        static_assert(DELTA == 0, "the ITER form is for exactly uniform grids");
+        th_lin = fma(k.omgcof(), t, k.TH0());
+        em_lin = fma(-k.bc4(), t, k.EM0());
+        tempa = fma(t, fma(t, k.T2(), k.T1()), k.T0());
+        nl = fma(t, fma(t, fma(t, k.N3(), k.N2()), k.N1()), k.N0());
+    } else {
+        t2 = t * t;
+        th_lin = fma(k.omgcof(), t, -k.xd());
+        em_lin = fma(-k.bc4(), t, k.ecb());
+        tempa = fma(-t, fma(t, fma(t, fma(t, k.d4(), k.d3()), k.d2()), k.cc1()), 1.0);
+        const double dtc = t - k.tc();
+        nl = fma(k.nl2() * dtc, dtc, t2 * (t * fma(t, fma(t, k.nl5(), k.nl4()), k.nl3())));
+    }
+    const double th = fma(k.xmcof(), dm * dm * dm, th_lin);
     if constexpr (DELTA != 0) nl = fma(k.udot(), dl, nl);
     bool bad = false;
     double p, q;
@@ -414,7 +494,7 @@
     const double smm = fma(cA, p, fma(sA, q, sA));
     const double sw = fma(-cW, p, fma(sW, q, sW));
     const double cw = fma(sW, p, fma(cW, q, cW));
-    const double em = fma(-k.bc5(), smm, fma(-k.bc4(), t, k.ecb()));
+    const double em = fma(-k.bc5(), smm, em_lin);
     AZ_FAST_PROBE(th, th)
     AZ_FAST_PROBE(em, em)
 
@@ -547,11 +627,19 @@
 
     const double mrt = fma(rl, fma(k.k_mrt() * temp2, betal, 1.0), k.k_c2u() * temp1 * cos2u);
     const double t2s = temp2 * sin2u;
-    const double a_nd = fma(k.k_node(), t2s, fma(k.nodedot(), t - k.tmid(), k.xnodcf() * t2));
+    double a_nd, sn, cn;
+    if constexpr (az_k_iter<K>::value) {
+        a_nd = fma(k.k_node(), t2s, fma(k.ND1(), t, k.xnodcf() * (t * t)));
+        sn = k.sn(); cn = k.cn();
+    } else {
+        a_nd = fma(k.k_node(), t2s, fma(k.nodedot(), t - k.tmid(), k.xnodcf() * t2));
+        sn = k.sOc(); cn = k.cOc();
+    }
     AZ_FAST_PROBE(a_nd, a_nd)
-    double ssu = sinu, csu = cosu, sn = k.sOc(), cn = k.cOc(), si = k.sinio(), ci = k.cosio();
+    double ssu = sinu, csu = cosu, si = k.sinio(), ci = k.cosio();
     az_rotate_tiny2(ssu, csu, k.k_su() * t2s, rk);
-    az_pq_16th(a_nd, rk, p, q);
+    if constexpr (az_k_iter<K>::value) az_pq_ecc_scaled(a_nd, rk, p, q);
+    else az_pq_16th(a_nd, rk, p, q);
     az_rot_apply2(sn, cn, p, q);
     az_rotate_tiny2(si, ci, k.k_inc() * temp2 * cos2u, rk);
 
diff --git a/astroz_amd/csrc/kernels.h b/astroz_amd/csrc/kernels.h
--- a/astroz_amd/csrc/kernels.h
+++ b/astroz_amd/csrc/kernels.h
@@ -45,7 +45,10 @@
     unsigned tile;
     unsigned tile_e, screen_nseg;
     unsigned tile_forced;
-    const double *seeds;
+    union {
+        const double *seeds;
+        const double *iter_tab;
+    };
     int mode;
     int f32;
     int tm_rows;
@@ -96,6 +99,7 @@
 #endif
 #define AZ_PLAN_ECC 16u
 #define AZ_PLAN_SET 32u
+#define AZ_PLAN_ITER 64u
 
 template <class T>
 __device__ __forceinline__ void az_put3(T *o, const double r[3])
@@ -558,6 +562,7 @@
     double *win;
     unsigned char *flag;
     unsigned *redo_static, *redo_c0, *redo_c1, *redo_items;
+    double *iter;
     AzGrav g;
 };
 __global__ void __launch_bounds__(256) k_plan_windows(PlanArgs a)
@@ -590,8 +595,14 @@
     double *w = a.win + at * AZ_PLAN_NUM;
     w[AZ_PLAN_sOc] = k0.sOc_; w[AZ_PLAN_cOc] = k0.cOc_; w[AZ_PLAN_sdU] = k0.sdU_; w[AZ_PLAN_cdU] = k0.cdU_;
     w[AZ_PLAN_s1U] = k1.sdU_; w[AZ_PLAN_c1U] = k1.cdU_;
+    const bool iter_ok = a.iter && ok && az_fast_iter_ok(k0, w_a, w_b, AZ_ITER_HALF * fabs(a.step));
     a.flag[at] = (unsigned char)((ok ? AZ_PLAN_OK | ((unsigned)tier << AZ_PLAN_TIER_SHIFT) : 0u) | (k0.tc_ != 0.0 ? AZ_PLAN_TC : 0u) |
-                                 (ecc ? AZ_PLAN_ECC : 0u) | AZ_PLAN_SET);
+                                 (ecc ? AZ_PLAN_ECC : 0u) | AZ_PLAN_SET | (iter_ok ? AZ_PLAN_ITER : 0u));
+    if (iter_ok) {
+        const double nodeo = a.el[(size_t)F_nodeo * a.n_pad + s];
+        double *b = a.iter + ((size_t)slot * ((a.n_times + 63u) / 64u) + t_lo / 64u) * FI_NUM;
+        for (unsigned t = t_lo; t < t_hi; t += 64u, b += FI_NUM) az_fast_iter_block(k0, nodeo, fma((double)t + 31.5, a.step, t_first), b);
+    }
     if (!ok) {
         const unsigned k = atomicAdd(a.redo_static, 1u);
         a.redo_items[3 * (size_t)k + 0] = slot;
@@ -604,7 +615,8 @@
     if (threadIdx.x == 0 && blockIdx.x == 0) *c0 = *c1 = *redo_static;
 }
 template <class K>
-__device__ __forceinline__ bool az_plan_window(const PropArgs &p, unsigned seg, unsigned slot, double w_a, double w_b, K &k0, unsigned *tier = nullptr)
+__device__ __forceinline__ bool az_plan_window(const PropArgs &p, unsigned seg, unsigned slot, double w_a, double w_b, K &k0, unsigned *tier = nullptr,
+                                               bool *iter_ok = nullptr)
 {
     const size_t at = (size_t)seg * p.plan_stride + slot;
     const double *w = p.plan_win + at * AZ_PLAN_NUM;
@@ -613,6 +625,7 @@
     k0.tc_ = (f & AZ_PLAN_TC) ? k0.tmid_ : 0.0;
     k0.sOc_ = w[AZ_PLAN_sOc]; k0.cOc_ = w[AZ_PLAN_cOc]; k0.sdU_ = w[AZ_PLAN_sdU]; k0.cdU_ = w[AZ_PLAN_cdU];
     if (tier) *tier = (f >> AZ_PLAN_TIER_SHIFT) & ((f & AZ_PLAN_ECC) ? AZ_PLAN_ETIER_MASK : AZ_PLAN_TIER_MASK);
+    if (iter_ok) *iter_ok = (f & AZ_PLAN_ITER) != 0;
     return (f & AZ_PLAN_OK) != 0;
 }
 
@@ -857,9 +870,13 @@
 }
 
 #define AZ_FRAME_SEG 256
-template <bool VEL, int FRAME, int SINK, bool ECC, int DELTA = 0>
+__device__ __forceinline__ void az_set_blocks(FastKBcastItT &k, const double *b) { k.blk = b; }
+__device__ __forceinline__ void az_set_blocks(FastKBcast &, const double *) {}
+#define AZ_ITER_STAGE 16
+template <bool VEL, int FRAME, int SINK, bool ECC, int DELTA = 0, bool ITER = false>
 __global__ void __launch_bounds__(64, FRAME >= 2 ? 4 : (ECC ? AZ_ROWSF_ECC_WAVES : (FRAME == 1 || DELTA == 2 ? 5 : AZ_ROWSF_WAVES))) k_rows_fast(PropArgs p)
 {
+    static_assert(!ITER || (FRAME == 0 && DELTA == 0 && SINK != AZ_SINK_SCREEN), "the ITER form: TEME rows on an exactly uniform grid");
     typedef typename std::conditional<SINK == AZ_SINK_F32, float, double>::type out_t;
     const unsigned lane = threadIdx.x;
     const unsigned row = az_list_slot(p);
@@ -873,23 +890,31 @@
     unsigned base = t_lo;
     bool window_ok;
     unsigned tier = AZ_TIER_GENERAL;
+    bool iter_ok = false;
     double best_d2 = __builtin_inf();
     unsigned best_t = 0xffffffffu;
     {
-        __shared__ __attribute__((aligned(16))) double cold_lds[AZ_FAST_TABLE];
+        __shared__ __attribute__((aligned(16))) double cold_lds[AZ_FAST_TABLE + (ITER ? AZ_ITER_STAGE * FI_NUM : 0)];
         __shared__ __attribute__((aligned(16))) out_t rows_stage[AZ_ROWS_LDS_STORE ? 2 * 64 * 3 : 4];
         const double off = az_uniform(p.offsets ? p.offsets[s] : 0.0);
         const double *__restrict__ rec = p.fast_rec + (size_t)s * FR_NUM;
         az_fill_fast_table(cold_lds, rec, lane);
+        if constexpr (ITER) {
+            const unsigned row_blocks = ((p.n_times + 63u) / 64u) * FI_NUM;
+            const double *__restrict__ blocks = p.iter_tab + (size_t)(row + p.redo_slot0) * row_blocks;
+#pragma unroll
+            for (unsigned j = lane; j < AZ_ITER_STAGE * FI_NUM; j += 64)
+                cold_lds[AZ_FAST_TABLE + j] = blocks[min((t_lo >> 6) * FI_NUM + j, row_blocks - 1u)];
+        }
         const size_t out_row = p.rows_compact ? (size_t)p.ecc_row0 + row : (size_t)s;
         out_t *prow = SINK == AZ_SINK_SCREEN ? nullptr : reinterpret_cast<out_t *>(p.pos) + out_row * p.n_times * 3;
         out_t *vrow = VEL ? reinterpret_cast<out_t *>(p.vel) + out_row * p.n_times * 3 : nullptr;
         const bool staged = AZ_ROWS_LDS_STORE && SINK != AZ_SINK_SCREEN &&
                             (((reinterpret_cast<size_t>(prow) | (VEL ? reinterpret_cast<size_t>(vrow) : 0)) & 15u) == 0);
-        FastKBcast k;
+        typename std::conditional<ITER, FastKBcastIt, FastKBcast>::type k;
         {
             const double w_a = fma((double)t_lo, p.uniform_step, p.grid_t0 + off), w_b = fma((double)(t_hi - 1), p.uniform_step, p.grid_t0 + off);
-            window_ok = az_plan_window(p, blockIdx.y, row + p.redo_slot0, w_a, w_b, k, &tier);
+            window_ok = az_plan_window(p, blockIdx.y, row + p.redo_slot0, w_a, w_b, k, &tier, &iter_ok);
             if (!window_ok) return;
             az_fast_rec_hot(rec, k);
             az_wave_lds_fence();
@@ -920,26 +945,35 @@
         }
         AzRowSink sink{};
         if constexpr (SINK != AZ_SINK_SCREEN) sink = az_row_sink(prow, vrow, p.n_times);
-        auto run = [&](auto tier_c, const unsigned t_end) __attribute__((always_inline)) {
+        [[maybe_unused]] const double delta = ((double)lane - 31.5) * step;
+        auto run = [&](auto tier_c, const unsigned t_end, auto form_c) __attribute__((always_inline)) {
         constexpr int TIER = decltype(tier_c)::value;
+        constexpr bool IT = decltype(form_c)::value;
 #pragma unroll 1
         for (; window_ok && base < t_end; base += 64) {
             const unsigned i = base + lane;
             const bool live = i < t_hi;
-            double t = fma((double)i, step, t_first), dl = 0.0;
+            double t, dl = 0.0;
+            if constexpr (IT) t = delta;
+            else t = fma((double)i, step, t_first);
             if (DELTA) {
                 dl = (double)dl_lds[i - t_lo];
                 t += dl;
             }
             const double *cold_now = az_opaque_lds(cold_lds);
             k.cold = cold_now;
+            if constexpr (IT) az_set_blocks(k, cold_now + AZ_FAST_TABLE + ((base - t_lo) >> 6) * FI_NUM);
             const RotCoefLds rk{cold_now + FCX_NUM};
             double r[3], v[3];
 #if defined(AZ_ABLATE) && AZ_ABLATE == 2
             r[0] = t; r[1] = t + 1.0; r[2] = t + 2.0; v[0] = t + 3.0; v[1] = t + 4.0; v[2] = t + 5.0;
 #else
-            const bool bad = az_sgp4_fast_step<VEL, ECC, DELTA, TIER>(k, p.g, rk, t, fc, r, v, dl);
-            if (az_any(bad && live)) break;
+            typedef typename std::conditional<ITER && !IT, FastKBcastItT, decltype(k)>::type k_form;
+            const bool bad = az_sgp4_fast_step<VEL, ECC, DELTA, TIER>(static_cast<const k_form &>(k), p.g, rk, t, fc, r, v, dl);
+            if (az_any(bad && live)) {
+                if constexpr (ITER) window_ok = false;
+                break;
+            }
 #endif
             if (SINK == AZ_SINK_SCREEN) {
                 const double *q = p.screen_target + (size_t)(live ? i : t_hi - 1) * 3;
@@ -975,12 +1009,15 @@
             az_rows_store<VEL>(staged, base + 64 <= t_hi, live, lane, rows_stage, prow, vrow, base, r, v, sink);
         }
         };
-        if constexpr (AZ_ROWS_TIERS && !ECC && FRAME == 0) run(std::integral_constant<int, AZ_TIER_EPS>(), tier == AZ_TIER_EPS ? t_hi : t_lo);
+        constexpr std::bool_constant<ITER> form;
+        const unsigned t_none = t_lo, t_all = ITER && !iter_ok ? t_lo : t_hi;
+        if constexpr (AZ_ROWS_TIERS && !ECC && FRAME == 0) run(std::integral_constant<int, AZ_TIER_EPS>(), tier == AZ_TIER_EPS ? t_all : t_none, form);
         if constexpr (AZ_ROWS_ETIERS && ECC && FRAME == 0 && DELTA != 2) {
-            run(std::integral_constant<int, AZ_ETIER_E1>(), tier == AZ_ETIER_E1 ? t_hi : t_lo);
-            if constexpr (AZ_ROWS_ETIERS == 1) run(std::integral_constant<int, AZ_ETIER_E2>(), tier == AZ_ETIER_E2 ? t_hi : t_lo);
-        }
-        run(std::integral_constant<int, AZ_TIER_GENERAL>(), t_hi);
+            run(std::integral_constant<int, AZ_ETIER_E1>(), tier == AZ_ETIER_E1 ? t_all : t_none, form);
+            if constexpr (AZ_ROWS_ETIERS == 1) run(std::integral_constant<int, AZ_ETIER_E2>(), tier == AZ_ETIER_E2 ? t_all : t_none, form);
+        }
+        run(std::integral_constant<int, AZ_TIER_GENERAL>(), t_all, form);
+        if constexpr (ITER) run(std::integral_constant<int, AZ_TIER_GENERAL>(), t_hi, std::false_type());
     }
     if (SINK == AZ_SINK_SCREEN) {
         az_wave_argmin(best_d2, best_t);
```
